# chagmgang/distributed_reinforcement_learning

Hardware: AMD Instinct MI355X
Metric: learner env-frames/sec (whole node), IMPALA deep-conv 84x84x4 (higher is better)
Workload: dtype bf16; 1 GPU; model=impala deep-conv 84x84x4 + LSTM256 V-trace, global_batch=32, seq_len=20, parallelism=dp1, num_action=18

## Files before the change

### distributed_reinforcement_learning_amd/models/blocks.py

```python

from __future__ import annotations

from typing import List, Optional, Sequence

import torch
import torch.nn as nn
import torch.nn.functional as F


class AtariConvStack(nn.Module):

    def __init__(self, in_channels: int):
        super().__init__()
        self.conv1 = nn.Conv2d(in_channels, 32, kernel_size=8, stride=4)
        self.conv2 = nn.Conv2d(32, 64, kernel_size=4, stride=2)
        self.conv3 = nn.Conv2d(64, 64, kernel_size=3, stride=1)
        self.out_features = 7 * 7 * 64
        self.conv1.to(memory_format=torch.channels_last)
        self.conv2.to(memory_format=torch.channels_last)
        self.conv3.to(memory_format=torch.channels_last)

    def forward(self, x_nhwc: torch.Tensor) -> torch.Tensor:
        if x_nhwc.is_cuda and x_nhwc.dtype == torch.uint8:
            from distributed_reinforcement_learning_amd.ops.conv_op import (
                atari_conv_stack, custom_stack_ok,
            )
            assert custom_stack_ok(self, x_nhwc), (
                "uint8 frames on GPU require the custom conv stack "
                "(bf16 weights + built extension)")
            return atari_conv_stack(self, x_nhwc)
        x = x_nhwc.to(self.conv1.weight.dtype).permute(0, 3, 1, 2)
        if x.device.type == "cuda":
            x = x.contiguous(memory_format=torch.channels_last)
        else:
            x = x.contiguous()
        x = F.relu(self.conv1(x))
        x = F.relu(self.conv2(x))
        x = F.relu(self.conv3(x))
        return x.permute(0, 2, 3, 1).flatten(1)


class ActionEmbedding(nn.Module):

    def __init__(self, num_action: int, hidden: int = 256):
        super().__init__()
        self.num_action = num_action
        self.table = nn.Parameter(torch.empty(num_action, hidden))
        self.bias1 = nn.Parameter(torch.zeros(hidden))
        nn.init.kaiming_uniform_(self.table, a=5 ** 0.5)
        self.fc2 = nn.Linear(hidden, hidden)
        self.out_features = hidden

    def forward(self, prev_action: torch.Tensor) -> torch.Tensor:
        from distributed_reinforcement_learning_amd.ops import embed_op, available
        t = self.table
        if (t.is_cuda and t.dtype == torch.bfloat16
                and t.shape[1] == 256 and self.fc2.out_features == 256
                and available()):
            return embed_op.fused_action_embed(
                prev_action.long(), t, self.bias1, self.fc2.weight,
                self.fc2.bias)
        x = F.relu(embed_op.embed_lookup(t, prev_action) + self.bias1)
        return F.relu(self.fc2(x))


class MLPHead(nn.Module):

    def __init__(self, in_features: int, hidden_list: Sequence[int],
                 out_features: int,
                 final_activation: Optional[str] = None):
        super().__init__()
        layers: List[nn.Module] = []
        prev = in_features
        for h in hidden_list:
            layers.append(nn.Linear(prev, h))
            prev = h
        self.hidden = nn.ModuleList(layers)
        self.out = nn.Linear(prev, out_features)
        self.final_activation = final_activation

    def logits(self, x: torch.Tensor) -> torch.Tensor:
        x = x.to(self.out.weight.dtype)
        for layer in self.hidden:
            x = F.relu(layer(x))
        return self.out(x)

    def forward(self, x: torch.Tensor) -> torch.Tensor:
        x = self.logits(x)
        if self.final_activation == "softmax":
            x = F.softmax(x.float(), dim=-1)
        return x


class _AugGateWeight(torch.autograd.Function):

    PAD = 8

    @staticmethod
    def forward(ctx, weight: torch.Tensor, bias: torch.Tensor):
        K, G = weight.shape
        ctx.K = K
        return weight.as_strided((K + _AugGateWeight.PAD, G), (G, 1))

    @staticmethod
    def backward(ctx, d_aug: torch.Tensor):
        return d_aug[:ctx.K], d_aug[ctx.K]


class LSTMCellTF(nn.Module):

    def __init__(self, input_size: int, hidden_size: int,
                 forget_bias: float = 1.0):
        super().__init__()
        self.input_size = input_size
        self.hidden_size = hidden_size
        self.forget_bias = forget_bias
        self.weight = nn.Parameter(
            torch.empty(input_size + hidden_size, 4 * hidden_size))
        self.bias = nn.Parameter(torch.zeros(4 * hidden_size))
        nn.init.xavier_uniform_(self.weight)

    def gates_from_xh(self, xh: torch.Tensor) -> torch.Tensor:
        if xh.is_cuda and xh.dtype == torch.bfloat16:
            return torch.addmm(self.bias, xh, self.weight)
        return torch.addmm(self.bias.to(xh.dtype), xh, self.weight)

    def _aug_weight_ok(self) -> bool:
        w, b = self.weight, self.bias
        if not (w.is_cuda and w.dtype == torch.bfloat16
                and b.dtype == w.dtype and w.numel() % 8 == 0
                and w.data_ptr() + w.numel() * w.element_size()
                == b.data_ptr()):
            return False
        need = (w.storage_offset() + w.numel()
                + _AugGateWeight.PAD * w.shape[1]) * w.element_size()
        return w.untyped_storage().nbytes() >= need

    def _ones_col(self, n: int, xh_dtype, dev) -> torch.Tensor:
        cache = getattr(self, "_ones_cache", None)
        if cache is None:
            cache = self._ones_cache = {}
        key = (n, xh_dtype, dev)
        if key not in cache:
            pad = torch.zeros(n, _AugGateWeight.PAD, dtype=xh_dtype,
                              device=dev)
            pad[:, 0] = 1
            cache[key] = pad
        return cache[key]

    def forward_cat(self, parts, c: torch.Tensor):
        dtype = parts[0].dtype
        parts = [p if p.dtype == dtype else p.to(dtype) for p in parts]
        if self._aug_weight_ok():
            n = parts[0].shape[0]
            xh = torch.cat(parts + [self._ones_col(n, dtype,
                                                   parts[0].device)], dim=1)
            g = torch.mm(xh, _AugGateWeight.apply(self.weight, self.bias))
        else:
            xh = torch.cat(parts, dim=1)
            g = self.gates_from_xh(xh)
        from distributed_reinforcement_learning_amd.ops.lstm_op import (
            lstm_fused_step,
        )
        if g.is_cuda:
            return lstm_fused_step(g, c.float(), self.forget_bias)
        return lstm_fused_step(g.float(), c.float(), self.forget_bias)

    def forward_xh(self, xh: torch.Tensor, c: torch.Tensor):
        from distributed_reinforcement_learning_amd.ops.lstm_op import (
            lstm_fused_step,
        )
        g = self.gates_from_xh(xh)
        if g.is_cuda:
            return lstm_fused_step(g, c.float(), self.forget_bias)
        return lstm_fused_step(g.float(), c.float(), self.forget_bias)

    def gates(self, x: torch.Tensor, h: torch.Tensor) -> torch.Tensor:
        xh = torch.cat([x, h.to(x.dtype)], dim=1)
        return torch.addmm(self.bias.to(xh.dtype), xh, self.weight)

    def forward(self, x: torch.Tensor, h: torch.Tensor, c: torch.Tensor):
        g = self.gates(x, h)
        from distributed_reinforcement_learning_amd.ops import lstm_fused_step
        if g.is_cuda:
            return lstm_fused_step(g, c.float(), self.forget_bias)
        return lstm_fused_step(g.float(), c.float(), self.forget_bias)
```

### distributed_reinforcement_learning_amd/models/impala_actor_critic.py

```python

from __future__ import annotations

import torch
import torch.nn as nn

from distributed_reinforcement_learning_amd.models.blocks import (
    ActionEmbedding, AtariConvStack, LSTMCellTF, MLPHead,
)


class ImpalaActorCritic(nn.Module):
    def __init__(self, input_shape, num_action: int, lstm_hidden_size: int = 256):
        super().__init__()
        h, w, c = input_shape
        assert (h, w) == (84, 84), "Atari conv stack expects 84x84 frames"
        self.num_action = num_action
        self.lstm_hidden_size = lstm_hidden_size
        self.conv = AtariConvStack(c)
        self.action_emb = ActionEmbedding(num_action)
        feat = self.conv.out_features + self.action_emb.out_features
        self.lstm = LSTMCellTF(feat, lstm_hidden_size)
        self.policy_head = MLPHead(lstm_hidden_size, [256, 256], num_action,
                                   "softmax")
        self.value_head = MLPHead(lstm_hidden_size, [256, 256], 1, None)

    def single_step(self, state: torch.Tensor, prev_action: torch.Tensor,
                    h: torch.Tensor, c: torch.Tensor):
        feat = torch.cat(
            [self.conv(state), self.action_emb(prev_action)], dim=1)
        new_h, new_c = self.lstm(feat, h, c)
        policy = self.policy_head(new_h)
        value = self.value_head(new_h).squeeze(-1)
        return policy, value, new_h, new_c

    def forward(self, state, prev_action, h, c):
        return self.single_step(state, prev_action, h, c)

    def _unroll_features(self, traj_state, traj_prev_action, traj_h, traj_c):
        B, T = traj_state.shape[:2]
        flat_state = traj_state.reshape(B * T, *traj_state.shape[2:])
        flat_pa = traj_prev_action.reshape(B * T)
        flat_h = traj_h.reshape(B * T, -1)
        flat_c = traj_c.reshape(B * T, -1)
        conv_out = self.conv(flat_state)
        emb = self.action_emb(flat_pa)
        new_h, _ = self.lstm.forward_cat([conv_out, emb, flat_h], flat_c)
        return new_h, B, T

    def unroll(self, traj_state: torch.Tensor, traj_prev_action: torch.Tensor,
               traj_h: torch.Tensor, traj_c: torch.Tensor):
        h, B, T = self._unroll_features(traj_state, traj_prev_action,
                                        traj_h, traj_c)
        policy = self.policy_head(h)
        value = self.value_head(h).squeeze(-1)
        return policy.reshape(B, T, -1), value.reshape(B, T)

    def unroll_logits(self, traj_state, traj_prev_action, traj_h, traj_c):
        h, B, T = self._unroll_features(traj_state, traj_prev_action,
                                        traj_h, traj_c)
        from distributed_reinforcement_learning_amd.ops.mlp_heads_op import (
            fused_mlp_heads, heads_fusable,
        )
        if heads_fusable(self, h):
            logits, value = fused_mlp_heads(h.float(), self.policy_head,
                                            self.value_head)
            return logits.reshape(B, T, -1), value.reshape(B, T)
        logits = self.policy_head.logits(h)
        value = self.value_head(h).squeeze(-1)
        return logits.reshape(B, T, -1), value.reshape(B, T)
```

### distributed_reinforcement_learning_amd/ops/conv_op.py

```python

from __future__ import annotations

import torch

from distributed_reinforcement_learning_amd import ops as _ops

_LAYER_CO = {0: 32, 1: 32, 2: 64, 3: 64}

_WGRAD_STREAM = None


def _side_enabled() -> bool:
    import os
    return os.environ.get("DRLA_WGRAD_SIDE") == "1"


def wgrad_stream() -> torch.cuda.Stream:
    global _WGRAD_STREAM
    if _WGRAD_STREAM is None:
        _WGRAD_STREAM = torch.cuda.Stream()
    return _WGRAD_STREAM


def join_wgrad_stream() -> None:
    if _WGRAD_STREAM is not None:
        torch.cuda.current_stream().wait_stream(_WGRAD_STREAM)


STASH_INPUTS = False


class _ConvLayer(torch.autograd.Function):
    @staticmethod
    def forward(ctx, x: torch.Tensor, w_flat: torch.Tensor,
                bias_f32: torch.Tensor, layer: int):
        ext = _ops.require_ext()
        stash = STASH_INPUTS and layer <= 1
        y, x_st = ext.conv_fwd(layer, x.contiguous(), w_flat.contiguous(),
                               bias_f32.contiguous(), stash)
        ctx.save_for_backward(x_st if stash else x, w_flat, y)
        ctx.layer = layer
        return y

    @staticmethod
    def backward(ctx, dy: torch.Tensor):
        x, w_flat, y = ctx.saved_tensors
        ext = _ops.require_ext()
        layer = ctx.layer
        co = _LAYER_CO[layer]
        if not (dy.is_contiguous() or (dy.stride(-1) == 1
                                        and dy.dim() >= 2)):
            dy = dy.contiguous()
        dy_m = ext.relu_mask_bwd(dy, y, co, layer)
        if _side_enabled():
            cur = torch.cuda.current_stream()
            side = wgrad_stream()
            side.wait_stream(cur)
            with torch.cuda.stream(side):
                dw, dbias = ext.conv_wgrad(layer, x, dy_m)
            if not torch.cuda.is_current_stream_capturing():
                cur.wait_stream(side)
                for t in (dw, dbias):
                    t.record_stream(cur)
                for t in (x, dy_m):
                    t.record_stream(side)
        else:
            dw, dbias = ext.conv_wgrad(layer, x, dy_m)
        dx = None
        if layer >= 2 and ctx.needs_input_grad[0]:
            dx = ext.conv_dgrad(layer, dy_m, w_flat)
        return dx, dw, dbias, None


def conv_layer(x: torch.Tensor, conv: torch.nn.Conv2d,
               layer: int) -> torch.Tensor:
    w = conv.weight
    co = w.shape[0]
    w_flat = w.permute(0, 2, 3, 1).reshape(co, -1)
    return _ConvLayer.apply(x, w_flat, conv.bias, layer)


def atari_conv_stack(stack, x_u8_nhwc: torch.Tensor) -> torch.Tensor:
    ci = x_u8_nhwc.shape[-1]
    l1 = 0 if ci == 4 else 1
    y = conv_layer(x_u8_nhwc, stack.conv1, l1)
    y = conv_layer(y, stack.conv2, 2)
    y = conv_layer(y, stack.conv3, 3)
    return y.reshape(y.shape[0], -1)


def custom_stack_ok(stack, x: torch.Tensor) -> bool:
    return (x.is_cuda and x.dtype == torch.uint8
            and x.shape[1] == 84 and x.shape[2] == 84
            and x.shape[3] in (1, 4)
            and stack.conv1.weight.dtype == torch.bfloat16
            and _ops.available())
```

### distributed_reinforcement_learning_amd/ops/embed_op.py

```python

from __future__ import annotations

import torch

from distributed_reinforcement_learning_amd import ops as _ops


class _EmbedLookup(torch.autograd.Function):
    @staticmethod
    def forward(ctx, table: torch.Tensor, idx: torch.Tensor):
        ctx.save_for_backward(idx)
        ctx.num_rows = table.shape[0]
        ctx.want_bf16 = table.dtype == torch.bfloat16
        return table.index_select(0, idx)

    @staticmethod
    def backward(ctx, grad_out: torch.Tensor):
        (idx,) = ctx.saved_tensors
        ext = _ops.require_ext()
        grad_table = ext.embed_bwd(idx.contiguous(),
                                   grad_out.contiguous(), ctx.num_rows,
                                   ctx.want_bf16)
        return grad_table, None


def embed_lookup(table: torch.Tensor, idx: torch.Tensor) -> torch.Tensor:
    if table.is_cuda:
        return _EmbedLookup.apply(table, idx.long())
    return torch.nn.functional.embedding(idx.long(), table)


class _FusedActionEmbed(torch.autograd.Function):

    @staticmethod
    def forward(ctx, idx, table, b1, w2, b2):
        ext = _ops.require_ext()
        out, a1 = ext.embed_mlp_fwd(idx, table, b1, w2, b2)
        ctx.save_for_backward(idx, a1, out, w2)
        ctx.A = table.shape[0]
        ctx.set_materialize_grads(False)
        return out

    @staticmethod
    def backward(ctx, dy):
        idx, a1, out, w2 = ctx.saved_tensors
        ext = _ops.require_ext()
        if dy is None:
            return (None,) * 5
        if not (dy.dim() == 2 and dy.stride(1) == 1):
            dy = dy.contiguous()
        dz2, dtable, db1, db2 = ext.embed_mlp_bwd(
            dy.to(torch.bfloat16), out, a1, w2, idx, ctx.A)
        dw2 = dz2.t().mm(a1)
        return None, dtable, db1, dw2, db2


def fused_action_embed(idx, table, b1, w2, b2):
    return _FusedActionEmbed.apply(idx, table, b1, w2, b2)
```

### distributed_reinforcement_learning_amd/ops/hip/bind.cpp

```cpp

#include <torch/extension.h>
#include <ATen/hip/HIPContext.h>
#include <hip/hip_runtime.h>

#include <algorithm>
#include <array>
#include <tuple>

#include "drla_kernels.h"

namespace {

hipStream_t cur_stream() {
  return at::hip::getCurrentHIPStream().stream();
}

void check_gpu_contig(const torch::Tensor& t, const char* name) {
  TORCH_CHECK(t.is_cuda(), name, " must be on the GPU");
  TORCH_CHECK(t.is_contiguous(), name, " must be contiguous");
}

template <typename... Ts>
void check_all_gpu_contig(const char* what, const Ts&... ts) {
  (check_gpu_contig(ts, what), ...);
// ... 27 lines not shown
torch::Tensor normalize_frames_f32(torch::Tensor frames) {
  check_gpu_contig(frames, "frames");
  TORCH_CHECK(frames.scalar_type() == torch::kUInt8, "frames must be uint8");
  auto out = torch::empty_like(frames, frames.options().dtype(torch::kFloat));
  const long long n = frames.numel();
  const long long n4 = n / 4;
  if (n4 > 0) {
    hipLaunchKernelGGL(drla_u8_normalize_f32, dim3(drla_grid(n4)),
                       dim3(DRLA_BLOCK), 0, cur_stream(),
                       reinterpret_cast<const uchar4*>(frames.data_ptr<uint8_t>()),
                       reinterpret_cast<float4*>(out.data_ptr<float>()), n4);
  }
  if (n % 4) {
    hipLaunchKernelGGL(drla_u8_normalize_f32_tail, dim3(1), dim3(DRLA_BLOCK),
                       0, cur_stream(), frames.data_ptr<uint8_t>(),
                       out.data_ptr<float>(), n4 * 4, n);
  }
  return out;
}

torch::Tensor normalize_frames_bf16(torch::Tensor frames) {
  check_gpu_contig(frames, "frames");
  TORCH_CHECK(frames.scalar_type() == torch::kUInt8, "frames must be uint8");
  auto out = torch::empty_like(frames,
                               frames.options().dtype(torch::kBFloat16));
  const long long n = frames.numel();
  const long long n4 = n / 4;
  if (n4 > 0) {
    hipLaunchKernelGGL(drla_u8_normalize_bf16, dim3(drla_grid(n4)),
                       dim3(DRLA_BLOCK), 0, cur_stream(),
                       reinterpret_cast<const uchar4*>(frames.data_ptr<uint8_t>()),
                       reinterpret_cast<ushort4v*>(out.data_ptr()), n4);
  }
  if (n % 4) {
    hipLaunchKernelGGL(drla_u8_normalize_bf16_tail, dim3(1), dim3(DRLA_BLOCK),
                       0, cur_stream(), frames.data_ptr<uint8_t>(),
                       BF16PM(out), n4 * 4, n);
  }
  return out;
}

torch::Tensor vtrace_scan(torch::Tensor deltas, torch::Tensor discounts,
                          torch::Tensor cs) {
  for (auto* t : {&deltas, &discounts, &cs}) {
    check_gpu_contig(*t, "vtrace input");
    TORCH_CHECK(t->scalar_type() == torch::kFloat, "vtrace wants float32");
  }
  const int B = deltas.size(0);
  const int T = deltas.size(1);
  auto out = torch::empty_like(deltas);
  hipLaunchKernelGGL(drla_vtrace_scan, dim3(drla_grid(B)), dim3(DRLA_BLOCK),
                     0, cur_stream(), deltas.data_ptr<float>(),
                     discounts.data_ptr<float>(), cs.data_ptr<float>(),
                     out.data_ptr<float>(), B, T);
  return out;
}

constexpr auto kConvFwdU8 = std::array{&drla_conv_fwd_l1, &drla_conv_fwd_l1_c1};
constexpr auto kConvFwdBf16 = std::array{&drla_conv_fwd_l2, &drla_conv_fwd_l3};
constexpr auto kConvWgradU8 =
    std::array{&drla_conv_wgrad_l1, &drla_conv_wgrad_l1_c1};
constexpr auto kConvWgradBf16 =
    std::array{&drla_conv_wgrad_l2, &drla_conv_wgrad_l3};

const DrlaConvLayer& conv_layer(int layer) {
  TORCH_CHECK(layer >= 0 && layer < 4, "bad layer");
  return DRLA_CONV_LAYERS[layer];
}
int conv_m_tiles(int rows) { return (rows + DRLA_CONV_BM - 1) / DRLA_CONV_BM; }

torch::Tensor mfma_probe(torch::Tensor A, torch::Tensor B) {
  check_gpu_contig(A, "A");
  check_gpu_contig(B, "B");
  auto D = torch::empty({16, 16}, A.options().dtype(torch::kFloat));
  hipLaunchKernelGGL(drla_mfma_probe, dim3(1), dim3(64), 0, cur_stream(),
                     static_cast<const bf16raw*>(A.data_ptr()),
                     static_cast<const bf16raw*>(B.data_ptr()),
                     D.data_ptr<float>());
  return D;
}

std::tuple<torch::Tensor, torch::Tensor> conv_fwd(
    int layer, torch::Tensor in, torch::Tensor w, torch::Tensor bias,
    bool stash_input) {
  check_gpu_contig(in, "in");
  check_gpu_contig(w, "w");
  check_gpu_contig(bias, "bias");
  const auto& cfg = conv_layer(layer);
  const int batch = in.size(0);
  auto out = torch::empty({batch, cfg.ho, cfg.wo, cfg.co},
                          in.options().dtype(torch::kBFloat16));
  const dim3 grid(conv_m_tiles(batch * cfg.ho * cfg.wo));
  torch::Tensor x_stash;
  unsigned char* stashp = nullptr;
  if (stash_input) {
    TORCH_CHECK(layer <= 1, "input stash is a u8-layer feature");
    TORCH_CHECK((in.numel() % 16) == 0, "stash wants 16-divisible bytes");
    x_stash = torch::empty_like(in);
    stashp = x_stash.data_ptr<uint8_t>();
  }
  if (layer <= 1) {
    hipLaunchKernelGGL(kConvFwdU8[layer], grid, dim3(DRLA_CONV_BLOCK), 0,
                       cur_stream(), in.data_ptr<uint8_t>(), BF16P(w),
                       BF16P(bias), BF16PM(out), batch, stashp);
  } else {
    hipLaunchKernelGGL(kConvFwdBf16[layer - 2], grid, dim3(DRLA_CONV_BLOCK),
                       0, cur_stream(), BF16P(in), BF16P(w), BF16P(bias),
                       BF16PM(out), batch);
  }
  return {out, x_stash};
}

static torch::Tensor& dbias_slot_buf(const torch::Tensor& like,
                                     int64_t slot_id) {
  static torch::Tensor bufs[4];
  TORCH_CHECK(slot_id >= 0 && slot_id < 4, "bad slot id");
  if (!bufs[slot_id].defined()) {
    bufs[slot_id] =
        torch::zeros({DRLA_DBIAS_SLOTS * DRLA_DBIAS_STRIDE},
                     like.options().dtype(torch::kFloat));
  }
  return bufs[slot_id];
}

torch::Tensor relu_mask_bwd(torch::Tensor dy, torch::Tensor y, int64_t CO,
                            int64_t slot_id) {
  check_gpu_contig(y, "y");
  TORCH_CHECK(dy.is_cuda(), "dy must be on GPU");
  long long n_stride, row_elems;
  if (dy.is_contiguous()) {
    n_stride = row_elems = dy.numel() / dy.size(0);
  } else {
    row_elems = 1;
    for (int d = 1; d < dy.dim(); ++d) {
      TORCH_CHECK(dy.stride(d - 1) >= dy.stride(d), "dy must be row-major");
      row_elems *= dy.size(d);
    }
    TORCH_CHECK(dy.stride(dy.dim() - 1) == 1 &&
                    dy.stride(0) >= row_elems && row_elems % 8 == 0,
                "dy view must be inner-contiguous");
    for (int d = 1; d + 1 < dy.dim(); ++d) {
      TORCH_CHECK(dy.stride(d) == dy.size(d + 1) * dy.stride(d + 1),
                  "dy inner dims must be contiguous");
    }
    n_stride = dy.stride(0);
  }
  auto out = torch::empty(dy.sizes(), dy.options());
  auto& slots = dbias_slot_buf(dy, slot_id);
  const long long n = dy.numel();
  TORCH_CHECK(n % 8 == 0, "relu_mask_bwd wants numel % 8 == 0");
  int grid = drla_grid(n / 8);
  if (grid > 640) grid = 640;
  hipLaunchKernelGGL(drla_relu_mask_bwd, dim3(grid), dim3(DRLA_BLOCK),
                     0, cur_stream(), BF16P(dy), BF16P(y), BF16PM(out),
                     slots.data_ptr<float>(), n, (int)CO, n_stride,
                     row_elems);
  return out;
}

std::tuple<torch::Tensor, torch::Tensor> conv_wgrad(int layer,
                                                    torch::Tensor in,
                                                    torch::Tensor dy) {
  check_gpu_contig(in, "in");
  check_gpu_contig(dy, "dy");
  const auto& cfg = conv_layer(layer);
  const int batch = in.size(0);
  const int K = cfg.kh * cfg.kw * cfg.ci;
  static int split_env = [] {
    const char* e = getenv("DRLA_WGRAD_SPLIT");
    return e ? atoi(e) : 0;
  }();
  const int split = split_env ? split_env : ((layer <= 1) ? 512 : 64);
  static torch::Tensor scratch_cache[4];
  if (!scratch_cache[layer].defined()) {
    scratch_cache[layer] =
        torch::zeros({K, cfg.co}, dy.options().dtype(torch::kFloat));
  }
  auto scratch = scratch_cache[layer];
  const dim3 grid((K + DRLA_CONV_WGRAD_BK - 1) / DRLA_CONV_WGRAD_BK, split);
  if (layer <= 1) {
    hipLaunchKernelGGL(kConvWgradU8[layer], grid, dim3(DRLA_CONV_BLOCK), 0,
                       cur_stream(), in.data_ptr<uint8_t>(), BF16P(dy),
                       scratch.data_ptr<float>(), batch);
  } else {
    hipLaunchKernelGGL(kConvWgradBf16[layer - 2], grid,
                       dim3(DRLA_CONV_BLOCK), 0, cur_stream(), BF16P(in),
                       BF16P(dy), scratch.data_ptr<float>(), batch);
  }
  auto dw = torch::empty({cfg.co, K}, dy.options().dtype(torch::kBFloat16));
  auto dbias = torch::empty({cfg.co}, dy.options().dtype(torch::kBFloat16));
  auto& slots = dbias_slot_buf(dy, layer);
  hipLaunchKernelGGL(drla_wgrad_finalize,
                     dim3(drla_grid((long long)K * cfg.co)),
                     dim3(DRLA_BLOCK), 0, cur_stream(),
                     scratch.data_ptr<float>(), BF16PM(dw), K, cfg.co,
                     slots.data_ptr<float>(), BF16PM(dbias));
  return {dw, dbias};
}

torch::Tensor conv_dgrad(int layer, torch::Tensor dy, torch::Tensor w) {
  check_gpu_contig(dy, "dy");
  check_gpu_contig(w, "w");
  TORCH_CHECK(layer == 2 || layer == 3, "dgrad only for l2/l3");
  const auto& cfg = conv_layer(layer);
  const int batch = dy.size(0);
  auto dx = torch::empty({batch, cfg.hi, cfg.wi, cfg.ci},
                         dy.options().dtype(torch::kBFloat16));
  if (layer == 2) {
    const int grid_c = conv_m_tiles(batch * (cfg.hi / 2) * (cfg.wi / 2));
    hipLaunchKernelGGL(drla_conv_dgrad_l2, dim3(grid_c, 4),
                       dim3(DRLA_CONV_BLOCK), 0, cur_stream(), BF16P(dy),
                       BF16P(w), BF16PM(dx), batch);
  } else {
    hipLaunchKernelGGL(drla_conv_dgrad_l3,
                       dim3(conv_m_tiles(batch * cfg.hi * cfg.wi)),
                       dim3(DRLA_CONV_BLOCK), 0, cur_stream(), BF16P(dy),
                       BF16P(w), BF16PM(dx), batch);
  }
  return dx;
}

std::tuple<torch::Tensor, torch::Tensor> dqn_loss_fwd(
    torch::Tensor main_q, torch::Tensor next_main, torch::Tensor next_tgt,
    torch::Tensor actions, torch::Tensor rewards, torch::Tensor discounts,
    torch::Tensor weights) {
  check_all_gpu_contig("dqn_loss input", main_q, next_main, next_tgt,
                       actions, rewards, discounts, weights);
  TORCH_CHECK(actions.scalar_type() == torch::kInt, "actions must be i32");
  const int B = main_q.size(0), A = main_q.size(1);
  const DualPtr mq = dual_ptr(main_q);
  auto fopt = rewards.options().dtype(torch::kFloat);
  auto loss = torch::zeros({1}, fopt);
  auto td = torch::empty({B}, fopt);
  hipLaunchKernelGGL(
      drla_dqn_loss_fwd, dim3((B + 255) / 256), dim3(256), 0, cur_stream(),
      mq.bf16, mq.f32, next_main.data_ptr<float>(), next_tgt.data_ptr<float>(),
      actions.data_ptr<int>(), rewards.data_ptr<float>(),
      discounts.data_ptr<float>(), weights.data_ptr<float>(),
      loss.data_ptr<float>(), td.data_ptr<float>(), B, A);
// ... 229 lines not shown
  check_gpu_contig(tree, "tree");
  long long hi = cap - 1;
  while (hi > 0) {
    const long long lo = hi >> 1;
    const long long count = hi - lo;
    hipLaunchKernelGGL(drla_per_rebuild_level,
                       dim3((count + 255) / 256), dim3(256), 0,
                       cur_stream(), tree.data_ptr<float>(), lo, count);
    hi = lo;
  }
}

void multi_gather(torch::Tensor rows, torch::Tensor srcs,
                  torch::Tensor dsts, torch::Tensor fbytes,
                  int64_t max_chunks) {
  check_all_gpu_contig("multi_gather table", rows, srcs, dsts, fbytes);
  TORCH_CHECK(rows.scalar_type() == torch::kLong, "rows must be i64");
  const int B = rows.numel();
  const int F = srcs.numel();
  if (B == 0 || F == 0) return;
  const long long total = (long long)B * max_chunks;
  const int gx = (int)std::min<long long>((total + 255) / 256, 4096);
  hipLaunchKernelGGL(drla_multi_gather, dim3(gx, F), dim3(256), 0,
                     cur_stream(), i64p(rows), u64p(srcs), u64p(dsts),
                     i64p(fbytes), B);
}

std::tuple<torch::Tensor, torch::Tensor> per_sample(torch::Tensor tree,
                                                    torch::Tensor s,
                                                    torch::Tensor n_entries,
                                                    int64_t cap) {
  check_gpu_contig(tree, "tree");
  check_gpu_contig(s, "s");
  check_gpu_contig(n_entries, "n_entries");
  const int n = s.numel();
  auto idx = torch::empty({n}, s.options().dtype(torch::kLong));
  auto prio = torch::empty({n}, s.options().dtype(torch::kFloat));
  if (n == 0) return {idx, prio};
  hipLaunchKernelGGL(drla_per_sample, dim3((n + 255) / 256), dim3(256), 0,
                     cur_stream(), tree.data_ptr<float>(),
                     s.data_ptr<float>(), n_entries.data_ptr<float>(),
                     i64p(idx), prio.data_ptr<float>(), n, cap);
  return {idx, prio};
}

torch::Tensor embed_bwd(torch::Tensor indices, torch::Tensor grad_out,
                        int64_t num_rows, bool want_bf16) {
  check_gpu_contig(indices, "indices");
  check_gpu_contig(grad_out, "grad_out");
  TORCH_CHECK(indices.scalar_type() == torch::kLong, "indices must be i64");
  const long long N = grad_out.size(0);
  const int H = grad_out.size(1);
  const DualPtr go = dual_ptr(grad_out);
  torch::Tensor scratch;
  if (want_bf16) {
    static torch::Tensor emb_scratch;
    if (!emb_scratch.defined() || emb_scratch.size(0) != num_rows ||
        emb_scratch.size(1) != H) {
      emb_scratch = torch::zeros({num_rows, H},
                                 grad_out.options().dtype(torch::kFloat));
    }
    scratch = emb_scratch;
  } else {
    scratch = torch::zeros({num_rows, H},
                           grad_out.options().dtype(torch::kFloat));
  }
  hipLaunchKernelGGL(
      drla_embed_bwd_scatter, dim3(drla_grid(N * H)), dim3(DRLA_BLOCK), 0,
      cur_stream(), i64p(indices), go.bf16, go.f32,
      scratch.data_ptr<float>(), N, H, (long long)num_rows);
  if (!want_bf16) return scratch;
  auto out = torch::empty({num_rows, H},
                          grad_out.options().dtype(torch::kBFloat16));
  hipLaunchKernelGGL(drla_f32_to_bf16_zero_kernel,
                     dim3(drla_grid(num_rows * H)), dim3(DRLA_BLOCK), 0,
                     cur_stream(), scratch.data_ptr<float>(), BF16PM(out),
                     (long long)(num_rows * H));
  return out;
}

std::vector<torch::Tensor> vtrace_loss_fwd(
    torch::Tensor logits, torch::Tensor value, torch::Tensor mu,
    torch::Tensor actions, torch::Tensor rewards, torch::Tensor done,
    double gamma, int64_t clip_mode, double c_bl, double c_ent) {
  check_all_gpu_contig("vtrace_loss input", logits, value, mu, actions,
                       rewards, done);
  TORCH_CHECK(actions.scalar_type() == torch::kInt, "actions must be int32");
  TORCH_CHECK(done.scalar_type() == torch::kBool, "done must be bool");
  const int B = logits.size(0), T = logits.size(1), A = logits.size(2);
  TORCH_CHECK(A <= VT_MAX_A, "num_action cap is ", VT_MAX_A);
  TORCH_CHECK(T <= VT_MAX_T, "trajectory cap is ", VT_MAX_T);
  const DualPtr lg = dual_ptr(logits);
  auto fopt = value.options().dtype(torch::kFloat);
  auto p_stash = torch::empty({B, T, A}, fopt);
  auto vs_stash = torch::empty({B, T - 2}, fopt);
  auto adv_stash = torch::empty({B, T - 2}, fopt);
  auto losses = torch::zeros({4}, fopt);
  hipLaunchKernelGGL(
      drla_vtrace_loss_fwd, dim3(B), dim3(256), 0, cur_stream(),
      lg.bf16, lg.f32, value.data_ptr<float>(), mu.data_ptr<float>(),
      actions.data_ptr<int>(), rewards.data_ptr<float>(), boolp(done),
      static_cast<float>(gamma), (int)clip_mode, static_cast<float>(c_bl),
      static_cast<float>(c_ent), p_stash.data_ptr<float>(),
      vs_stash.data_ptr<float>(), adv_stash.data_ptr<float>(),
      losses.data_ptr<float>(), B, T, A);
  return {losses, p_stash, vs_stash, adv_stash};
}

std::tuple<torch::Tensor, torch::Tensor> vtrace_loss_bwd(
    torch::Tensor p_stash, torch::Tensor vs_stash, torch::Tensor adv_stash,
    torch::Tensor value, torch::Tensor actions, torch::Tensor grad3,
    bool from_total, double c_bl, double c_ent, bool want_bf16) {
  check_all_gpu_contig("vtrace_loss bwd input", p_stash, vs_stash,
                       adv_stash, value, actions, grad3);
  const int B = p_stash.size(0), T = p_stash.size(1), A = p_stash.size(2);
  auto dlogits = torch::empty(
      {B, T, A},
      value.options().dtype(want_bf16 ? torch::kBFloat16 : torch::kFloat));
  auto dvalue = torch::empty({B, T}, value.options().dtype(torch::kFloat));
  const DualPtr out = dual_ptr(dlogits);
  hipLaunchKernelGGL(
      drla_vtrace_loss_bwd, dim3(drla_grid((long long)B * T)), dim3(256), 0,
      cur_stream(), p_stash.data_ptr<float>(), vs_stash.data_ptr<float>(),
      adv_stash.data_ptr<float>(), value.data_ptr<float>(),
      actions.data_ptr<int>(), grad3.data_ptr<float>(),
      from_total ? 1 : 0, static_cast<float>(c_bl),
      static_cast<float>(c_ent), out.bf16, out.f32, dvalue.data_ptr<float>(),
      B, T, A);
  return {dlogits, dvalue};
}

std::tuple<torch::Tensor, torch::Tensor, torch::Tensor> lstm_tail_fwd(
    torch::Tensor gates, torch::Tensor c_prev, double forget_bias) {
  check_gpu_contig(gates, "gates");
  check_gpu_contig(c_prev, "c_prev");
  const bool bf16 = gates.scalar_type() == torch::kBFloat16;
  TORCH_CHECK(bf16 || gates.scalar_type() == torch::kFloat,
              "gates must be bf16 or float32");
  TORCH_CHECK(c_prev.scalar_type() == torch::kFloat, "c_prev must be float32");
  const long long N = gates.size(0);
  const int H4 = gates.size(1);
  TORCH_CHECK(H4 % 4 == 0, "gates dim1 must be 4*H");
  const int H = H4 / 4;
  TORCH_CHECK(c_prev.size(1) == H, "c_prev width mismatch");
  auto new_h = torch::empty_like(c_prev);
  auto new_c = torch::empty_like(c_prev);
  auto stash = torch::empty({N, (long long)H4},
                            c_prev.options().dtype(torch::kFloat));
  if (bf16) {
    hipLaunchKernelGGL(drla_lstm_tail_fwd_bf16, dim3(drla_grid(N * H)),
                       dim3(DRLA_BLOCK), 0, cur_stream(), BF16P(gates),
                       c_prev.data_ptr<float>(), new_h.data_ptr<float>(),
                       new_c.data_ptr<float>(), stash.data_ptr<float>(),
                       static_cast<float>(forget_bias), N, H);
  } else {
    hipLaunchKernelGGL(drla_lstm_tail_fwd, dim3(drla_grid(N * H)),
                       dim3(DRLA_BLOCK), 0, cur_stream(),
                       gates.data_ptr<float>(), c_prev.data_ptr<float>(),
                       new_h.data_ptr<float>(), new_c.data_ptr<float>(),
                       stash.data_ptr<float>(),
                       static_cast<float>(forget_bias), N, H);
  }
  return {new_h, new_c, stash};
}

std::tuple<torch::Tensor, torch::Tensor> lstm_tail_bwd(
    torch::Tensor grad_h, c10::optional<torch::Tensor> grad_c_opt,
    torch::Tensor stash, torch::Tensor c_prev, torch::Tensor new_c,
    bool bf16_gates) {
  check_all_gpu_contig("lstm bwd input", stash, c_prev, new_c);
  const float* grad_c_ptr = nullptr;
  if (grad_c_opt.has_value()) {
    check_gpu_contig(*grad_c_opt, "grad_c");
    grad_c_ptr = grad_c_opt->data_ptr<float>();
  }
  TORCH_CHECK(grad_h.is_cuda() && grad_h.dim() == 2 &&
              grad_h.stride(1) == 1, "grad_h must be row-contiguous");
  const long long gh_stride = grad_h.stride(0);
  const long long N = stash.size(0);
  const int H = stash.size(1) / 4;
  auto grad_c_prev = torch::empty_like(c_prev);
  if (bf16_gates) {
    auto grad_gates = torch::empty(
        {N, (long long)stash.size(1)},
        stash.options().dtype(torch::kBFloat16));
    hipLaunchKernelGGL(drla_lstm_tail_bwd_bf16, dim3(drla_grid(N * H)),
                       dim3(DRLA_BLOCK), 0, cur_stream(),
                       grad_h.data_ptr<float>(), grad_c_ptr,
                       stash.data_ptr<float>(), c_prev.data_ptr<float>(),
                       new_c.data_ptr<float>(), BF16PM(grad_gates),
                       grad_c_prev.data_ptr<float>(), N, H, gh_stride);
    return {grad_gates, grad_c_prev};
  }
  auto grad_gates = torch::empty_like(stash);
  hipLaunchKernelGGL(drla_lstm_tail_bwd, dim3(drla_grid(N * H)),
                     dim3(DRLA_BLOCK), 0, cur_stream(),
                     grad_h.data_ptr<float>(), grad_c_ptr,
                     stash.data_ptr<float>(), c_prev.data_ptr<float>(),
                     new_c.data_ptr<float>(), grad_gates.data_ptr<float>(),
                     grad_c_prev.data_ptr<float>(), N, H, gh_stride);
  return {grad_gates, grad_c_prev};
}

int mh_row_tiles(int N) { return (N + MH_BM - 1) / MH_BM; }

std::vector<torch::Tensor> mlp_heads_fwd(
    torch::Tensor h, std::vector<torch::Tensor> weights,
    std::vector<torch::Tensor> biases, int64_t A) {
  check_gpu_contig(h, "h");
  TORCH_CHECK(weights.size() == 6 && biases.size() == 6);
  for (auto& t : weights) check_gpu_contig(t, "W");
  for (auto& t : biases) check_gpu_contig(t, "b");
  const int N = h.size(0);
  TORCH_CHECK(h.size(1) == MH_HID && A <= MH_MAX_A);
  auto bopt = h.options().dtype(torch::kBFloat16);
  auto logits = torch::empty({N, A}, bopt);
  auto value = torch::empty({N}, h.options().dtype(torch::kFloat));
  auto stash = torch::empty({N, 5 * 256}, bopt);
  hipLaunchKernelGGL(
      drla_mlp_heads_fwd, dim3(mh_row_tiles(N), 2), dim3(256), 0,
      cur_stream(), h.data_ptr<float>(),
      BF16P(weights[0]), BF16P(biases[0]), BF16P(weights[1]),
      BF16P(biases[1]), BF16P(weights[2]), BF16P(biases[2]),
      BF16P(weights[3]), BF16P(biases[3]), BF16P(weights[4]),
      BF16P(biases[4]), BF16P(weights[5]), BF16P(biases[5]),
      BF16PM(logits), value.data_ptr<float>(), BF16PM(stash), N, (int)A);
  return {logits, value, stash};
}

std::vector<torch::Tensor> mlp_heads_bwd(
    torch::Tensor dlogits, torch::Tensor dvalue, torch::Tensor stash,
    std::vector<torch::Tensor> weights, int64_t A) {
  check_gpu_contig(dlogits, "dlogits");
  check_gpu_contig(dvalue, "dvalue");
  check_gpu_contig(stash, "stash");
  TORCH_CHECK(weights.size() == 6);
  const int N = dvalue.numel();
  auto bopt = dlogits.options().dtype(torch::kBFloat16);
  auto fopt = dvalue.options().dtype(torch::kFloat);
  auto dz1p = torch::empty({N, 256}, bopt);
  auto dz2p = torch::empty({N, 256}, bopt);
  auto dz1v = torch::empty({N, 256}, bopt);
  auto dz2v = torch::empty({N, 256}, bopt);
  const long long ws_n = (long long)N * 256 + 4 * 256 + A + 1;
  auto ws = torch::zeros({ws_n}, fopt);
  long long off = 0;
  auto dh = ws.narrow(0, off, (long long)N * 256).view({N, 256});
  off += (long long)N * 256;
  auto db1p = ws.narrow(0, off, 256); off += 256;
  auto db2p = ws.narrow(0, off, 256); off += 256;
  auto db3p = ws.narrow(0, off, A); off += A;
  auto db1v = ws.narrow(0, off, 256); off += 256;
  auto db2v = ws.narrow(0, off, 256); off += 256;
  auto db3v = ws.narrow(0, off, 1);
  hipLaunchKernelGGL(
      drla_mlp_heads_bwd, dim3(mh_row_tiles(N), 2), dim3(256), 0,
      cur_stream(), BF16P(dlogits), dvalue.data_ptr<float>(), BF16P(stash),
      BF16P(weights[0]), BF16P(weights[1]), BF16P(weights[2]),
      BF16P(weights[3]), BF16P(weights[4]), BF16P(weights[5]), BF16PM(dz1p),
      BF16PM(dz2p), BF16PM(dz1v), BF16PM(dz2v), dh.data_ptr<float>(),
      db1p.data_ptr<float>(), db2p.data_ptr<float>(),
      db3p.data_ptr<float>(), db1v.data_ptr<float>(),
      db2v.data_ptr<float>(), db3v.data_ptr<float>(), N, (int)A);
  return {dz1p, dz2p, dz1v, dz2v, dh,   db1p, db2p, db3p, db1v, db2v,
          db3v, ws};
}

std::tuple<torch::Tensor, torch::Tensor> embed_mlp_fwd(
    torch::Tensor pa, torch::Tensor table, torch::Tensor b1,
    torch::Tensor w2, torch::Tensor b2) {
  check_all_gpu_contig("embed fwd input", pa, table, b1, w2, b2);
  TORCH_CHECK(pa.scalar_type() == torch::kLong, "pa must be int64");
  const int N = pa.numel();
  auto bopt = table.options();
  auto out = torch::empty({N, 256}, bopt);
  auto a1 = torch::empty({N, 256}, bopt);
  hipLaunchKernelGGL(drla_embed_mlp_fwd, dim3(mh_row_tiles(N)), dim3(256), 0,
                     cur_stream(), i64p(pa), BF16P(table), BF16P(b1),
                     BF16P(w2), BF16P(b2), BF16PM(out), BF16PM(a1), N,
                     (int)table.size(0));
  return {out, a1};
}

std::vector<torch::Tensor> embed_mlp_bwd(torch::Tensor dy, torch::Tensor out,
                                         torch::Tensor a1, torch::Tensor w2,
                                         torch::Tensor idx, int64_t A) {
  check_all_gpu_contig("embed bwd input", out, a1, w2);
  check_gpu_contig(idx, "idx");
  TORCH_CHECK(dy.is_cuda() && dy.dim() == 2 && dy.stride(1) == 1,
              "dy must be row-contiguous");
  const int N = out.size(0);
  const long long n_table = (long long)A * 256;
  auto bopt = out.options();
  static torch::Tensor w2t, scratch;
  if (!w2t.defined()) w2t = torch::empty({65536}, bopt);
  if (!scratch.defined() || scratch.numel() != n_table + 512) {
    scratch = torch::zeros({n_table + 512}, bopt.dtype(torch::kFloat));
  }
  hipLaunchKernelGGL(drla_embed_w2t_pack, dim3(drla_grid(65536)),
                     dim3(DRLA_BLOCK), 0, cur_stream(), BF16P(w2),
                     BF16PM(w2t));
  auto dz2 = torch::empty({N, 256}, bopt);
  auto da1 = torch::empty({N, 256}, bopt);
  float* bias_ws = scratch.data_ptr<float>() + n_table;
  hipLaunchKernelGGL(drla_embed_mlp_bwd, dim3(mh_row_tiles(N)), dim3(256), 0,
                     cur_stream(), BF16P(dy), (long long)dy.stride(0),
                     BF16P(out), BF16P(a1), BF16P(w2t), BF16PM(dz2),
                     BF16PM(da1), bias_ws, N);
  hipLaunchKernelGGL(
      drla_embed_bwd_scatter, dim3(drla_grid((long long)N * 256)),
      dim3(DRLA_BLOCK), 0, cur_stream(), i64p(idx), BF16P(da1), nullptr,
      scratch.data_ptr<float>(), N, 256, (long long)A);
  auto dtable = torch::empty({A, 256}, bopt);
  auto db1 = torch::empty({256}, bopt);
  auto db2 = torch::empty({256}, bopt);
  hipLaunchKernelGGL(drla_embed_finalize, dim3(drla_grid(n_table + 512)),
                     dim3(DRLA_BLOCK), 0, cur_stream(),
                     scratch.data_ptr<float>(), BF16PM(dtable), BF16PM(db1),
                     BF16PM(db2), n_table);
  return {dz2, dtable, db1, db2};
}

torch::Tensor mlp_heads_pack_wt(std::vector<torch::Tensor> weights,
                                int64_t A) {
  TORCH_CHECK(weights.size() == 6);
  for (auto& w : weights) check_gpu_contig(w, "pack weight");
  auto out = torch::empty({4 * 65536 + 256 * 32 + 256},
                          weights[0].options());
  hipLaunchKernelGGL(drla_heads_wt_pack, dim3(drla_grid(out.numel())),
                     dim3(DRLA_BLOCK), 0, cur_stream(), BF16P(weights[0]),
                     BF16P(weights[1]), BF16P(weights[2]), BF16P(weights[3]),
                     BF16P(weights[4]), BF16P(weights[5]), BF16PM(out),
                     (int)A);
  return out;
}

std::vector<torch::Tensor> mlp_heads_wgrad(
    torch::Tensor dz1p, torch::Tensor dz2p, torch::Tensor dz1v,
    torch::Tensor dz2v, torch::Tensor dlogits, torch::Tensor dvalue,
    torch::Tensor stash, torch::Tensor ws, int64_t A) {
  check_all_gpu_contig("wgrad input", dz1p, dz2p, dz1v, dz2v, dlogits, stash,
                       ws);
  check_gpu_contig(dvalue, "dvalue");
  const int N = dvalue.numel();
  auto bopt = dz1p.options();
  auto dw1p = torch::empty({256, 256}, bopt);
  auto dw2p = torch::empty({256, 256}, bopt);
  auto dw3p = torch::empty({A, 256}, bopt);
  auto dw1v = torch::empty({256, 256}, bopt);
  auto dw2v = torch::empty({256, 256}, bopt);
  auto dw3v = torch::empty({1, 256}, bopt);
  auto db1p = torch::empty({256}, bopt);
  auto db2p = torch::empty({256}, bopt);
  auto db3p = torch::empty({A}, bopt);
  auto db1v = torch::empty({256}, bopt);
  auto db2v = torch::empty({256}, bopt);
  auto db3v = torch::empty({1}, bopt);
  const float* ws_tail = ws.data_ptr<float>() + (long long)N * 256;
  hipLaunchKernelGGL(drla_heads_wgrad, dim3(73), dim3(256), 0, cur_stream(),
                     BF16P(dz1p), BF16P(dz2p), BF16P(dz1v), BF16P(dz2v),
                     BF16P(dlogits), dvalue.data_ptr<float>(), BF16P(stash),
                     BF16PM(dw1p), BF16PM(dw2p), BF16PM(dw3p), BF16PM(dw1v),
                     BF16PM(dw2v), BF16PM(dw3v), ws_tail, BF16PM(db1p),
                     BF16PM(db2p), BF16PM(db3p), BF16PM(db1v), BF16PM(db2v),
                     BF16PM(db3v), N, (int)A);
  return {dw1p, dw2p, dw3p, dw1v, dw2v, dw3v,
          db1p, db2p, db3p, db1v, db2v, db3v};
}

void check_lstm_seq_hidden(int H, const torch::Tensor& Wh) {
  TORCH_CHECK(H >= 1 && H <= LSTM_SEQ_MAX_HIDDEN, "lstm hidden cap is ",
              LSTM_SEQ_MAX_HIDDEN, ", got H=", H);
  TORCH_CHECK(Wh.numel() == (int64_t)drla_lstm_seq_wh_elems(H),
              "Wh must be [H, 4H] for H=", H);
}
void check_lstm_seq_wide_wh(const torch::Tensor& Wh) {
  TORCH_CHECK(reinterpret_cast<uintptr_t>(Wh.data_ptr()) % 4 == 0,
              "lstm wide kernels need a 4-byte aligned Wh");
}

std::tuple<torch::Tensor, torch::Tensor, torch::Tensor> lstm_seq_fwd(
    torch::Tensor xgates, torch::Tensor Wh, torch::Tensor h0,
    torch::Tensor c0, torch::Tensor done, double forget_bias) {
  check_all_gpu_contig("lstm_seq input", xgates, Wh, h0, c0, done);
  TORCH_CHECK(done.scalar_type() == torch::kBool, "done must be bool");
  const int B = xgates.size(0), L = xgates.size(1);
  const int H = xgates.size(2) / 4;
  check_lstm_seq_hidden(H, Wh);
  const bool wh_in_lds = drla_lstm_seq_wh_fits_lds(H);
  const DualPtr xg = dual_ptr(xgates);
  auto fopt = h0.options().dtype(torch::kFloat);
  auto h_out = torch::empty({B, L, H}, fopt);
  auto h_fin = torch::empty({B, H}, fopt);
  auto c_fin = torch::empty({B, H}, fopt);
  if (4 * H > LSTM_SEQ_MAX_GATES) {
// ... 145 lines not shown
}

void adam_step_bf16_t(torch::Tensor p, torch::Tensor g, torch::Tensor master,
                      torch::Tensor m, torch::Tensor v, double clip,
                      torch::Tensor lr_buf, double beta1, double beta2,
                      double eps) {
  check_all_gpu_contig("adam bf16 tensor", p, g, master, m, v, lr_buf);
  const long long n = p.numel();
  torch::Tensor norm_buf;
  if (clip > 0) {
    norm_buf = sq_norm_bf16(g);
  } else {
    norm_buf = torch::zeros({1}, master.options());
  }
  hipLaunchKernelGGL(drla_adam_step_bf16, dim3(drla_grid(n)),
                     dim3(DRLA_BLOCK), 0, cur_stream(), BF16PM(p), BF16P(g),
                     master.data_ptr<float>(), m.data_ptr<float>(),
                     v.data_ptr<float>(), norm_buf.data_ptr<float>(),
                     static_cast<float>(clip), lr_buf.data_ptr<float>(),
                     static_cast<float>(beta1), static_cast<float>(beta2),
                     static_cast<float>(eps), n);
}

void rmsprop_step_t(torch::Tensor p, torch::Tensor g, torch::Tensor ms,
                    double clip, torch::Tensor lr_buf, double rho,
                    double eps) {
  check_all_gpu_contig("rmsprop tensor", p, g, ms, lr_buf);
  const long long n = p.numel();
  torch::Tensor norm_buf;
  if (clip > 0) {
    norm_buf = sq_norm(g);
  } else {
    norm_buf = torch::zeros({1}, p.options());
  }
  hipLaunchKernelGGL(drla_rmsprop_step, dim3(drla_grid(n)), dim3(DRLA_BLOCK),
                     0, cur_stream(), p.data_ptr<float>(),
                     g.data_ptr<float>(), ms.data_ptr<float>(),
                     norm_buf.data_ptr<float>(), static_cast<float>(clip),
                     lr_buf.data_ptr<float>(), static_cast<float>(rho),
                     static_cast<float>(eps), n);
}

void rmsprop_step(torch::Tensor p, torch::Tensor g, torch::Tensor ms,
                  double clip, double lr, double rho, double eps) {
  auto lr_buf = torch::full({1}, lr, p.options());
  rmsprop_step_t(p, g, ms, clip, lr_buf, rho, eps);
}

void adam_step_t(torch::Tensor p, torch::Tensor g, torch::Tensor m,
                 torch::Tensor v, double clip, torch::Tensor lr_buf,
                 double beta1, double beta2, double eps) {
  check_all_gpu_contig("adam tensor", p, g, m, v, lr_buf);
  const long long n = p.numel();
  torch::Tensor norm_buf;
  if (clip > 0) {
    norm_buf = sq_norm(g);
  } else {
    norm_buf = torch::zeros({1}, p.options());
  }
  hipLaunchKernelGGL(drla_adam_step, dim3(drla_grid(n)), dim3(DRLA_BLOCK), 0,
                     cur_stream(), p.data_ptr<float>(), g.data_ptr<float>(),
                     m.data_ptr<float>(), v.data_ptr<float>(),
                     norm_buf.data_ptr<float>(), static_cast<float>(clip),
                     lr_buf.data_ptr<float>(), static_cast<float>(beta1),
                     static_cast<float>(beta2), static_cast<float>(eps), n);
}

void adam_step(torch::Tensor p, torch::Tensor g, torch::Tensor m,
               torch::Tensor v, double clip, double lr_t, double beta1,
               double beta2, double eps) {
  auto lr_buf = torch::full({1}, lr_t, p.options());
  adam_step_t(p, g, m, v, clip, lr_buf, beta1, beta2, eps);
}

}

PYBIND11_MODULE(TORCH_EXTENSION_NAME, m) {
  m.def("normalize_frames_f32", &normalize_frames_f32,
        "uint8 frames -> float32/255 (K11)");
  m.def("normalize_frames_bf16", &normalize_frames_bf16,
        "uint8 frames -> bf16/255 (K11)");
  m.def("vtrace_scan", &vtrace_scan, "fused V-trace reverse scan (K5)");
  m.def("vtrace_loss_fwd", &vtrace_loss_fwd,
        "fused IMPALA loss pipeline forward (K5+K7+K13)");
  m.def("vtrace_loss_bwd", &vtrace_loss_bwd,
        "fused IMPALA loss pipeline backward (closed form)");
  m.def("mfma_probe", &mfma_probe, "16x16x32 bf16 MFMA layout probe");
  m.def("conv_fwd", &conv_fwd,
        "MFMA implicit-GEMM conv fwd, fused normalize+bias+ReLU (K1)");
  m.def("conv_wgrad", &conv_wgrad, "MFMA conv weight gradient (K1 bwd)");
  m.def("conv_dgrad", &conv_dgrad, "MFMA conv data gradient (K1 bwd)");
  m.def("relu_mask_bwd", &relu_mask_bwd,
        "fused-ReLU backward mask + bias gradient");
  m.def("dqn_loss_fwd", &dqn_loss_fwd,
        "fused double-DQN target + IS-weighted TD loss (K8)");
  m.def("dqn_loss_bwd", &dqn_loss_bwd, "closed-form K8 backward");
  m.def("a2c_loss_fwd", &a2c_loss_fwd, "fused A2C loss fwd (K6)");
  m.def("a2c_loss_bwd", &a2c_loss_bwd, "fused A2C loss bwd (K6)");
  m.def("r2d2_loss_fwd", &r2d2_loss_fwd,
        "fused R2D2 sequence-TD tail fwd (K9; n_step > 1 or "
        "priority_eta >= 0 selects the n-step kernel)",
        py::arg("mq"), py::arg("tq"), py::arg("actions"), py::arg("rewards"),
        py::arg("done"), py::arg("weights"), py::arg("gamma"),
        py::arg("clip_mode"), py::arg("n_step") = 1,
        py::arg("priority_eta") = -1.0);
  m.def("dhead_train_fwd", &dhead_train_fwd,
        "grad-carrying dueling head fwd (R2D2 trained window)");
  m.def("dhead_train_bwd", &dhead_train_bwd,
        "grad-carrying dueling head bwd chain + weight grads");
  m.def("dueling_head_fwd", &dueling_head_fwd,
        "no-grad dueling head over the post-burn-in window");
  m.def("r2d2_loss_bwd", &r2d2_loss_bwd,
        "fused R2D2 sequence-TD tail bwd (K9)");
  m.def("per_update", &per_update, "GPU PER segment-tree batched update");
  m.def("per_sample", &per_sample, "GPU PER stratified sample descent");
  m.def("multi_gather", &multi_gather,
        "one-kernel replay batch gather (all fields)");
  m.def("per_rebuild", &per_rebuild,
        "GPU PER interior-sum rebuild (float32 drift repair)");
  m.def("embed_bwd", &embed_bwd,
        "action-embedding table gradient (K2 backward)");
  m.def("lstm_tail_fwd", &lstm_tail_fwd, "fused LSTM gate tail fwd (K3)");
  m.def("lstm_tail_bwd", &lstm_tail_bwd, "fused LSTM gate tail bwd (K3)");
  m.def("mlp_heads_fwd", &mlp_heads_fwd,
        "fused policy+value MLP heads forward (K4)");
  m.def("mlp_heads_bwd", &mlp_heads_bwd,
        "fused heads dgrad chain + ReLU masks + bias grads (K4 bwd)");
  m.def("embed_mlp_fwd", &embed_mlp_fwd,
        "fused action-embedding MLP forward (K2)");
  m.def("embed_mlp_bwd", &embed_mlp_bwd,
        "fused action-embedding MLP backward (K2 bwd)");
  m.def("mlp_heads_pack_wt", &mlp_heads_pack_wt,
        "one-kernel transposed-weight pack for the heads dgrad");
  m.def("mlp_heads_wgrad", &mlp_heads_wgrad,
        "all six head wgrads (dW = dz^T @ act) in one MFMA launch");
  m.def("lstm_seq_train_fwd", &lstm_seq_train_fwd,
        "grad-carrying whole-sequence LSTM forward (K3 seq, R2D2 train)");
  m.def("lstm_seq_train_bwd", &lstm_seq_train_bwd,
        "whole-sequence LSTM backward (one kernel over the recurrence)");
  m.def("lstm_seq_fwd", &lstm_seq_fwd,
        "whole no-grad LSTM unroll in one kernel (K3 seq / burn-in)");
  m.def("sq_norm", &sq_norm, "squared L2 norm of a flat tensor (K12)");
  m.def("grad_gather", &grad_gather,
        "one-kernel scattered-grad -> flat bucket pack (K12b)");
  m.def("rmsprop_step", &rmsprop_step,
        "fused global-norm-clip + TF-RMSProp update (K12)");
  m.def("rmsprop_step_t", &rmsprop_step_t,
        "RMSProp update with device-tensor lr (hipGraph-safe)");
  m.def("adam_step", &adam_step,
        "fused global-norm-clip + TF-Adam update (K12)");
  m.def("adam_step_t", &adam_step_t,
        "Adam update with device-tensor lr_t (hipGraph-safe)");
  m.def("sq_norm_bf16", &sq_norm_bf16, "squared L2 norm of a bf16 tensor");
  m.def("rmsprop_step_bf16_t", &rmsprop_step_bf16_t,
        "bf16-model/fp32-master RMSProp (K12, mixed precision)");
  m.def("adam_step_bf16_t", &adam_step_bf16_t,
        "bf16-model/fp32-master Adam (K12, mixed precision)");
}
```

### distributed_reinforcement_learning_amd/ops/hip/conv.hip

```cpp

#include "drla_kernels.h"

#define CONV_KERNEL \
  extern "C" __global__ __launch_bounds__(DRLA_CONV_BLOCK) void

__device__ __forceinline__ float cv_bf2f(bf16raw u) {
  unsigned int x = ((unsigned int)u) << 16;
  return __uint_as_float(x);
}

extern "C" __global__ void drla_mfma_probe(const bf16raw* __restrict__ A,
                                           const bf16raw* __restrict__ B,
                                           float* __restrict__ D) {
  const int l = threadIdx.x;
  bf16x8 a_frag, b_frag;
  for (int e = 0; e < 8; ++e) {
    a_frag[e] = (short)A[(l & 15) * 32 + ((l >> 4) * 8 + e)];
    b_frag[e] = (short)B[((l >> 4) * 8 + e) * 16 + (l & 15)];
  }
  f32x4 acc = {0.f, 0.f, 0.f, 0.f};
  acc = __builtin_amdgcn_mfma_f32_16x16x32_bf16(a_frag, b_frag, acc, 0, 0, 0);
  for (int r = 0; r < 4; ++r) {
    D[((l >> 4) * 4 + r) * 16 + (l & 15)] = acc[r];
  }
}


template <typename IN_T, int CI, int CO, int KH, int KW, int STRIDE, int HI,
          int WI, int HO, int WO>
__device__ void conv_fwd_impl(const IN_T* __restrict__ in,
                              const bf16raw* __restrict__ w,
                              const bf16raw* __restrict__ bias,
                              bf16raw* __restrict__ out,
                              int batch,
                              IN_T* __restrict__ x_stash = nullptr) {
  constexpr int K = KH * KW * CI;
  constexpr int BM = DRLA_CONV_BM;
  constexpr int BK = 32;
  constexpr int APAD = 8;
  constexpr int NFRAG = CO / 16;
  const int M = batch * HO * WO;

  __shared__ bf16raw Abuf[BM][BK + APAD];
  __shared__ bf16raw Bbuf[CO][BK + APAD];
  __shared__ float BiasBuf[CO];

  const int tid = threadIdx.x;
  const int wave = tid / 64;
  const int lane = tid % 64;
  const int row0 = blockIdx.x * BM;

  if (tid < CO) BiasBuf[tid] = cv_bf2f(bias[tid]);

  f32x4 acc[2][NFRAG];
  for (int mi = 0; mi < 2; ++mi)
    for (int ni = 0; ni < NFRAG; ++ni)
      acc[mi][ni] = {0.f, 0.f, 0.f, 0.f};

  const int a_row = tid >> 1;
  const int a_k0 = (tid & 1) * 16;
  const int gm = row0 + a_row;
  const int n_idx = gm / (HO * WO);
  const int rem = gm - n_idx * (HO * WO);
  const int ho = rem / WO;
  const int wo = rem - ho * WO;
  const long long in_base =
      ((long long)n_idx * HI + ho * STRIDE) * WI + wo * STRIDE;

  unsigned int ra4u_0, ra4u_1, ra4u_2, ra4u_3;
  unsigned int ra1u[4];
  bf16x8 rab0 = {0, 0, 0, 0, 0, 0, 0, 0}, rab1 = rab0;
  uint4 rbw4;
  uint2 rbw2;
  constexpr int THREADS_PER_CO = DRLA_CONV_BLOCK / CO;
  constexpr int KCHUNK = BK / THREADS_PER_CO;
  const int b_co = tid / THREADS_PER_CO;
  const int b_kpart = (tid % THREADS_PER_CO) * KCHUNK;

  auto load_chunk = [&](int k0) {
    if (gm < M) {
      if constexpr (CI == 4) {
        const int kk = k0 + a_k0;
        const int kh = kk / (KW * CI);
        const int kw = (kk - kh * KW * CI) / CI;
        const uint4 packed = *reinterpret_cast<const uint4*>(
            in + (in_base + (long long)kh * WI + kw) * CI);
        ra4u_0 = packed.x; ra4u_1 = packed.y;
        ra4u_2 = packed.z; ra4u_3 = packed.w;
      } else if constexpr (CI == 1) {
        const int kh0 = (k0 + a_k0) / KW;
#pragma unroll
        for (int rrow = 0; rrow < 2; ++rrow) {
          const unsigned char* src =
              in + in_base + (long long)(kh0 + rrow) * WI;
          ra1u[rrow * 2 + 0] = *reinterpret_cast<const unsigned int*>(src);
          ra1u[rrow * 2 + 1] =
              *reinterpret_cast<const unsigned int*>(src + 4);
        }
      } else {
        const int kk = k0 + a_k0;
        const int kh = kk / (KW * CI);
        const int kwci = kk - kh * KW * CI;
        const int kw = kwci / CI;
        const int ci = kwci - kw * CI;
        const bf16raw* src = reinterpret_cast<const bf16raw*>(in) +
                             (in_base + (long long)kh * WI + kw) * CI + ci;
        rab0 = *reinterpret_cast<const bf16x8*>(src);
        rab1 = *reinterpret_cast<const bf16x8*>(src + 8);
      }
    }
    const bf16raw* src = w + (long long)b_co * K + k0 + b_kpart;
    if constexpr (KCHUNK == 8) {
      rbw4 = *reinterpret_cast<const uint4*>(src);
    } else {
      rbw2 = *reinterpret_cast<const uint2*>(src);
    }
  };

  auto store_chunk = [&]() {
    if (gm < M) {
      if constexpr (CI == 4) {
        const float sc = 1.0f / 255.0f;
#define DRLA_CF_PUT(t, u)                                               \
        {                                                               \
          const int o = a_k0 + (t) * 4;                                 \
          Abuf[a_row][o + 0] = drla_f32_to_bf16((float)((u) & 0xFF) * sc); \
          Abuf[a_row][o + 1] =                                          \
              drla_f32_to_bf16((float)(((u) >> 8) & 0xFF) * sc);        \
          Abuf[a_row][o + 2] =                                          \
              drla_f32_to_bf16((float)(((u) >> 16) & 0xFF) * sc);       \
          Abuf[a_row][o + 3] = drla_f32_to_bf16((float)((u) >> 24) * sc); \
        }
        DRLA_CF_PUT(0, ra4u_0); DRLA_CF_PUT(1, ra4u_1);
        DRLA_CF_PUT(2, ra4u_2); DRLA_CF_PUT(3, ra4u_3);
#undef DRLA_CF_PUT
      } else if constexpr (CI == 1) {
        const float sc = 1.0f / 255.0f;
#pragma unroll
        for (int q = 0; q < 4; ++q) {
          const unsigned int u = ra1u[q];
          Abuf[a_row][a_k0 + q * 4 + 0] =
              drla_f32_to_bf16((float)(u & 0xFF) * sc);
          Abuf[a_row][a_k0 + q * 4 + 1] =
              drla_f32_to_bf16((float)((u >> 8) & 0xFF) * sc);
          Abuf[a_row][a_k0 + q * 4 + 2] =
              drla_f32_to_bf16((float)((u >> 16) & 0xFF) * sc);
          Abuf[a_row][a_k0 + q * 4 + 3] =
              drla_f32_to_bf16((float)(u >> 24) * sc);
        }
      } else {
        *reinterpret_cast<bf16x8*>(&Abuf[a_row][a_k0]) = rab0;
        *reinterpret_cast<bf16x8*>(&Abuf[a_row][a_k0 + 8]) = rab1;
      }
    } else {
      for (int t = 0; t < 16; t += 8) {
        *reinterpret_cast<uint4*>(&Abuf[a_row][a_k0 + t]) = uint4{0, 0, 0, 0};
      }
    }
    if constexpr (KCHUNK == 8) {
      *reinterpret_cast<uint4*>(&Bbuf[b_co][b_kpart]) = rbw4;
    } else {
      *reinterpret_cast<uint2*>(&Bbuf[b_co][b_kpart]) = rbw2;
    }
  };

  load_chunk(0);
  for (int k0 = 0; k0 < K; k0 += BK) {
    store_chunk();
    __syncthreads();
    if (k0 + BK < K) load_chunk(k0 + BK);
    for (int mi = 0; mi < 2; ++mi) {
      const int arow = wave * 32 + mi * 16 + (lane & 15);
      const bf16x8 a_frag =
          *reinterpret_cast<const bf16x8*>(&Abuf[arow][(lane >> 4) * 8]);
      for (int ni = 0; ni < NFRAG; ++ni) {
        const bf16x8 b_frag = *reinterpret_cast<const bf16x8*>(
            &Bbuf[ni * 16 + (lane & 15)][(lane >> 4) * 8]);
        acc[mi][ni] = __builtin_amdgcn_mfma_f32_16x16x32_bf16(
            a_frag, b_frag, acc[mi][ni], 0, 0, 0);
      }
    }
    __syncthreads();
  }

  for (int mi = 0; mi < 2; ++mi) {
    for (int ni = 0; ni < NFRAG; ++ni) {
      const int col = ni * 16 + (lane & 15);
      const float b = BiasBuf[col];
      for (int r = 0; r < 4; ++r) {
        const int grow = row0 + wave * 32 + mi * 16 + (lane >> 4) * 4 + r;
        if (grow < M) {
          const float v = fmaxf(acc[mi][ni][r] + b, 0.0f);
          out[(long long)grow * CO + col] = drla_f32_to_bf16(v);
        }
      }
    }
  }

  if (x_stash) {
    const long long n16 =
        (long long)batch * HI * WI * CI * (long long)sizeof(IN_T) / 16;
    const uint4* src = reinterpret_cast<const uint4*>(in);
    uint4* dst = reinterpret_cast<uint4*>(x_stash);
    const long long nthreads = gridDim.x * (long long)blockDim.x;
    for (long long i = blockIdx.x * (long long)blockDim.x + threadIdx.x;
         i < n16; i += nthreads) {
      dst[i] = src[i];
    }
  }
}


CONV_KERNEL drla_conv_fwd_l1(
    const unsigned char* in, const bf16raw* w, const bf16raw* bias,
    bf16raw* out, int batch, unsigned char* x_stash) {
  conv_fwd_impl<unsigned char, DRLA_CONV_GEOM(0)>(in, w, bias, out, batch,
                                                  x_stash);
}

CONV_KERNEL drla_conv_fwd_l1_c1(
    const unsigned char* in, const bf16raw* w, const bf16raw* bias,
    bf16raw* out, int batch, unsigned char* x_stash) {
  conv_fwd_impl<unsigned char, DRLA_CONV_GEOM(1)>(in, w, bias, out, batch,
                                                  x_stash);
}

CONV_KERNEL drla_conv_fwd_l2(
    const bf16raw* in, const bf16raw* w, const bf16raw* bias, bf16raw* out,
    int batch) {
  conv_fwd_impl<bf16raw, DRLA_CONV_GEOM(2)>(in, w, bias, out, batch);
}

CONV_KERNEL drla_conv_fwd_l3(
    const bf16raw* in, const bf16raw* w, const bf16raw* bias, bf16raw* out,
    int batch) {
  conv_fwd_impl<bf16raw, DRLA_CONV_GEOM(3)>(in, w, bias, out, batch);
}


extern "C" __global__ void drla_relu_mask_bwd(
    const bf16raw* __restrict__ dy, const bf16raw* __restrict__ y,
    bf16raw* __restrict__ out, float* __restrict__ dbias_slots,
    long long n, int CO, long long n_stride, long long row_elems) {
  const long long n8 = n / 8;
  const long long stride = gridDim.x * (long long)blockDim.x;
  long long i = blockIdx.x * (long long)blockDim.x + threadIdx.x;
  const int tid = threadIdx.x;
  float acc[8] = {0, 0, 0, 0, 0, 0, 0, 0};
  const uint4* dy4 = reinterpret_cast<const uint4*>(dy);
  const uint4* y4 = reinterpret_cast<const uint4*>(y);
  uint4* out4 = reinterpret_cast<uint4*>(out);
#define DRLA_RM_LANE(dw, yw, ow, a0, a1)                              \
  {                                                                   \
    const bf16raw d0 = (bf16raw)((dw) & 0xFFFF);                      \
    const bf16raw d1 = (bf16raw)((dw) >> 16);                         \
    const bf16raw m0 =                                                \
        (cv_bf2f((bf16raw)((yw) & 0xFFFF)) > 0.0f) ? d0 : (bf16raw)0; \
    const bf16raw m1 =                                                \
        (cv_bf2f((bf16raw)((yw) >> 16)) > 0.0f) ? d1 : (bf16raw)0;    \
    (ow) = ((unsigned int)m1 << 16) | m0;                             \
    (a0) += cv_bf2f(m0);                                              \
    (a1) += cv_bf2f(m1);                                              \
  }
  const long long row8 = row_elems / 8;
  const bool strided = (n_stride != row_elems);
  for (; i < n8; i += stride) {
    long long si = i;
    if (strided) {
      const long long r = i / row8;
      si = (r * n_stride + (i - r * row8) * 8) / 8;
    }
    const uint4 dv = dy4[si];
    const uint4 yv = y4[i];
    uint4 ov;
    DRLA_RM_LANE(dv.x, yv.x, ov.x, acc[0], acc[1]);
    DRLA_RM_LANE(dv.y, yv.y, ov.y, acc[2], acc[3]);
    DRLA_RM_LANE(dv.z, yv.z, ov.z, acc[4], acc[5]);
    DRLA_RM_LANE(dv.w, yv.w, ov.w, acc[6], acc[7]);
    out4[i] = ov;
  }
#undef DRLA_RM_LANE
  __shared__ float red[DRLA_BLOCK * 8];
  for (int e = 0; e < 8; ++e) red[tid * 8 + e] = acc[e];
  __syncthreads();
  if (tid < CO) {
    const int g = tid / 8;
    const int e = tid % 8;
    float s = 0.0f;
    for (int t = g; t < DRLA_BLOCK; t += CO / 8) s += red[t * 8 + e];
    atomicAdd(&dbias_slots[(blockIdx.x & (DRLA_DBIAS_SLOTS - 1)) *
                               DRLA_DBIAS_STRIDE +
                           tid], s);
  }
}

extern "C" __global__ void drla_wgrad_finalize(
    float* __restrict__ scratch, bf16raw* __restrict__ dw, int K,
    int CO, float* __restrict__ dbias_slots,
    bf16raw* __restrict__ dbias) {
  if (dbias_slots && blockIdx.x == 0 && (int)threadIdx.x < CO) {
    float s = 0.0f;
    for (int t = 0; t < DRLA_DBIAS_SLOTS; ++t) {
      s += dbias_slots[t * DRLA_DBIAS_STRIDE + threadIdx.x];
      dbias_slots[t * DRLA_DBIAS_STRIDE + threadIdx.x] = 0.0f;
    }
    dbias[threadIdx.x] = drla_f32_to_bf16(s);
  }
  long long i = blockIdx.x * (long long)blockDim.x + threadIdx.x;
  const long long total = (long long)K * CO;
  const long long stride = gridDim.x * (long long)blockDim.x;
  for (; i < total; i += stride) {
    const int co = i / K;
    const int k = i - (long long)co * K;
    const long long si = (long long)k * CO + co;
    dw[i] = drla_f32_to_bf16(scratch[si]);
    scratch[si] = 0.0f;
  }
}


template <typename IN_T, int CI, int CO, int KH, int KW, int STRIDE, int HI,
          int WI, int HO, int WO>
__device__ void conv_wgrad_impl(const IN_T* __restrict__ in,
                                const bf16raw* __restrict__ dy,
                                float* __restrict__ scratch,
                                int batch) {
  constexpr int K = KH * KW * CI;
  constexpr int BKM = 64;
  constexpr int BKK = DRLA_CONV_WGRAD_BK;
  constexpr int PAD = 8;
  constexpr int NFRAG = CO / 16;
  constexpr int CO_PER_T = (CO * 32) / DRLA_CONV_BLOCK;
  const int M = batch * HO * WO;

  __shared__ bf16raw Am[2][BKK][BKM + PAD];
  __shared__ bf16raw BmT[2][CO][BKM + PAD];

  const int tid = threadIdx.x;
  const int wave = tid / 64;
  const int lane = tid % 64;
  const int k_row0 = blockIdx.x * BKK;

  f32x4 acc[NFRAG];
  for (int ni = 0; ni < NFRAG; ++ni) acc[ni] = {0.f, 0.f, 0.f, 0.f};

  const int m_per_split = (M + gridDim.y - 1) / gridDim.y;
  const int m_begin = blockIdx.y * m_per_split;
  const int m_end = min(M, m_begin + m_per_split);

  const int a_m = tid >> 2;
  const int a_k = (tid & 3) * 16;
  long long a_off0 = 0, a_off1 = 0;
  long long a_offc[16];
  if constexpr (CI == 4) {
    const int kb = k_row0 + a_k;
    const int kh = kb / (KW * CI);
// ... 452 lines not shown
```

### distributed_reinforcement_learning_amd/ops/hip/drla_kernels.h

```cpp
#pragma once

#include <hip/hip_runtime.h>

#include "drla_common.h"

#define DRLA_KERNEL extern "C" __global__ void

DRLA_KERNEL drla_u8_normalize_f32(const uchar4*, float4*, long long);
DRLA_KERNEL drla_u8_normalize_bf16(const uchar4*, ushort4v*, long long);
DRLA_KERNEL drla_u8_normalize_f32_tail(const unsigned char*, float*,
                                       long long, long long);
DRLA_KERNEL drla_u8_normalize_bf16_tail(const unsigned char*, bf16raw*,
                                        long long, long long);
DRLA_KERNEL drla_embed_bwd_scatter(const long long*, const bf16raw*,
                                   const float*, float*, long long, int,
                                   long long);
DRLA_KERNEL drla_f32_to_bf16_zero_kernel(float*, bf16raw*, long long);

DRLA_KERNEL drla_vtrace_scan(const float*, const float*, const float*,
                             float*, int, int);

DRLA_KERNEL drla_vtrace_loss_fwd(
    const bf16raw*, const float*, const float*, const float*, const int*,
    const float*, const unsigned char*, float, int, float, float, float*,
    float*, float*, float*, int, int, int);
DRLA_KERNEL drla_vtrace_loss_bwd(
    const float*, const float*, const float*, const float*, const int*,
    const float*, int, float, float, bf16raw*, float*, float*, int, int,
    int);

DRLA_KERNEL drla_lstm_tail_fwd(const float*, const float*, float*, float*,
                               float*, float, long long, int);
DRLA_KERNEL drla_lstm_tail_bwd(const float*, const float*, const float*,
                               const float*, const float*, float*, float*,
                               long long, int, long long);
DRLA_KERNEL drla_lstm_tail_fwd_bf16(const bf16raw*, const float*, float*,
                                    float*, float*, float, long long, int);
DRLA_KERNEL drla_lstm_tail_bwd_bf16(const float*, const float*, const float*,
                                    const float*, const float*, bf16raw*,
                                    float*, long long, int, long long);
DRLA_KERNEL drla_lstm_seq_fwd(
    const bf16raw*, const float*, const bf16raw*, const float*, const float*,
    const unsigned char*, float*, float*, float*, float, int, int, int);
DRLA_KERNEL drla_lstm_seq_fwd_gmem(
    const bf16raw*, const float*, const bf16raw*, const float*, const float*,
    const unsigned char*, float*, float*, float*, float, int, int, int);
DRLA_KERNEL drla_lstm_seq_train_fwd(
    const bf16raw*, const bf16raw*, const float*, const float*,
    const unsigned char*, float*, float*, float*, float*, float*, bf16raw*,
    float, int, int, int);
DRLA_KERNEL drla_lstm_seq_train_bwd(
    const float*, const float*, const float*, const float*, const float*,
    const bf16raw*, const unsigned char*, bf16raw*, float*, float*, int, int,
    int);
DRLA_KERNEL drla_lstm_seq_wide_fwd(
    const bf16raw*, const float*, const bf16raw*, const float*, const float*,
    const unsigned char*, float*, float*, float*, float, int, int, int);
DRLA_KERNEL drla_lstm_seq_wide_train_fwd(
    const bf16raw*, const bf16raw*, const float*, const float*,
    const unsigned char*, float*, float*, float*, float*, float*, bf16raw*,
    float, int, int, int);
DRLA_KERNEL drla_lstm_seq_wide_train_bwd(
    const float*, const float*, const float*, const float*, const float*,
    const bf16raw*, const unsigned char*, bf16raw*, float*, float*, int, int,
    int);

DRLA_KERNEL drla_sq_norm(const float*, float*, long long);
DRLA_KERNEL drla_sq_norm_bf16(const bf16raw*, float*, long long);
DRLA_KERNEL drla_rmsprop_step(float*, const float*, float*, const float*,
                              float, const float*, float, float, long long);
DRLA_KERNEL drla_rmsprop_step_bf16(bf16raw*, const bf16raw*, float*, float*,
                                   const float*, float, const float*, float,
                                   float, long long);
DRLA_KERNEL drla_adam_step(float*, const float*, float*, float*,
                           const float*, float, const float*, float, float,
                           float, long long);
DRLA_KERNEL drla_adam_step_bf16(bf16raw*, const bf16raw*, float*, float*,
                                float*, const float*, float, const float*,
                                float, float, float, long long);
DRLA_KERNEL drla_grad_gather(const unsigned long long*, const long long*,
                             const long long*, bf16raw*, int, long long,
                             float*, int);

DRLA_KERNEL drla_mfma_probe(const bf16raw*, const bf16raw*, float*);
DRLA_KERNEL drla_conv_fwd_l1(const unsigned char*, const bf16raw*,
                             const bf16raw*, bf16raw*, int, unsigned char*);
DRLA_KERNEL drla_conv_fwd_l1_c1(const unsigned char*, const bf16raw*,
                                const bf16raw*, bf16raw*, int,
                                unsigned char*);
DRLA_KERNEL drla_conv_fwd_l2(const bf16raw*, const bf16raw*, const bf16raw*,
                             bf16raw*, int);
DRLA_KERNEL drla_conv_fwd_l3(const bf16raw*, const bf16raw*, const bf16raw*,
                             bf16raw*, int);
DRLA_KERNEL drla_relu_mask_bwd(const bf16raw*, const bf16raw*, bf16raw*,
                               float*, long long, int, long long, long long);
DRLA_KERNEL drla_wgrad_finalize(float*, bf16raw*, int, int, float*,
                                bf16raw*);
DRLA_KERNEL drla_conv_wgrad_l1(const unsigned char*, const bf16raw*, float*,
                               int);
DRLA_KERNEL drla_conv_wgrad_l1_c1(const unsigned char*, const bf16raw*,
                                  float*, int);
DRLA_KERNEL drla_conv_wgrad_l2(const bf16raw*, const bf16raw*, float*, int);
DRLA_KERNEL drla_conv_wgrad_l3(const bf16raw*, const bf16raw*, float*, int);
DRLA_KERNEL drla_conv_dgrad_l2(const bf16raw*, const bf16raw*, bf16raw*,
                               int);
DRLA_KERNEL drla_conv_dgrad_l3(const bf16raw*, const bf16raw*, bf16raw*,
                               int);

DRLA_KERNEL drla_per_update(float*, const long long*, const float*, int,
                            long long);
DRLA_KERNEL drla_per_rebuild_level(float*, long long, long long);
DRLA_KERNEL drla_multi_gather(const long long*, const unsigned long long*,
                              const unsigned long long*, const long long*,
                              int);
DRLA_KERNEL drla_per_sample(const float*, const float*, const float*,
                            long long*, float*, int, long long);

DRLA_KERNEL drla_dqn_loss_fwd(
    const bf16raw*, const float*, const float*, const float*, const int*,
    const float*, const float*, const float*, float*, float*, int, int);
DRLA_KERNEL drla_dqn_loss_bwd(const float*, const int*, const float*,
                              const float*, bf16raw*, float*, int, int);

DRLA_KERNEL drla_a2c_loss_fwd(
    const bf16raw*, const float*, const float*, const float*, const int*,
    const float*, const unsigned char*, float, int, float, float, float*,
    float*, float*, int, int);
DRLA_KERNEL drla_a2c_loss_bwd(const float*, const float*, const int*,
                              const float*, int, float, float, bf16raw*,
                              float*, float*, int, int);

DRLA_KERNEL drla_r2d2_loss_fwd(
    const bf16raw*, const float*, const bf16raw*, const float*, const int*,
    const float*, const unsigned char*, const float*, float, int, float*,
    float*, float*, int, int, int);
DRLA_KERNEL drla_r2d2_nstep_loss_fwd(
    const bf16raw*, const float*, const bf16raw*, const float*, const int*,
    const float*, const unsigned char*, const float*, float, int, int, float,
    float*, float*, float*, int, int, int);
DRLA_KERNEL drla_r2d2_loss_bwd(const float*, const int*, const float*,
                               const float*, bf16raw*, float*, int, int,
                               int);
DRLA_KERNEL drla_dueling_head_fwd(
    const float*, const bf16raw*, const bf16raw*, const bf16raw*,
    const bf16raw*, bf16raw*, int, int, int, int, int, int);
DRLA_KERNEL drla_dhead_train_fwd(
    const float*, const bf16raw*, const bf16raw*, const bf16raw*,
    const bf16raw*, bf16raw*, bf16raw*, int, int, int, int);
DRLA_KERNEL drla_dhead_train_bwd(
    const bf16raw*, const bf16raw*, const float*, const bf16raw*,
    const bf16raw*, float*, float*, int, int, int, int);
DRLA_KERNEL drla_dhead_train_fin(const float*, bf16raw*, bf16raw*, bf16raw*,
                                 bf16raw*, int, int, int);

DRLA_KERNEL drla_mlp_heads_fwd(
    const float*, const bf16raw*, const bf16raw*, const bf16raw*,
    const bf16raw*, const bf16raw*, const bf16raw*, const bf16raw*,
    const bf16raw*, const bf16raw*, const bf16raw*, const bf16raw*,
    const bf16raw*, bf16raw*, float*, bf16raw*, int, int);
DRLA_KERNEL drla_mlp_heads_bwd(
    const bf16raw*, const float*, const bf16raw*, const bf16raw*,
    const bf16raw*, const bf16raw*, const bf16raw*, const bf16raw*,
    const bf16raw*, bf16raw*, bf16raw*, bf16raw*, bf16raw*, float*, float*,
    float*, float*, float*, float*, float*, int, int);
DRLA_KERNEL drla_heads_wt_pack(const bf16raw*, const bf16raw*,
                               const bf16raw*, const bf16raw*,
                               const bf16raw*, const bf16raw*, bf16raw*,
                               int);
DRLA_KERNEL drla_heads_wgrad(
    const bf16raw*, const bf16raw*, const bf16raw*, const bf16raw*,
    const bf16raw*, const float*, const bf16raw*, bf16raw*, bf16raw*,
    bf16raw*, bf16raw*, bf16raw*, bf16raw*, const float*, bf16raw*,
    bf16raw*, bf16raw*, bf16raw*, bf16raw*, bf16raw*, int, int);
DRLA_KERNEL drla_embed_mlp_fwd(const long long*, const bf16raw*,
                               const bf16raw*, const bf16raw*,
                               const bf16raw*, bf16raw*, bf16raw*, int, int);
DRLA_KERNEL drla_embed_w2t_pack(const bf16raw*, bf16raw*);
DRLA_KERNEL drla_embed_mlp_bwd(const bf16raw*, long long, const bf16raw*,
                               const bf16raw*, const bf16raw*, bf16raw*,
                               bf16raw*, float*, int);
DRLA_KERNEL drla_embed_finalize(float*, bf16raw*, bf16raw*, bf16raw*,
                                long long);

#undef DRLA_KERNEL
```

### distributed_reinforcement_learning_amd/ops/hip/lstm_gates.hip

```cpp

#include "drla_kernels.h"

__device__ __forceinline__ float lstm_b2f(bf16raw u) {
  unsigned int x = ((unsigned int)u) << 16;
  return __uint_as_float(x);
}

extern "C" __global__ void drla_lstm_tail_fwd(
    const float* __restrict__ gates, const float* __restrict__ c_prev,
    float* __restrict__ new_h, float* __restrict__ new_c,
    float* __restrict__ stash,
    float forget_bias, long long N, int H) {
  long long idx = blockIdx.x * (long long)blockDim.x + threadIdx.x;
  const long long total = N * H;
  const long long stride = gridDim.x * (long long)blockDim.x;
  for (; idx < total; idx += stride) {
    const long long n = idx / H;
    const int h = idx - n * H;
    const long long g0 = n * 4LL * H + h;
    const float i_s = drla_sigmoid(gates[g0]);
    const float g_t = tanhf(gates[g0 + H]);
    const float f_s = drla_sigmoid(gates[g0 + 2 * H] + forget_bias);
    const float o_s = drla_sigmoid(gates[g0 + 3 * H]);
    const float c_new = f_s * c_prev[idx] + i_s * g_t;
    new_c[idx] = c_new;
    new_h[idx] = o_s * tanhf(c_new);
    stash[g0] = i_s;
    stash[g0 + H] = g_t;
    stash[g0 + 2 * H] = f_s;
    stash[g0 + 3 * H] = o_s;
  }
}

extern "C" __global__ void drla_lstm_tail_bwd(
    const float* __restrict__ grad_h, const float* __restrict__ grad_c,
    const float* __restrict__ stash, const float* __restrict__ c_prev,
    const float* __restrict__ new_c, float* __restrict__ grad_gates,
    float* __restrict__ grad_c_prev, long long N, int H,
    long long gh_stride) {
  long long idx = blockIdx.x * (long long)blockDim.x + threadIdx.x;
  const long long total = N * H;
  const long long stride = gridDim.x * (long long)blockDim.x;
  for (; idx < total; idx += stride) {
    const long long n = idx / H;
    const int h = idx - n * H;
    const long long g0 = n * 4LL * H + h;
    const float i_s = stash[g0];
    const float g_t = stash[g0 + H];
    const float f_s = stash[g0 + 2 * H];
    const float o_s = stash[g0 + 3 * H];
    const float tc = tanhf(new_c[idx]);
    const float dh = grad_h[n * gh_stride + h];
    const float gc = grad_c ? grad_c[idx] : 0.0f;
    const float d_tc = dh * o_s * (1.0f - tc * tc) + gc;
    grad_c_prev[idx] = d_tc * f_s;
    const float di = d_tc * g_t;
    const float dg = d_tc * i_s;
    const float df = d_tc * c_prev[idx];
    const float do_ = dh * tc;
    grad_gates[g0] = di * i_s * (1.0f - i_s);
    grad_gates[g0 + H] = dg * (1.0f - g_t * g_t);
    grad_gates[g0 + 2 * H] = df * f_s * (1.0f - f_s);
    grad_gates[g0 + 3 * H] = do_ * o_s * (1.0f - o_s);
  }
}

extern "C" __global__ void drla_lstm_tail_fwd_bf16(
    const unsigned short* __restrict__ gates,
    const float* __restrict__ c_prev, float* __restrict__ new_h,
    float* __restrict__ new_c, float* __restrict__ stash, float forget_bias,
    long long N, int H) {
  long long idx = blockIdx.x * (long long)blockDim.x + threadIdx.x;
  const long long total = N * H;
  const long long stride = gridDim.x * (long long)blockDim.x;
  for (; idx < total; idx += stride) {
    const long long n = idx / H;
    const int h = idx - n * H;
    const long long g0 = n * 4LL * H + h;
    const float i_s = drla_sigmoid(lstm_b2f(gates[g0]));
    const float g_t = tanhf(lstm_b2f(gates[g0 + H]));
    const float f_s = drla_sigmoid(lstm_b2f(gates[g0 + 2 * H])
                                   + forget_bias);
    const float o_s = drla_sigmoid(lstm_b2f(gates[g0 + 3 * H]));
    const float c_new = f_s * c_prev[idx] + i_s * g_t;
    new_c[idx] = c_new;
    new_h[idx] = o_s * tanhf(c_new);
    stash[g0] = i_s;
    stash[g0 + H] = g_t;
    stash[g0 + 2 * H] = f_s;
    stash[g0 + 3 * H] = o_s;
  }
}

extern "C" __global__ void drla_lstm_tail_bwd_bf16(
    const float* __restrict__ grad_h, const float* __restrict__ grad_c,
    const float* __restrict__ stash, const float* __restrict__ c_prev,
    const float* __restrict__ new_c, unsigned short* __restrict__ grad_gates,
    float* __restrict__ grad_c_prev, long long N, int H,
    long long gh_stride) {
  long long idx = blockIdx.x * (long long)blockDim.x + threadIdx.x;
  const long long total = N * H;
  const long long stride = gridDim.x * (long long)blockDim.x;
  for (; idx < total; idx += stride) {
    const long long n = idx / H;
    const int h = idx - n * H;
    const long long g0 = n * 4LL * H + h;
    const float i_s = stash[g0];
    const float g_t = stash[g0 + H];
    const float f_s = stash[g0 + 2 * H];
    const float o_s = stash[g0 + 3 * H];
    const float tc = tanhf(new_c[idx]);
    const float dh = grad_h[n * gh_stride + h];
    const float gc = grad_c ? grad_c[idx] : 0.0f;
    const float d_tc = dh * o_s * (1.0f - tc * tc) + gc;
    grad_c_prev[idx] = d_tc * f_s;
    const float di = d_tc * g_t;
    const float dg = d_tc * i_s;
    const float df = d_tc * c_prev[idx];
    const float do_ = dh * tc;
    grad_gates[g0] = drla_f32_to_bf16(di * i_s * (1.0f - i_s));
    grad_gates[g0 + H] = drla_f32_to_bf16(dg * (1.0f - g_t * g_t));
    grad_gates[g0 + 2 * H] = drla_f32_to_bf16(df * f_s * (1.0f - f_s));
    grad_gates[g0 + 3 * H] = drla_f32_to_bf16(do_ * o_s * (1.0f - o_s));
  }
}


template <bool WH_IN_LDS>
__device__ __forceinline__ void lstm_seq_fwd_impl(
    const bf16raw* __restrict__ xg16,
    const float* __restrict__ xg32,
    const bf16raw* __restrict__ Wh,
    const float* __restrict__ h0,
    const float* __restrict__ c0,
    const unsigned char* __restrict__ done,
    float* __restrict__ h_out,
    float* __restrict__ h_fin,
    float* __restrict__ c_fin,
    float forget_bias, int B, int L, int H) {
  extern __shared__ __attribute__((aligned(16))) char smem[];
  bf16raw* wh_lds = reinterpret_cast<bf16raw*>(smem);
  float* hbuf = reinterpret_cast<float*>(
      wh_lds + (WH_IN_LDS ? drla_lstm_seq_wh_elems(H) : 0));
  float* cbuf = hbuf + H;

  const int b = blockIdx.x;
  const int j = threadIdx.x;
  const int G = 4 * H;

  if (WH_IN_LDS) {
    for (int i = j; i < H * G; i += blockDim.x) wh_lds[i] = Wh[i];
  }
  const bf16raw* wh = WH_IN_LDS ? wh_lds : Wh;
  if (j < H) {
    hbuf[j] = h0[(long long)b * H + j];
    cbuf[j] = c0[(long long)b * H + j];
  }
  __syncthreads();

  for (int t = 0; t < L; ++t) {
    float g = 0.0f;
    for (int k = 0; k < H; ++k) {
      g = fmaf(hbuf[k], lstm_b2f(wh[k * G + j]), g);
    }
    const long long xbase = ((long long)b * L + t) * G + j;
    g += xg16 ? lstm_b2f(xg16[xbase]) : xg32[xbase];
    __shared__ float gates[LSTM_SEQ_MAX_GATES];
// ... 364 lines not shown
```

### distributed_reinforcement_learning_amd/ops/hip/mlp_heads.hip

```cpp

#include "drla_kernels.h"

#define MH_PAD 8
#define MH_LD (MH_HID + MH_PAD)

__device__ __forceinline__ float mh_b2f(bf16raw u) {
  unsigned int x = ((unsigned int)u) << 16;
  return __uint_as_float(x);
}

template <bool RELU, bool ACCUM>
__device__ void mh_pass(const bf16raw (*act_in)[MH_LD],
                        bf16raw (*act_out)[MH_LD],
                        const bf16raw* __restrict__ M,
                        const bf16raw* __restrict__ bias,
                        const bf16raw* __restrict__ mask_stash,
                        bf16raw* __restrict__ dz_global,
                        float* __restrict__ colsum,
                        bf16raw* __restrict__ stash,
                        float* __restrict__ dh_global,
                        int row0, int N, int nout, int kdim) {
  const int tid = threadIdx.x;
  const int wave = tid / 64;
  const int lane = tid % 64;
  const int out0 = wave * 64;
  const bool live = out0 < nout;

  f32x4 acc[4];
  for (int ni = 0; ni < 4; ++ni) acc[ni] = {0.f, 0.f, 0.f, 0.f};

  const bf16x8 zero8 = {0, 0, 0, 0, 0, 0, 0, 0};
  if (live) {
    bf16x8 a_cur0, a_cur1, a_cur2, a_cur3;
    const int kf = (lane >> 4) * 8;
#define DRLA_MH_LOAD(ni, dst, k0)                                       \
    {                                                                   \
      const int orow = out0 + (ni) * 16 + (lane & 15);                  \
      dst = (orow < nout)                                               \
          ? *reinterpret_cast<const bf16x8*>(                           \
                M + (long long)orow * kdim + (k0) + kf)                 \
          : zero8;                                                      \
    }
    DRLA_MH_LOAD(0, a_cur0, 0); DRLA_MH_LOAD(1, a_cur1, 0);
    DRLA_MH_LOAD(2, a_cur2, 0); DRLA_MH_LOAD(3, a_cur3, 0);
    for (int k0 = 0; k0 < kdim; k0 += 32) {
      bf16x8 a_nxt0, a_nxt1, a_nxt2, a_nxt3;
      if (k0 + 32 < kdim) {
        DRLA_MH_LOAD(0, a_nxt0, k0 + 32); DRLA_MH_LOAD(1, a_nxt1, k0 + 32);
        DRLA_MH_LOAD(2, a_nxt2, k0 + 32); DRLA_MH_LOAD(3, a_nxt3, k0 + 32);
      }
      const bf16x8 b_frag =
          *reinterpret_cast<const bf16x8*>(&act_in[lane & 15][k0 + kf]);
      acc[0] = __builtin_amdgcn_mfma_f32_16x16x32_bf16(a_cur0, b_frag,
                                                       acc[0], 0, 0, 0);
      acc[1] = __builtin_amdgcn_mfma_f32_16x16x32_bf16(a_cur1, b_frag,
                                                       acc[1], 0, 0, 0);
      acc[2] = __builtin_amdgcn_mfma_f32_16x16x32_bf16(a_cur2, b_frag,
                                                       acc[2], 0, 0, 0);
      acc[3] = __builtin_amdgcn_mfma_f32_16x16x32_bf16(a_cur3, b_frag,
                                                       acc[3], 0, 0, 0);
      a_cur0 = a_nxt0; a_cur1 = a_nxt1; a_cur2 = a_nxt2; a_cur3 = a_nxt3;
    }
#undef DRLA_MH_LOAD
  }
  __syncthreads();
  if (live) {
    for (int ni = 0; ni < 4; ++ni) {
      for (int r = 0; r < 4; ++r) {
        const int oc = out0 + ni * 16 + (lane >> 4) * 4 + r;
        const int lrow = lane & 15;
        const int grow = row0 + lrow;
        float v = acc[ni][r];
        if (bias) v += (oc < nout) ? mh_b2f(bias[oc]) : 0.0f;
        if (RELU) v = fmaxf(v, 0.0f);
        if (mask_stash) {
          const float a = (grow < N)
              ? mh_b2f(mask_stash[(long long)grow * MH_HID + oc]) : 0.0f;
          v = (a > 0.0f) ? v : 0.0f;
        }
        if (dh_global) {
          if (grow < N && oc < nout) {
            atomicAdd(&dh_global[(long long)grow * MH_HID + oc], v);
          }
        } else {
          const bf16raw bv = drla_f32_to_bf16(v);
          act_out[lrow][oc] = bv;
          if (stash && grow < N && oc < nout) {
            stash[(long long)grow * nout + oc] = bv;
          }
          if (dz_global && grow < N && oc < nout) {
            dz_global[(long long)grow * MH_HID + oc] = bv;
          }
          if (colsum && oc < nout && grow < N) {
            atomicAdd(&colsum[oc], v);
          }
        }
      }
    }
  }
  __syncthreads();
}

extern "C" __global__ __launch_bounds__(256) void drla_mlp_heads_fwd(
    const float* __restrict__ h,
    const bf16raw* __restrict__ W1p, const bf16raw* __restrict__ b1p,
    const bf16raw* __restrict__ W2p, const bf16raw* __restrict__ b2p,
    const bf16raw* __restrict__ W3p, const bf16raw* __restrict__ b3p,
    const bf16raw* __restrict__ W1v, const bf16raw* __restrict__ b1v,
    const bf16raw* __restrict__ W2v, const bf16raw* __restrict__ b2v,
    const bf16raw* __restrict__ W3v, const bf16raw* __restrict__ b3v,
    bf16raw* __restrict__ logits,
    float* __restrict__ value,
    bf16raw* __restrict__ stash,
    int N, int A) {
  __shared__ bf16raw hb[MH_BM][MH_LD];
  __shared__ bf16raw acta[MH_BM][MH_LD];
  __shared__ bf16raw actb[MH_BM][MH_LD];

  const int tid = threadIdx.x;
  const int row0 = blockIdx.x * MH_BM;
  const bool policy = blockIdx.y == 0;
  const long long soff = (long long)N * MH_HID;

  {
    const int r = tid >> 4;
    const int c0 = (tid & 15) * 16;
    const int grow = row0 + r;
    for (int c = 0; c < 16; ++c) {
      const float v = (grow < N) ? h[(long long)grow * MH_HID + c0 + c]
                                 : 0.0f;
      const bf16raw bv = drla_f32_to_bf16(v);
      hb[r][c0 + c] = bv;
      if (policy && grow < N) {
        stash[4 * soff + (long long)grow * MH_HID + c0 + c] = bv;
      }
    }
  }
  __syncthreads();

  if (policy) {
    mh_pass<true, false>(hb, acta, W1p, b1p, nullptr, nullptr, nullptr,
                         stash, nullptr, row0, N, MH_HID, MH_HID);
    mh_pass<true, false>(acta, actb, W2p, b2p, nullptr, nullptr, nullptr,
                         stash + soff, nullptr, row0, N, MH_HID, MH_HID);
    mh_pass<false, false>(actb, acta, W3p, b3p, nullptr, nullptr, nullptr,
                          nullptr, nullptr, row0, N, A, MH_HID);
    const int r = tid >> 3;
    const int c = tid & 7;
    if (r < MH_BM) {
      for (int cc = c; cc < A; cc += 8) {
        if (row0 + r < N) {
          logits[(long long)(row0 + r) * A + cc] = acta[r][cc];
        }
      }
    }
  } else {
    mh_pass<true, false>(hb, acta, W1v, b1v, nullptr, nullptr, nullptr,
                         stash + 2 * soff, nullptr, row0, N, MH_HID,
                         MH_HID);
    mh_pass<true, false>(acta, actb, W2v, b2v, nullptr, nullptr, nullptr,
                         stash + 3 * soff, nullptr, row0, N, MH_HID,
                         MH_HID);
    mh_pass<false, false>(actb, acta, W3v, b3v, nullptr, nullptr, nullptr,
                          nullptr, nullptr, row0, N, 1, MH_HID);
    if (tid < MH_BM && row0 + tid < N) {
      value[row0 + tid] = mh_b2f(acta[tid][0]);
    }
  }
}

extern "C" __global__ __launch_bounds__(256) void drla_mlp_heads_bwd(
    const bf16raw* __restrict__ dlogits,
    const float* __restrict__ dvalue,
    const bf16raw* __restrict__ stash,
    const bf16raw* __restrict__ wT1p, const bf16raw* __restrict__ wT2p,
    const bf16raw* __restrict__ wT3p,
    const bf16raw* __restrict__ wT1v, const bf16raw* __restrict__ wT2v,
    const bf16raw* __restrict__ W3v,
    bf16raw* __restrict__ dz1p, bf16raw* __restrict__ dz2p,
    bf16raw* __restrict__ dz1v, bf16raw* __restrict__ dz2v,
    float* __restrict__ dh,
    float* __restrict__ db1p, float* __restrict__ db2p,
    float* __restrict__ db3p,
    float* __restrict__ db1v, float* __restrict__ db2v,
    float* __restrict__ db3v,
    int N, int A) {
  __shared__ bf16raw dza[MH_BM][MH_LD];
  __shared__ bf16raw dzb[MH_BM][MH_LD];
  __shared__ float colsum[MH_HID];

  const int tid = threadIdx.x;
  const int row0 = blockIdx.x * MH_BM;
  const long long soff = (long long)N * MH_HID;
  const bf16raw* a1p = stash;
  const bf16raw* a2p = stash + soff;
  const bf16raw* a1v = stash + 2 * soff;
  const bf16raw* a2v = stash + 3 * soff;

  if (tid < MH_HID) colsum[tid] = 0.0f;

  if (blockIdx.y == 0) {
    {
      const int r = tid >> 4;
      const int c = tid & 15;
      for (int cc = c; cc < 32; cc += 16) {
// ... 164 lines not shown

  f32x4 acc[4];
  for (int ni = 0; ni < 4; ++ni) acc[ni] = {0.f, 0.f, 0.f, 0.f};

  const int st_kk = tid >> 3;
  const int st_c0 = (tid & 7) * 8;
  const bf16x8 z8 = {0, 0, 0, 0, 0, 0, 0, 0};
  bf16x8 r_act = z8, r_dz = z8;

  auto load_chunk = [&](int k0) {
    const int k = k0 + st_kk;
    r_act = z8;
    if (k < N) {
      r_act = *reinterpret_cast<const bf16x8*>(
          act + (long long)k * MH_HID + n0 + st_c0);
    }
    if (job < 4) {
      r_dz = z8;
      if (k < N) {
        r_dz = *reinterpret_cast<const bf16x8*>(
            dz + (long long)k * MH_HID + m0 + st_c0);
      }
    } else if (job == 4) {
#pragma unroll
      for (int e = 0; e < 8; ++e) {
        const int m = st_c0 + e;
        r_dz[e] = (k < N && m < A)
            ? (short)dlogits[(long long)k * A + m] : (short)0;
      }
    } else {
#pragma unroll
      for (int e = 0; e < 8; ++e) {
        const int m = st_c0 + e;
        r_dz[e] = (k < N && m == 0)
            ? (short)drla_f32_to_bf16(dvalue[k]) : (short)0;
      }
    }
  };

  auto store_chunk = [&]() {
    actT[st_c0 + 0][st_kk] = r_act[0]; actT[st_c0 + 1][st_kk] = r_act[1];
    actT[st_c0 + 2][st_kk] = r_act[2]; actT[st_c0 + 3][st_kk] = r_act[3];
    actT[st_c0 + 4][st_kk] = r_act[4]; actT[st_c0 + 5][st_kk] = r_act[5];
    actT[st_c0 + 6][st_kk] = r_act[6]; actT[st_c0 + 7][st_kk] = r_act[7];
    dzT[st_c0 + 0][st_kk] = r_dz[0]; dzT[st_c0 + 1][st_kk] = r_dz[1];
    dzT[st_c0 + 2][st_kk] = r_dz[2]; dzT[st_c0 + 3][st_kk] = r_dz[3];
    dzT[st_c0 + 4][st_kk] = r_dz[4]; dzT[st_c0 + 5][st_kk] = r_dz[5];
    dzT[st_c0 + 6][st_kk] = r_dz[6]; dzT[st_c0 + 7][st_kk] = r_dz[7];
  };

  load_chunk(0);
  for (int k0 = 0; k0 < N; k0 += 32) {
    store_chunk();
    __syncthreads();
    if (k0 + 32 < N) load_chunk(k0 + 32);
    const bf16x8 a_frag = *reinterpret_cast<const bf16x8*>(
        &dzT[wave * 16 + (lane & 15)][(lane >> 4) * 8]);
    for (int ni = 0; ni < 4; ++ni) {
      const bf16x8 b_frag = *reinterpret_cast<const bf16x8*>(
          &actT[ni * 16 + (lane & 15)][(lane >> 4) * 8]);
      acc[ni] = __builtin_amdgcn_mfma_f32_16x16x32_bf16(
          a_frag, b_frag, acc[ni], 0, 0, 0);
    }
    __syncthreads();
  }
  for (int ni = 0; ni < 4; ++ni) {
    for (int r = 0; r < 4; ++r) {
      const int m = m0 + wave * 16 + (lane >> 4) * 4 + r;
      const int n = n0 + ni * 16 + (lane & 15);
      if (m < M) out[(long long)m * MH_HID + n] = drla_f32_to_bf16(acc[ni][r]);
    }
  }
}


extern "C" __global__ __launch_bounds__(256) void drla_embed_mlp_fwd(
    const long long* __restrict__ pa,
    const bf16raw* __restrict__ table,
    const bf16raw* __restrict__ b1,
    const bf16raw* __restrict__ W2,
    const bf16raw* __restrict__ b2,
    bf16raw* __restrict__ out,
    bf16raw* __restrict__ a1stash,
    int N, int A) {
  __shared__ bf16raw a1img[MH_BM][MH_LD];
  __shared__ bf16raw outimg[MH_BM][MH_LD];
  const int tid = threadIdx.x;
  const int row0 = blockIdx.x * MH_BM;
  {
    const int r = tid >> 4;
    const int c0 = (tid & 15) * 16;
    const int grow = row0 + r;
    const long long idx =
        (grow < N) ? drla_clamp_idx((int)pa[grow], A) : 0;
    const bf16raw* trow = table + idx * MH_HID + c0;
    for (int c = 0; c < 16; ++c) {
      const float v =
          fmaxf(mh_b2f(trow[c]) + mh_b2f(b1[c0 + c]), 0.0f);
      const bf16raw bv = drla_f32_to_bf16(v);
      a1img[r][c0 + c] = bv;
      if (grow < N) a1stash[(long long)grow * MH_HID + c0 + c] = bv;
    }
  }
  __syncthreads();
  mh_pass<true, false>(a1img, outimg, W2, b2, nullptr, nullptr, nullptr,
                       out, nullptr, row0, N, MH_HID, MH_HID);
}

extern "C" __global__ void drla_embed_w2t_pack(
    const bf16raw* __restrict__ w2, bf16raw* __restrict__ out) {
  for (int i = blockIdx.x * blockDim.x + threadIdx.x; i < 65536;
       i += gridDim.x * blockDim.x) {
    out[i] = w2[(i & 255) * 256 + (i >> 8)];
  }
}

extern "C" __global__ __launch_bounds__(256) void drla_embed_mlp_bwd(
    const bf16raw* __restrict__ dy, long long dy_stride,
    const bf16raw* __restrict__ out, const bf16raw* __restrict__ a1stash,
    const bf16raw* __restrict__ W2T,
    bf16raw* __restrict__ dz2,
    bf16raw* __restrict__ da1,
    float* __restrict__ bias_ws, int N) {
  __shared__ bf16raw dz2img[MH_BM][MH_LD];
  __shared__ bf16raw da1img[MH_BM][MH_LD];
  __shared__ float colsum[MH_HID];
  const int tid = threadIdx.x;
  const int row0 = blockIdx.x * MH_BM;
  if (tid < MH_HID) colsum[tid] = 0.0f;
  __syncthreads();
  {
    const int r = tid >> 4;
    const int c0 = (tid & 15) * 16;
    const int grow = row0 + r;
    float part[16];
    for (int c = 0; c < 16; ++c) {
      float v = 0.0f;
      if (grow < N) {
        const float o =
            mh_b2f(out[(long long)grow * MH_HID + c0 + c]);
        if (o > 0.0f) {
          v = mh_b2f(dy[(long long)grow * dy_stride + c0 + c]);
        }
      }
      const bf16raw bv = drla_f32_to_bf16(v);
      dz2img[r][c0 + c] = bv;
      if (grow < N) dz2[(long long)grow * MH_HID + c0 + c] = bv;
      part[c] = v;
    }
    for (int c = 0; c < 16; ++c) atomicAdd(&colsum[c0 + c], part[c]);
  }
  __syncthreads();
  if (tid < MH_HID) {
    atomicAdd(&bias_ws[MH_HID + tid], colsum[tid]);
    colsum[tid] = 0.0f;
  }
  __syncthreads();
  mh_pass<false, false>(dz2img, da1img, W2T, nullptr, a1stash, da1,
                        colsum, nullptr, nullptr, row0, N, MH_HID, MH_HID);
  if (tid < MH_HID) atomicAdd(&bias_ws[tid], colsum[tid]);
}

extern "C" __global__ void drla_embed_finalize(
    float* __restrict__ src, bf16raw* __restrict__ dtable,
    bf16raw* __restrict__ db1, bf16raw* __restrict__ db2,
    long long n_table) {
  const long long total = n_table + 512;
  for (long long i = blockIdx.x * (long long)blockDim.x + threadIdx.x;
       i < total; i += gridDim.x * (long long)blockDim.x) {
    const bf16raw v = drla_f32_to_bf16(src[i]);
    src[i] = 0.0f;
    if (i < n_table) dtable[i] = v;
    else if (i < n_table + 256) db1[i - n_table] = v;
    else db2[i - n_table - 256] = v;
  }
}
```

### distributed_reinforcement_learning_amd/ops/hip/vtrace_loss.hip

```cpp

#include "drla_kernels.h"

__device__ __forceinline__ float vt_ld(const bf16raw* p, long long i) {
  unsigned int x = ((unsigned int)p[i]) << 16;
  return __uint_as_float(x);
}

extern "C" __global__ __launch_bounds__(256)
void drla_vtrace_loss_fwd(
    const bf16raw* __restrict__ logits_bf16,
    const float* __restrict__ logits_f32,
    const float* __restrict__ value,
    const float* __restrict__ mu,
    const int* __restrict__ actions,
    const float* __restrict__ rewards,
    const unsigned char* __restrict__ done,
    float gamma, int clip_mode, float c_bl, float c_ent,
    float* __restrict__ p_stash,
    float* __restrict__ vs_stash,
    float* __restrict__ adv_stash,
    float* __restrict__ losses,
    int B, int T, int A) {
  __shared__ float rho[VT_MAX_T];
  __shared__ float vsm[VT_MAX_T];
  __shared__ float rc[VT_MAX_T];
  __shared__ float gc[VT_MAX_T];
  __shared__ float red[3 * 4];

  const int b = blockIdx.x;
  const int tid = threadIdx.x;
  const int Tp = T - 2;
  const long long row = (long long)b * T;

  for (int t = tid; t < T; t += blockDim.x) {
    {
      const float rr = rewards[row + t];
      float rcl;
      if (clip_mode == 0) {
        rcl = fminf(1.0f, fmaxf(-1.0f, rr));
      } else if (clip_mode == 1) {
        const float sq = tanhf(rr * 0.2f);
        rcl = ((rr < 0.0f) ? 0.3f * sq : sq) * 5.0f;
      } else {
        rcl = rr;
      }
      rc[t] = rcl;
      gc[t] = done[row + t] ? 0.0f : gamma;
    }
    const long long base = (row + t) * (long long)A;
    float mx = -1e30f;
    for (int k = 0; k < A; ++k) {
      const float x = logits_bf16 ? vt_ld(logits_bf16, base + k)
                                  : logits_f32[base + k];
      mx = fmaxf(mx, x);
    }
    float denom = 0.0f;
    for (int k = 0; k < A; ++k) {
      const float x = logits_bf16 ? vt_ld(logits_bf16, base + k)
                                  : logits_f32[base + k];
      denom += __expf(x - mx);
    }
    const float inv = 1.0f / denom;
    for (int k = 0; k < A; ++k) {
      const float x = logits_bf16 ? vt_ld(logits_bf16, base + k)
                                  : logits_f32[base + k];
      p_stash[base + k] = __expf(x - mx) * inv;
    }
    const int a = drla_clamp_idx(actions[row + t], A);
    rho[t] = p_stash[base + a] / mu[base + a];
  }
  __syncthreads();

  if (tid == 0) {
    const float* v = value + row;
    const float* r = rc;
    const float* g = gc;
    float acc = 0.0f;
    for (int t = Tp - 1; t >= 0; --t) {
      const float c = fminf(1.0f, rho[t + 1]);
      const float delta = c * (r[t + 1] + g[t + 1] * v[t + 2] - v[t + 1]);
      acc = delta + g[t + 1] * c * acc;
      vsm[t] = acc + v[t + 1];
    }
    acc = 0.0f;
    for (int t = Tp - 1; t >= 0; --t) {
      const float c = fminf(1.0f, rho[t]);
      const float delta = c * (r[t] + g[t] * v[t + 1] - v[t]);
      acc = delta + g[t] * c * acc;
      const float vs = acc + v[t];
      vs_stash[b * Tp + t] = vs;
      adv_stash[b * Tp + t] = c * (r[t] + g[t] * vsm[t] - v[t]);
    }
  }
  __syncthreads();

  float pi_l = 0.0f, base_l = 0.0f, ent_l = 0.0f;
  for (int i = tid; i < Tp * A; i += blockDim.x) {
    const int t = i / A;
    const int k = i - t * A;
    const long long pbase = (row + t) * (long long)A;
    const float p = p_stash[pbase + k];
    ent_l += p * __logf(fmaxf(p, 1e-30f));
    if (k == 0) {
      const float adv = adv_stash[b * Tp + t];
      pi_l -= __logf(p_stash[pbase + drla_clamp_idx(
                  actions[row + t], A)] + 1e-8f) * adv;
      const float diff = vs_stash[b * Tp + t] - value[row + t];
      base_l += 0.5f * diff * diff;
    }
  }
  for (int off = DRLA_WAVE / 2; off > 0; off >>= 1) {
    pi_l += __shfl_down(pi_l, off, DRLA_WAVE);
    base_l += __shfl_down(base_l, off, DRLA_WAVE);
    ent_l += __shfl_down(ent_l, off, DRLA_WAVE);
  }
  const int wave = tid / DRLA_WAVE;
  const int lane = tid % DRLA_WAVE;
  if (lane == 0) {
    red[wave] = pi_l;
    red[4 + wave] = base_l;
    red[8 + wave] = ent_l;
  }
  __syncthreads();
  if (tid == 0) {
    float s0 = 0, s1 = 0, s2 = 0;
    for (int w = 0; w < (int)(blockDim.x / DRLA_WAVE); ++w) {
      s0 += red[w];
      s1 += red[4 + w];
      s2 += red[8 + w];
    }
    atomicAdd(&losses[0], s0);
    atomicAdd(&losses[1], s1);
    atomicAdd(&losses[2], s2);
    atomicAdd(&losses[3], s0 + c_bl * s1 + c_ent * s2);
  }
}

extern "C" __global__ void drla_vtrace_loss_bwd(
    const float* __restrict__ p_stash, const float* __restrict__ vs_stash,
    const float* __restrict__ adv_stash, const float* __restrict__ value,
    const int* __restrict__ actions, const float* __restrict__ grad3,
    int from_total, float c_bl, float c_ent,
    bf16raw* __restrict__ dlogits_bf16, float* __restrict__ dlogits_f32,
    float* __restrict__ dvalue, int B, int T, int A) {
  const float gpi = grad3[0];
  const float gb = from_total ? gpi * c_bl : grad3[1];
  const float ge = from_total ? gpi * c_ent : grad3[2];
  const int Tp = T - 2;
  long long i = blockIdx.x * (long long)blockDim.x + threadIdx.x;
  const long long total = (long long)B * T;
  const long long stride = gridDim.x * (long long)blockDim.x;
  for (; i < total; i += stride) {
    const int b = i / T;
    const int t = i - (long long)b * T;
    const long long pbase = i * A;
    if (t >= Tp) {
      for (int k = 0; k < A; ++k) {
        if (dlogits_bf16) dlogits_bf16[pbase + k] = 0;
        else dlogits_f32[pbase + k] = 0.0f;
      }
      dvalue[i] = 0.0f;
      continue;
    }
    const int wi = b * Tp + t;
    const int a = drla_clamp_idx(actions[i], A);
    const float adv = adv_stash[wi];
    const float sa = p_stash[pbase + a];
    const float w = sa / (sa + 1e-8f);
    float E = 0.0f;
    for (int k = 0; k < A; ++k) {
      const float s = p_stash[pbase + k];
      E += s * __logf(fmaxf(s, 1e-30f));
    }
    for (int k = 0; k < A; ++k) {
      const float s = p_stash[pbase + k];
      const float onehot = (k == a) ? 1.0f : 0.0f;
      const float d_pi = -adv * w * (onehot - s);
      const float d_ent = s * (__logf(fmaxf(s, 1e-30f)) - E);
      const float d = gpi * d_pi + ge * d_ent;
      if (dlogits_bf16) dlogits_bf16[pbase + k] = drla_f32_to_bf16(d);
      else dlogits_f32[pbase + k] = d;
    }
    dvalue[i] = gb * (value[i] - vs_stash[wi]);
  }
}
```

### distributed_reinforcement_learning_amd/ops/lstm_op.py

```python

from __future__ import annotations

from typing import Tuple

import torch

from distributed_reinforcement_learning_amd import ops as _ops

LSTM_SEQ_MAX_HIDDEN = 512


class _FusedLstmTail(torch.autograd.Function):
    @staticmethod
    def forward(ctx, gates: torch.Tensor, c_prev: torch.Tensor,
                forget_bias: float):
        ext = _ops.require_ext()
        new_h, new_c, stash = ext.lstm_tail_fwd(gates.contiguous(),
                                                c_prev.contiguous(),
                                                forget_bias)
        ctx.save_for_backward(stash, c_prev, new_c)
        ctx.bf16_gates = gates.dtype == torch.bfloat16
        ctx.set_materialize_grads(False)
        return new_h, new_c

    @staticmethod
    def backward(ctx, grad_h: torch.Tensor, grad_c: torch.Tensor):
        stash, c_prev, new_c = ctx.saved_tensors
        ext = _ops.require_ext()
        if grad_h is None:
            grad_h = torch.zeros(c_prev.shape, dtype=torch.float32,
                                 device=c_prev.device)
        if not (grad_h.dim() == 2 and grad_h.stride(1) == 1):
            grad_h = grad_h.contiguous()
        grad_gates, grad_c_prev = ext.lstm_tail_bwd(
            grad_h, None if grad_c is None else grad_c.contiguous(),
            stash, c_prev.contiguous(), new_c, ctx.bf16_gates)
        return grad_gates, grad_c_prev, None


def lstm_fused_step(gates: torch.Tensor, c_prev: torch.Tensor,
                    forget_bias: float = 1.0
                    ) -> Tuple[torch.Tensor, torch.Tensor]:
    if gates.is_cuda:
        return _FusedLstmTail.apply(gates, c_prev, forget_bias)
    gates = gates.float()
    i, g, f, o = gates.chunk(4, dim=1)
    new_c = torch.sigmoid(f + forget_bias) * c_prev \
        + torch.sigmoid(i) * torch.tanh(g)
    new_h = torch.sigmoid(o) * torch.tanh(new_c)
    return new_h, new_c


class _LstmSeqTrain(torch.autograd.Function):

    @staticmethod
    def forward(ctx, xg, wh, h0, c0, done, forget_bias):
        ext = _ops.require_ext()
        wh = wh.contiguous()
        done = done.contiguous()
        h_out, h_fin, c_fin, acts, c_prev, h_prev = ext.lstm_seq_train_fwd(
            xg.contiguous(), wh, h0.contiguous(),
            c0.contiguous(), done, forget_bias)
        ctx.save_for_backward(acts, c_prev, h_prev, wh, done)
        ctx.set_materialize_grads(False)
        return h_out, h_fin, c_fin

    @staticmethod
    def backward(ctx, dh_out, dh_fin, dc_fin):
        acts, c_prev, h_prev, wh, done = ctx.saved_tensors
        ext = _ops.require_ext()
        B, L, H = c_prev.shape
        if dh_out is None:
            dh_out = torch.zeros(B, L, H, dtype=torch.float32,
                                 device=c_prev.device)
        dxg, dh0, dc0 = ext.lstm_seq_train_bwd(
            dh_out.float().contiguous(),
            None if dh_fin is None else dh_fin.float().contiguous(),
            None if dc_fin is None else dc_fin.float().contiguous(),
            acts, c_prev, wh, done)
        dwh = h_prev.reshape(B * L, H).t().mm(dxg.reshape(B * L, 4 * H))
        return dxg, dwh, dh0, dc0, None, None


def lstm_seq_train(xg, wh, h0, c0, done, forget_bias: float = 1.0):
    return _LstmSeqTrain.apply(xg, wh, h0, c0, done, float(forget_bias))
```

### distributed_reinforcement_learning_amd/ops/mlp_heads_op.py

```python

from __future__ import annotations

from typing import Tuple

import torch

from distributed_reinforcement_learning_amd import ops as _ops


class _FusedMlpHeads(torch.autograd.Function):
    @staticmethod
    def forward(ctx, h: torch.Tensor,
                w1p, b1p, w2p, b2p, w3p, b3p,
                w1v, b1v, w2v, b2v, w3v, b3v):
        ext = _ops.require_ext()
        A = w3p.shape[0]
        weights = [w1p, w2p, w3p, w1v, w2v, w3v]
        biases = [b.contiguous() for b in (b1p, b2p, b3p, b1v, b2v, b3v)]
        logits, value, stash = ext.mlp_heads_fwd(
            h.contiguous(), [w.contiguous() for w in weights], biases, A)
        ctx.save_for_backward(stash, *weights)
        ctx.A = A
        ctx.N = h.shape[0]
        return logits, value

    @staticmethod
    def backward(ctx, dlogits: torch.Tensor, dvalue: torch.Tensor):
        stash, w1p, w2p, w3p, w1v, w2v, w3v = ctx.saved_tensors
        ext = _ops.require_ext()
        N, A = ctx.N, ctx.A
        dev = stash.device
        if dlogits is None:
            dlogits = torch.zeros(N, A, dtype=torch.bfloat16, device=dev)
        if dvalue is None:
            dvalue = torch.zeros(N, dtype=torch.float32, device=dev)
        dlogits = dlogits.to(torch.bfloat16).contiguous()
        dvalue = dvalue.float().contiguous()
        packed = ext.mlp_heads_pack_wt(
            [w1p, w2p, w3p, w1v, w2v, w3v], A)
        wT = [packed.narrow(0, 0, 65536).view(256, 256),
              packed.narrow(0, 65536, 65536).view(256, 256),
              packed.narrow(0, 131072, 8192).view(256, 32),
              packed.narrow(0, 139264, 65536).view(256, 256),
              packed.narrow(0, 204800, 65536).view(256, 256),
              packed.narrow(0, 270336, 256).view(1, 256)]
        (dz1p, dz2p, dz1v, dz2v, dh, _db1p, _db2p, _db3p, _db1v, _db2v,
         _db3v, ws) = ext.mlp_heads_bwd(dlogits, dvalue, stash, wT, A)
        (dw1p, dw2p, dw3p, dw1v, dw2v, dw3v, db1p, db2p, db3p, db1v,
         db2v, db3v) = ext.mlp_heads_wgrad(
            dz1p, dz2p, dz1v, dz2v, dlogits, dvalue, stash, ws, A)
        return (dh, dw1p, db1p, dw2p, db2p, dw3p, db3p,
                dw1v, db1v, dw2v, db2v, dw3v, db3v)


def fused_mlp_heads(h: torch.Tensor, policy_head, value_head
                    ) -> Tuple[torch.Tensor, torch.Tensor]:
    return _FusedMlpHeads.apply(
        h,
        policy_head.hidden[0].weight, policy_head.hidden[0].bias,
        policy_head.hidden[1].weight, policy_head.hidden[1].bias,
        policy_head.out.weight, policy_head.out.bias,
        value_head.hidden[0].weight, value_head.hidden[0].bias,
        value_head.hidden[1].weight, value_head.hidden[1].bias,
        value_head.out.weight, value_head.out.bias)


def heads_fusable(model, h: torch.Tensor) -> bool:
    ph, vh = model.policy_head, model.value_head
    return (h.is_cuda and h.shape[-1] == 256
            and ph.out.weight.dtype == torch.bfloat16
            and len(ph.hidden) == 2
            and all(l.out_features == 256 for l in ph.hidden)
            and all(l.out_features == 256 for l in vh.hidden)
            and ph.out.out_features <= 32 and vh.out.out_features == 1
            and _ops.available())
```

### distributed_reinforcement_learning_amd/ops/vtrace_loss_op.py

```python

from __future__ import annotations

from typing import Tuple

import torch

from distributed_reinforcement_learning_amd import ops as _ops

_CLIP_MODE = {"abs_one": 0, "soft_asymmetric": 1, "none": 2}


class _FusedVtraceLoss(torch.autograd.Function):
    @staticmethod
    def forward(ctx, logits: torch.Tensor, value: torch.Tensor,
                mu: torch.Tensor, actions: torch.Tensor,
                rewards: torch.Tensor, done: torch.Tensor, gamma: float,
                clip_mode: int, c_bl: float, c_ent: float):
        ext = _ops.require_ext()
        losses, p_stash, vs_stash, adv_stash = ext.vtrace_loss_fwd(
            logits.contiguous(), value.contiguous(), mu.contiguous(),
            actions.contiguous(), rewards.contiguous(), done.contiguous(),
            gamma, clip_mode, c_bl, c_ent)
        ctx.save_for_backward(p_stash, vs_stash, adv_stash,
                              value.contiguous(), actions.contiguous())
        ctx.want_bf16 = logits.dtype == torch.bfloat16
        ctx.coefs = (c_bl, c_ent)
        ctx.set_materialize_grads(False)
        return losses[0], losses[1], losses[2], losses[3]

    @staticmethod
    def backward(ctx, g_pi, g_base, g_ent, g_total):
        p_stash, vs_stash, adv_stash, value, actions = ctx.saved_tensors
        ext = _ops.require_ext()
        c_bl, c_ent = ctx.coefs
        none3 = g_pi is None and g_base is None and g_ent is None
        if g_total is not None and none3:
            grad3 = g_total.reshape(1)
            from_total = True
        else:
            dev = p_stash.device
            z = torch.zeros((), dtype=torch.float32, device=dev)
            grad3 = torch.stack([
                g_pi if g_pi is not None else z,
                g_base if g_base is not None else z,
                g_ent if g_ent is not None else z,
            ]).float().contiguous()
            if g_total is not None:
                grad3 = grad3 + g_total.float() * torch.tensor(
                    [1.0, c_bl, c_ent], device=dev)
            from_total = False
        dlogits, dvalue = ext.vtrace_loss_bwd(
            p_stash, vs_stash, adv_stash, value, actions,
            grad3.float().contiguous(), from_total, c_bl, c_ent,
            ctx.want_bf16)
        return (dlogits, dvalue) + (None,) * 8


def fused_vtrace_loss(logits: torch.Tensor, value: torch.Tensor,
                      mu: torch.Tensor, actions: torch.Tensor,
                      rewards: torch.Tensor, done: torch.Tensor,
                      gamma: float, reward_clipping: str, c_bl: float,
                      c_ent: float
                      ) -> Tuple[torch.Tensor, torch.Tensor, torch.Tensor,
                                 torch.Tensor]:
    return _FusedVtraceLoss.apply(logits, value, mu,
                                  actions.to(torch.int32), rewards, done,
                                  float(gamma), _CLIP_MODE[reward_clipping],
                                  float(c_bl), float(c_ent))
```

### distributed_reinforcement_learning_amd/runtime/graphed.py

```python

from __future__ import annotations

import os
from typing import Dict, Optional, Tuple

import numpy as np
import torch

from distributed_reinforcement_learning_amd.ops import conv_op
from distributed_reinforcement_learning_amd.runtime._capture import (
    CapturedStep, OptimizerGraph, warmup_preserving_state,
)


class GraphedImpalaStep(CapturedStep):
    def __init__(self, agent, batch_size: int, warmup_iters: int = 3):
        assert agent.device.type == "cuda", "graphed step needs a GPU"
        conv_op.STASH_INPUTS = True
        self.agent = agent
        B, T = batch_size, agent.trajectory
        A, H = agent.num_action, agent.lstm_hidden_size
        HH, WW, C = agent.input_shape
        dev = agent.device

        def z(shape, dtype):
            return torch.zeros(shape, dtype=dtype, device=dev)

        self.inputs: Dict[str, torch.Tensor] = {
            "state": z((B, T, HH, WW, C), torch.uint8),
            "reward": z((B, T), torch.float32),
            "action": z((B, T), torch.int32),
            "done": z((B, T), torch.bool),
            "behavior_policy": z((B, T, A), torch.float32),
            "previous_action": z((B, T), torch.int64),
            "initial_h": z((B, T, H), torch.float32),
            "initial_c": z((B, T, H), torch.float32),
        }
        self.pinned: Dict[str, torch.Tensor] = {
            k: torch.empty_like(v, device="cpu").pin_memory()
            for k, v in self.inputs.items()
        }
        self.lr_buf = torch.zeros(1, dtype=torch.float32, device=dev)
        self._consumed = torch.cuda.Event()
        self._consumed.record()
        self._uploaded = torch.cuda.Event()
        self._uploaded.record()
        self._fwd_done = torch.cuda.Event()
        self._copy_stream = torch.cuda.Stream()
        self._primed = False
        self._last_lr = 0.0

        opt = agent.optimizer
        warmup_preserving_state(opt, self._fwd_bwd, warmup_iters, self.lr_buf)

        self.g_fwd = torch.cuda.CUDAGraph()
        with torch.cuda.graph(self.g_fwd):
            self._total, self.losses = self._fwd()
        self._bwd_seed = torch.ones((), device=dev)
        self.g_bwd = torch.cuda.CUDAGraph()
        with torch.cuda.graph(self.g_bwd, pool=self.g_fwd.pool()):
            self._total.backward(gradient=self._bwd_seed,
                                 retain_graph=True)
            conv_op.join_wgrad_stream()
        opt.build_gather_table()
        self._opt = OptimizerGraph(agent, self.lr_buf, self.g_fwd.pool())

    def _fwd(self):
        agent = self.agent
        i = dict(self.inputs)
        if os.environ.get("DRLA_NO_INPUT_CLONE") != "1":
            for k in ("previous_action", "action", "initial_c"):
                i[k] = i[k].clone()
        s = agent.prepare_frames(i["state"])
        pi_loss, baseline_loss, entropy, total = agent.compute_losses(
            s, i["reward"], i["action"], i["done"], i["behavior_policy"],
            i["previous_action"], i["initial_h"], i["initial_c"])
        return total, (pi_loss.detach(), baseline_loss.detach(),
                       entropy.detach())

    def _fwd_bwd(self) -> Tuple[torch.Tensor, ...]:
        agent = self.agent
        if not agent.optimizer.scatter:
            agent.optimizer.flat_grads.zero_()
        total, losses = self._fwd()
        total.backward()
        return losses


    def stage_to_pinned(self, batch: Dict[str, np.ndarray]) -> None:
        for k, pin in self.pinned.items():
            pin.copy_(torch.as_tensor(np.asarray(batch[k])))

    def upload_inputs(self, src: Optional[Dict[str, torch.Tensor]] = None
                      ) -> None:
        self._consumed.synchronize()
        src = src or self.pinned
        for k, dst in self.inputs.items():
            dst.copy_(src[k], non_blocking=True)
        self._uploaded.record()
        self._primed = True

    def _upload_overlapped(self, src: Dict[str, torch.Tensor]) -> None:
        with torch.cuda.stream(self._copy_stream):
            self._copy_stream.wait_event(self._fwd_done)
            for k, dst in self.inputs.items():
                dst.copy_(src[k], non_blocking=True)
            self._uploaded.record(self._copy_stream)

    def wait_pinned_free(self) -> None:
        self._uploaded.synchronize()


    def step(self, batch: Optional[Dict[str, np.ndarray]] = None,
             pinned_src: Optional[Dict[str, torch.Tensor]] = None
             ) -> Tuple[torch.Tensor, ...]:
        agent = self.agent
        main = torch.cuda.current_stream()
        if batch is not None:
            self.stage_to_pinned(batch)
            self.upload_inputs()
            src = None
        else:
            src = pinned_src if pinned_src is not None else self.pinned
            if not self._primed:
                self.upload_inputs(src)
                src = None
        main.wait_event(self._uploaded)
        self._last_lr = self._opt.begin_step()
        self.g_fwd.replay()
        self._fwd_done.record(main)
        if src is not None:
            self._upload_overlapped(src)
        self.g_bwd.replay()
        self._opt.replay()
        self._consumed.record()
        agent.global_step += 1
        agent.num_env_frames += int(np.prod(self.inputs["reward"].shape))
        return self.losses

    def last_losses(self) -> Tuple[float, float, float, float]:
        pi, bl, ent = (float(x) for x in self.losses)
        return pi, bl, ent, self._last_lr
```

Before: 1.014 million frames/s.

## Write conv, embedding and h directly into a shared LSTM input slab

The conv3 output, the fused action embedding and the hidden state are now written straight into one preallocated bf16 xh slab with a ones-pad column, so the torch.cat before the gate GEMM goes away. Inside the graph, the per-step input clones are replaced by kernels that stash the small tensors they need for backward (idx, c, actions). Other parts of the diff: the V-trace loss drops its zero-fill in favour of a last-block partials reduction, and the transposed weights for the MLP heads and embedding are precomputed during forward. The cost is added complexity from strided outputs, alignment checks and static scratch buffers.

```diff
diff --git a/distributed_reinforcement_learning_amd/models/blocks.py b/distributed_reinforcement_learning_amd/models/blocks.py
--- a/distributed_reinforcement_learning_amd/models/blocks.py
+++ b/distributed_reinforcement_learning_amd/models/blocks.py
@@ -51,12 +51,25 @@
         self.fc2 = nn.Linear(hidden, hidden)
         self.out_features = hidden
 
+    def fused_ok(self) -> bool:
+        from distributed_reinforcement_learning_amd.ops import available
+        t = self.table
+        return (t.is_cuda and t.dtype == torch.bfloat16
+                and t.shape[1] == 256 and self.fc2.out_features == 256
+                and available())
+
+    def forward_into(self, prev_action: torch.Tensor, xh_slab: torch.Tensor,
+                     emb_col: int, h: torch.Tensor) -> torch.Tensor:
+        from distributed_reinforcement_learning_amd.ops import embed_op
+        assert self.fused_ok()
+        return embed_op.fused_action_embed(
+            prev_action.long(), self.table, self.bias1, self.fc2.weight,
+            self.fc2.bias, xh_slab, emb_col, h)
+
     def forward(self, prev_action: torch.Tensor) -> torch.Tensor:
-        from distributed_reinforcement_learning_amd.ops import embed_op, available
+        from distributed_reinforcement_learning_amd.ops import embed_op
         t = self.table
-        if (t.is_cuda and t.dtype == torch.bfloat16
-                and t.shape[1] == 256 and self.fc2.out_features == 256
-                and available()):
+        if self.fused_ok():
             return embed_op.fused_action_embed(
                 prev_action.long(), t, self.bias1, self.fc2.weight,
                 self.fc2.bias)
@@ -166,6 +179,13 @@
             return lstm_fused_step(g, c.float(), self.forget_bias)
         return lstm_fused_step(g.float(), c.float(), self.forget_bias)
 
+    def forward_slab(self, xh: torch.Tensor, c: torch.Tensor):
+        from distributed_reinforcement_learning_amd.ops.lstm_op import (
+            lstm_fused_step,
+        )
+        g = torch.mm(xh, _AugGateWeight.apply(self.weight, self.bias))
+        return lstm_fused_step(g, c.float(), self.forget_bias)
+
     def forward_xh(self, xh: torch.Tensor, c: torch.Tensor):
         from distributed_reinforcement_learning_amd.ops.lstm_op import (
             lstm_fused_step,
diff --git a/distributed_reinforcement_learning_amd/models/impala_actor_critic.py b/distributed_reinforcement_learning_amd/models/impala_actor_critic.py
--- a/distributed_reinforcement_learning_amd/models/impala_actor_critic.py
+++ b/distributed_reinforcement_learning_amd/models/impala_actor_critic.py
@@ -36,12 +36,44 @@
     def forward(self, state, prev_action, h, c):
         return self.single_step(state, prev_action, h, c)
 
+    USE_XH_SLAB = True
+
+    def _xh_slab_ok(self, flat_state, flat_h) -> bool:
+        if not (self.USE_XH_SLAB and flat_state.is_cuda
+                and flat_state.dtype == torch.uint8):
+            return False
+        from distributed_reinforcement_learning_amd.ops.conv_op import (
+            custom_stack_ok,
+        )
+        return (custom_stack_ok(self.conv, flat_state)
+                and self.action_emb.fused_ok()
+                and self.lstm._aug_weight_ok()
+                and flat_h.dtype == torch.float32
+                and flat_h.shape[1] % 8 == 0)
+
     def _unroll_features(self, traj_state, traj_prev_action, traj_h, traj_c):
         B, T = traj_state.shape[:2]
         flat_state = traj_state.reshape(B * T, *traj_state.shape[2:])
         flat_pa = traj_prev_action.reshape(B * T)
         flat_h = traj_h.reshape(B * T, -1)
         flat_c = traj_c.reshape(B * T, -1)
+        if self._xh_slab_ok(flat_state, flat_h):
+            from distributed_reinforcement_learning_amd.ops import xh_op
+            from distributed_reinforcement_learning_amd.ops.conv_op import (
+                atari_conv_stack,
+            )
+            n_conv = self.conv.out_features
+            H = flat_h.shape[1]
+            slab = torch.empty(
+                B * T, xh_op.slab_width(n_conv, self.action_emb.out_features,
+                                        H),
+                dtype=torch.bfloat16, device=flat_state.device)
+            conv_y = atari_conv_stack(self.conv, flat_state, out_slab=slab)
+            emb = self.action_emb.forward_into(flat_pa, slab, n_conv,
+                                               flat_h.contiguous())
+            xh = xh_op.assemble_xh(conv_y, emb, slab)
+            new_h, _ = self.lstm.forward_slab(xh, flat_c)
+            return new_h, B, T
         conv_out = self.conv(flat_state)
         emb = self.action_emb(flat_pa)
         new_h, _ = self.lstm.forward_cat([conv_out, emb, flat_h], flat_c)
diff --git a/distributed_reinforcement_learning_amd/ops/conv_op.py b/distributed_reinforcement_learning_amd/ops/conv_op.py
--- a/distributed_reinforcement_learning_amd/ops/conv_op.py
+++ b/distributed_reinforcement_learning_amd/ops/conv_op.py
@@ -33,11 +33,11 @@
 class _ConvLayer(torch.autograd.Function):
     @staticmethod
     def forward(ctx, x: torch.Tensor, w_flat: torch.Tensor,
-                bias_f32: torch.Tensor, layer: int):
+                bias_f32: torch.Tensor, layer: int, out_slab=None):
         ext = _ops.require_ext()
         stash = STASH_INPUTS and layer <= 1
         y, x_st = ext.conv_fwd(layer, x.contiguous(), w_flat.contiguous(),
-                               bias_f32.contiguous(), stash)
+                               bias_f32.contiguous(), stash, out_slab)
         ctx.save_for_backward(x_st if stash else x, w_flat, y)
         ctx.layer = layer
         return y
@@ -49,7 +49,9 @@
         layer = ctx.layer
         co = _LAYER_CO[layer]
         if not (dy.is_contiguous() or (dy.stride(-1) == 1
-                                        and dy.dim() >= 2)):
+                                        and dy.dim() >= 2
+                                        and dy.stride(0) % 8 == 0
+                                        and dy.storage_offset() % 8 == 0)):
             dy = dy.contiguous()
         dy_m = ext.relu_mask_bwd(dy, y, co, layer)
         if _side_enabled():
@@ -69,23 +71,26 @@
         dx = None
         if layer >= 2 and ctx.needs_input_grad[0]:
             dx = ext.conv_dgrad(layer, dy_m, w_flat)
-        return dx, dw, dbias, None
+        return dx, dw, dbias, None, None
 
 
 def conv_layer(x: torch.Tensor, conv: torch.nn.Conv2d,
-               layer: int) -> torch.Tensor:
+               layer: int, out_slab=None) -> torch.Tensor:
     w = conv.weight
     co = w.shape[0]
     w_flat = w.permute(0, 2, 3, 1).reshape(co, -1)
-    return _ConvLayer.apply(x, w_flat, conv.bias, layer)
+    return _ConvLayer.apply(x, w_flat, conv.bias, layer, out_slab)
 
 
-def atari_conv_stack(stack, x_u8_nhwc: torch.Tensor) -> torch.Tensor:
+def atari_conv_stack(stack, x_u8_nhwc: torch.Tensor,
+                     out_slab=None) -> torch.Tensor:
     ci = x_u8_nhwc.shape[-1]
     l1 = 0 if ci == 4 else 1
     y = conv_layer(x_u8_nhwc, stack.conv1, l1)
     y = conv_layer(y, stack.conv2, 2)
-    y = conv_layer(y, stack.conv3, 3)
+    y = conv_layer(y, stack.conv3, 3, out_slab)
+    if out_slab is not None:
+        return y
     return y.reshape(y.shape[0], -1)
 
 
diff --git a/distributed_reinforcement_learning_amd/ops/embed_op.py b/distributed_reinforcement_learning_amd/ops/embed_op.py
--- a/distributed_reinforcement_learning_amd/ops/embed_op.py
+++ b/distributed_reinforcement_learning_amd/ops/embed_op.py
@@ -4,12 +4,13 @@
 import torch
 
 from distributed_reinforcement_learning_amd import ops as _ops
+from distributed_reinforcement_learning_amd.ops import conv_op
 
 
 class _EmbedLookup(torch.autograd.Function):
     @staticmethod
     def forward(ctx, table: torch.Tensor, idx: torch.Tensor):
-        ctx.save_for_backward(idx)
+        ctx.save_for_backward(idx.clone() if conv_op.STASH_INPUTS else idx)
         ctx.num_rows = table.shape[0]
         ctx.want_bf16 = table.dtype == torch.bfloat16
         return table.index_select(0, idx)
@@ -33,10 +34,17 @@
 class _FusedActionEmbed(torch.autograd.Function):
 
     @staticmethod
-    def forward(ctx, idx, table, b1, w2, b2):
+    def forward(ctx, idx, table, b1, w2, b2, xh_slab=None, emb_col=0,
+                h=None, grad_on=False):
         ext = _ops.require_ext()
-        out, a1 = ext.embed_mlp_fwd(idx, table, b1, w2, b2)
-        ctx.save_for_backward(idx, a1, out, w2)
+        stash = conv_op.STASH_INPUTS
+        want_w2t = grad_on and any(ctx.needs_input_grad)
+        res = ext.embed_mlp_fwd(idx, table, b1, w2, b2, stash_idx=stash,
+                                want_w2t=want_w2t, xh_slab=xh_slab,
+                                emb_col=emb_col, h=h)
+        out, a1 = res[0], res[1]
+        ctx.save_for_backward(res[2] if stash else idx, a1, out, w2)
+        ctx.w2t = res[-1] if want_w2t else None
         ctx.A = table.shape[0]
         ctx.set_materialize_grads(False)
         return out
@@ -46,14 +54,17 @@
         idx, a1, out, w2 = ctx.saved_tensors
         ext = _ops.require_ext()
         if dy is None:
-            return (None,) * 5
+            return (None,) * 9
         if not (dy.dim() == 2 and dy.stride(1) == 1):
             dy = dy.contiguous()
         dz2, dtable, db1, db2 = ext.embed_mlp_bwd(
-            dy.to(torch.bfloat16), out, a1, w2, idx, ctx.A)
+            dy.to(torch.bfloat16), out, a1, w2, idx, ctx.A, w2t=ctx.w2t,
+            fuse_scatter=True)
         dw2 = dz2.t().mm(a1)
-        return None, dtable, db1, dw2, db2
+        return None, dtable, db1, dw2, db2, None, None, None, None
 
 
-def fused_action_embed(idx, table, b1, w2, b2):
-    return _FusedActionEmbed.apply(idx, table, b1, w2, b2)
+def fused_action_embed(idx, table, b1, w2, b2, xh_slab=None, emb_col=0,
+                       h=None):
+    return _FusedActionEmbed.apply(idx, table, b1, w2, b2, xh_slab, emb_col,
+                                   h, torch.is_grad_enabled())
diff --git a/distributed_reinforcement_learning_amd/ops/hip/bind.cpp b/distributed_reinforcement_learning_amd/ops/hip/bind.cpp
--- a/distributed_reinforcement_learning_amd/ops/hip/bind.cpp
+++ b/distributed_reinforcement_learning_amd/ops/hip/bind.cpp
@@ -133,14 +133,32 @@
 
 std::tuple<torch::Tensor, torch::Tensor> conv_fwd(
     int layer, torch::Tensor in, torch::Tensor w, torch::Tensor bias,
-    bool stash_input) {
+    bool stash_input, c10::optional<torch::Tensor> out_slab) {
   check_gpu_contig(in, "in");
   check_gpu_contig(w, "w");
   check_gpu_contig(bias, "bias");
   const auto& cfg = conv_layer(layer);
   const int batch = in.size(0);
-  auto out = torch::empty({batch, cfg.ho, cfg.wo, cfg.co},
-                          in.options().dtype(torch::kBFloat16));
+  torch::Tensor out;
+  long long out_n_stride = 0;
+  if (out_slab.has_value()) {
+    const auto& slab = *out_slab;
+    const long long row = (long long)cfg.ho * cfg.wo * cfg.co;
+    TORCH_CHECK(layer >= 2, "out_slab is a bf16-layer feature");
+    TORCH_CHECK(slab.is_cuda() && slab.dim() == 2 &&
+                    slab.scalar_type() == torch::kBFloat16 &&
+                    slab.size(0) == batch && slab.size(1) >= row &&
+                    slab.stride(1) == 1 && slab.stride(0) >= slab.size(1),
+                "out_slab must be a row-major [batch, >= ho*wo*co] bf16 "
+                "buffer");
+    out_n_stride = slab.stride(0);
+    out = slab.as_strided(
+        {batch, cfg.ho, cfg.wo, cfg.co},
+        {out_n_stride, (long long)cfg.wo * cfg.co, cfg.co, 1});
+  } else {
+    out = torch::empty({batch, cfg.ho, cfg.wo, cfg.co},
+                       in.options().dtype(torch::kBFloat16));
+  }
   const dim3 grid(conv_m_tiles(batch * cfg.ho * cfg.wo));
   torch::Tensor x_stash;
   unsigned char* stashp = nullptr;
@@ -157,7 +175,7 @@
   } else {
     hipLaunchKernelGGL(kConvFwdBf16[layer - 2], grid, dim3(DRLA_CONV_BLOCK),
                        0, cur_stream(), BF16P(in), BF16P(w), BF16P(bias),
-                       BF16PM(out), batch);
+                       BF16PM(out), batch, out_n_stride);
   }
   return {out, x_stash};
 }
@@ -176,26 +194,27 @@
 
 torch::Tensor relu_mask_bwd(torch::Tensor dy, torch::Tensor y, int64_t CO,
                             int64_t slot_id) {
-  check_gpu_contig(y, "y");
-  TORCH_CHECK(dy.is_cuda(), "dy must be on GPU");
-  long long n_stride, row_elems;
-  if (dy.is_contiguous()) {
-    n_stride = row_elems = dy.numel() / dy.size(0);
-  } else {
-    row_elems = 1;
-    for (int d = 1; d < dy.dim(); ++d) {
-      TORCH_CHECK(dy.stride(d - 1) >= dy.stride(d), "dy must be row-major");
-      row_elems *= dy.size(d);
+  TORCH_CHECK(dy.is_cuda() && y.is_cuda(), "dy and y must be on GPU");
+  TORCH_CHECK(dy.numel() == y.numel() && dy.size(0) == y.size(0),
+              "dy and y must hold the same rows");
+  long long row_elems = dy.numel() / std::max<int64_t>(dy.size(0), 1);
+  auto n_stride_of = [row_elems](const torch::Tensor& t, const char* name) {
+    if (t.is_contiguous()) return row_elems;
+    for (int d = 1; d < t.dim(); ++d) {
+      TORCH_CHECK(t.stride(d - 1) >= t.stride(d), name, " must be row-major");
     }
-    TORCH_CHECK(dy.stride(dy.dim() - 1) == 1 &&
-                    dy.stride(0) >= row_elems && row_elems % 8 == 0,
-                "dy view must be inner-contiguous");
-    for (int d = 1; d + 1 < dy.dim(); ++d) {
-      TORCH_CHECK(dy.stride(d) == dy.size(d + 1) * dy.stride(d + 1),
-                  "dy inner dims must be contiguous");
+    TORCH_CHECK(t.stride(t.dim() - 1) == 1 && t.stride(0) >= row_elems &&
+                    row_elems % 8 == 0 && t.stride(0) % 8 == 0 &&
+                    t.storage_offset() % 8 == 0,
+                name, " view must be inner-contiguous and 16 B aligned");
+    for (int d = 1; d + 1 < t.dim(); ++d) {
+      TORCH_CHECK(t.stride(d) == t.size(d + 1) * t.stride(d + 1), name,
+                  " inner dims must be contiguous");
     }
-    n_stride = dy.stride(0);
-  }
+    return (long long)t.stride(0);
+  };
+  const long long n_stride = n_stride_of(dy, "dy");
+  const long long y_n_stride = n_stride_of(y, "y");
   auto out = torch::empty(dy.sizes(), dy.options());
   auto& slots = dbias_slot_buf(dy, slot_id);
   const long long n = dy.numel();
@@ -205,7 +224,7 @@
   hipLaunchKernelGGL(drla_relu_mask_bwd, dim3(grid), dim3(DRLA_BLOCK),
                      0, cur_stream(), BF16P(dy), BF16P(y), BF16PM(out),
                      slots.data_ptr<float>(), n, (int)CO, n_stride,
-                     row_elems);
+                     row_elems, y_n_stride);
   return out;
 }
 
@@ -601,7 +620,8 @@
 std::vector<torch::Tensor> vtrace_loss_fwd(
     torch::Tensor logits, torch::Tensor value, torch::Tensor mu,
     torch::Tensor actions, torch::Tensor rewards, torch::Tensor done,
-    double gamma, int64_t clip_mode, double c_bl, double c_ent) {
+    double gamma, int64_t clip_mode, double c_bl, double c_ent,
+    bool nofill, bool stash_actions) {
   check_all_gpu_contig("vtrace_loss input", logits, value, mu, actions,
                        rewards, done);
   TORCH_CHECK(actions.scalar_type() == torch::kInt, "actions must be int32");
@@ -614,7 +634,32 @@
   auto p_stash = torch::empty({B, T, A}, fopt);
   auto vs_stash = torch::empty({B, T - 2}, fopt);
   auto adv_stash = torch::empty({B, T - 2}, fopt);
-  auto losses = torch::zeros({4}, fopt);
+  torch::Tensor losses, act_stash;
+  float* partials_ptr = nullptr;
+  unsigned int* counter_ptr = nullptr;
+  if (nofill) {
+    static torch::Tensor partials, counter;
+    static std::vector<torch::Tensor> retired;
+    if (!partials.defined() || partials.size(0) < B ||
+        partials.device() != value.device()) {
+      if (partials.defined()) {
+        retired.push_back(partials);
+        retired.push_back(counter);
+      }
+      partials = torch::zeros({std::max<int64_t>(B, 4096), 4}, fopt);
+      counter = torch::zeros({1}, fopt.dtype(torch::kInt));
+    }
+    partials_ptr = partials.data_ptr<float>();
+    counter_ptr = reinterpret_cast<unsigned int*>(counter.data_ptr<int>());
+    losses = torch::empty({4}, fopt);
+  } else {
+    losses = torch::zeros({4}, fopt);
+  }
+  int* act_stash_ptr = nullptr;
+  if (stash_actions) {
+    act_stash = torch::empty_like(actions);
+    act_stash_ptr = act_stash.data_ptr<int>();
+  }
   hipLaunchKernelGGL(
       drla_vtrace_loss_fwd, dim3(B), dim3(256), 0, cur_stream(),
       lg.bf16, lg.f32, value.data_ptr<float>(), mu.data_ptr<float>(),
@@ -622,7 +667,9 @@
       static_cast<float>(gamma), (int)clip_mode, static_cast<float>(c_bl),
       static_cast<float>(c_ent), p_stash.data_ptr<float>(),
       vs_stash.data_ptr<float>(), adv_stash.data_ptr<float>(),
-      losses.data_ptr<float>(), B, T, A);
+      losses.data_ptr<float>(), B, T, A, partials_ptr, counter_ptr,
+      act_stash_ptr);
+  if (stash_actions) return {losses, p_stash, vs_stash, adv_stash, act_stash};
   return {losses, p_stash, vs_stash, adv_stash};
 }
 
@@ -649,8 +696,9 @@
   return {dlogits, dvalue};
 }
 
-std::tuple<torch::Tensor, torch::Tensor, torch::Tensor> lstm_tail_fwd(
-    torch::Tensor gates, torch::Tensor c_prev, double forget_bias) {
+std::vector<torch::Tensor> lstm_tail_fwd(
+    torch::Tensor gates, torch::Tensor c_prev, double forget_bias,
+    bool stash_c) {
   check_gpu_contig(gates, "gates");
   check_gpu_contig(c_prev, "c_prev");
   const bool bf16 = gates.scalar_type() == torch::kBFloat16;
@@ -666,20 +714,27 @@
   auto new_c = torch::empty_like(c_prev);
   auto stash = torch::empty({N, (long long)H4},
                             c_prev.options().dtype(torch::kFloat));
+  torch::Tensor c_stash;
+  float* c_stash_ptr = nullptr;
+  if (stash_c) {
+    c_stash = torch::empty_like(c_prev);
+    c_stash_ptr = c_stash.data_ptr<float>();
+  }
   if (bf16) {
     hipLaunchKernelGGL(drla_lstm_tail_fwd_bf16, dim3(drla_grid(N * H)),
                        dim3(DRLA_BLOCK), 0, cur_stream(), BF16P(gates),
                        c_prev.data_ptr<float>(), new_h.data_ptr<float>(),
                        new_c.data_ptr<float>(), stash.data_ptr<float>(),
-                       static_cast<float>(forget_bias), N, H);
+                       static_cast<float>(forget_bias), N, H, c_stash_ptr);
   } else {
     hipLaunchKernelGGL(drla_lstm_tail_fwd, dim3(drla_grid(N * H)),
                        dim3(DRLA_BLOCK), 0, cur_stream(),
                        gates.data_ptr<float>(), c_prev.data_ptr<float>(),
                        new_h.data_ptr<float>(), new_c.data_ptr<float>(),
                        stash.data_ptr<float>(),
-                       static_cast<float>(forget_bias), N, H);
-  }
+                       static_cast<float>(forget_bias), N, H, c_stash_ptr);
+  }
+  if (stash_c) return {new_h, new_c, stash, c_stash};
   return {new_h, new_c, stash};
 }
 
@@ -725,7 +780,7 @@
 
 std::vector<torch::Tensor> mlp_heads_fwd(
     torch::Tensor h, std::vector<torch::Tensor> weights,
-    std::vector<torch::Tensor> biases, int64_t A) {
+    std::vector<torch::Tensor> biases, int64_t A, bool want_bwd_bufs) {
   check_gpu_contig(h, "h");
   TORCH_CHECK(weights.size() == 6 && biases.size() == 6);
   for (auto& t : weights) check_gpu_contig(t, "W");
@@ -736,6 +791,16 @@
   auto logits = torch::empty({N, A}, bopt);
   auto value = torch::empty({N}, h.options().dtype(torch::kFloat));
   auto stash = torch::empty({N, 5 * 256}, bopt);
+  torch::Tensor ws, wt;
+  float* ws_ptr = nullptr;
+  bf16raw* wt_ptr = nullptr;
+  if (want_bwd_bufs) {
+    ws = torch::empty({(long long)N * 256 + 4 * 256 + A + 1},
+                      h.options().dtype(torch::kFloat));
+    wt = torch::empty({4 * 65536 + 256 * 32 + 256}, bopt);
+    ws_ptr = ws.data_ptr<float>();
+    wt_ptr = BF16PM(wt);
+  }
   hipLaunchKernelGGL(
       drla_mlp_heads_fwd, dim3(mh_row_tiles(N), 2), dim3(256), 0,
       cur_stream(), h.data_ptr<float>(),
@@ -743,13 +808,16 @@
       BF16P(biases[1]), BF16P(weights[2]), BF16P(biases[2]),
       BF16P(weights[3]), BF16P(biases[3]), BF16P(weights[4]),
       BF16P(biases[4]), BF16P(weights[5]), BF16P(biases[5]),
-      BF16PM(logits), value.data_ptr<float>(), BF16PM(stash), N, (int)A);
+      BF16PM(logits), value.data_ptr<float>(), BF16PM(stash), N, (int)A,
+      wt_ptr, ws_ptr);
+  if (want_bwd_bufs) return {logits, value, stash, ws, wt};
   return {logits, value, stash};
 }
 
 std::vector<torch::Tensor> mlp_heads_bwd(
     torch::Tensor dlogits, torch::Tensor dvalue, torch::Tensor stash,
-    std::vector<torch::Tensor> weights, int64_t A) {
+    std::vector<torch::Tensor> weights, int64_t A,
+    c10::optional<torch::Tensor> ws_opt) {
   check_gpu_contig(dlogits, "dlogits");
   check_gpu_contig(dvalue, "dvalue");
   check_gpu_contig(stash, "stash");
@@ -762,7 +830,15 @@
   auto dz1v = torch::empty({N, 256}, bopt);
   auto dz2v = torch::empty({N, 256}, bopt);
   const long long ws_n = (long long)N * 256 + 4 * 256 + A + 1;
-  auto ws = torch::zeros({ws_n}, fopt);
+  torch::Tensor ws;
+  if (ws_opt.has_value()) {
+    ws = *ws_opt;
+    check_gpu_contig(ws, "ws");
+    TORCH_CHECK(ws.scalar_type() == torch::kFloat && ws.numel() == ws_n,
+                "ws must be f32 [N*256 + 4*256 + A + 1]");
+  } else {
+    ws = torch::zeros({ws_n}, fopt);
+  }
   long long off = 0;
   auto dh = ws.narrow(0, off, (long long)N * 256).view({N, 256});
   off += (long long)N * 256;
@@ -785,51 +861,115 @@
           db3v, ws};
 }
 
-std::tuple<torch::Tensor, torch::Tensor> embed_mlp_fwd(
+std::vector<torch::Tensor> embed_mlp_fwd(
     torch::Tensor pa, torch::Tensor table, torch::Tensor b1,
-    torch::Tensor w2, torch::Tensor b2) {
+    torch::Tensor w2, torch::Tensor b2, bool stash_idx, bool want_w2t,
+    c10::optional<torch::Tensor> xh_slab, int64_t emb_col,
+    c10::optional<torch::Tensor> h_opt) {
   check_all_gpu_contig("embed fwd input", pa, table, b1, w2, b2);
   TORCH_CHECK(pa.scalar_type() == torch::kLong, "pa must be int64");
   const int N = pa.numel();
   auto bopt = table.options();
-  auto out = torch::empty({N, 256}, bopt);
+  torch::Tensor out;
+  long long slab_stride = 0;
+  const float* h_ptr = nullptr;
+  int H = 0;
+  if (xh_slab.has_value()) {
+    const auto& slab = *xh_slab;
+    TORCH_CHECK(h_opt.has_value(), "xh_slab needs h");
+    const auto& h = *h_opt;
+    check_gpu_contig(h, "h");
+    check_gpu_contig(slab, "xh_slab");
+    TORCH_CHECK(h.scalar_type() == torch::kFloat && h.dim() == 2 &&
+                    h.size(0) == N && h.size(1) % 8 == 0,
+                "h must be f32 [N, H], H % 8 == 0");
+    H = h.size(1);
+    TORCH_CHECK(slab.dim() == 2 && slab.scalar_type() == torch::kBFloat16 &&
+                    slab.size(0) == N && emb_col >= 0 && emb_col % 8 == 0 &&
+                    slab.size(1) == emb_col + 256 + H + 8 &&
+                    slab.storage_offset() % 8 == 0,
+                "xh_slab must be bf16 [N, emb_col + 256 + H + 8]");
+    slab_stride = slab.stride(0);
+    h_ptr = h.data_ptr<float>();
+    out = slab.narrow(1, emb_col, 256);
+  } else {
+    out = torch::empty({N, 256}, bopt);
+  }
   auto a1 = torch::empty({N, 256}, bopt);
+  std::vector<torch::Tensor> res = {out, a1};
+  long long* idx_ptr = nullptr;
+  bf16raw* w2t_ptr = nullptr;
+  if (stash_idx) {
+    res.push_back(torch::empty({N}, pa.options()));
+    idx_ptr = reinterpret_cast<long long*>(res.back().data_ptr<int64_t>());
+  }
+  if (want_w2t) {
+    res.push_back(torch::empty({256, 256}, bopt));
+    w2t_ptr = BF16PM(res.back());
+  }
   hipLaunchKernelGGL(drla_embed_mlp_fwd, dim3(mh_row_tiles(N)), dim3(256), 0,
                      cur_stream(), i64p(pa), BF16P(table), BF16P(b1),
                      BF16P(w2), BF16P(b2), BF16PM(out), BF16PM(a1), N,
-                     (int)table.size(0));
-  return {out, a1};
+                     (int)table.size(0), idx_ptr, w2t_ptr, slab_stride, h_ptr,
+                     H);
+  return res;
 }
 
 std::vector<torch::Tensor> embed_mlp_bwd(torch::Tensor dy, torch::Tensor out,
                                          torch::Tensor a1, torch::Tensor w2,
-                                         torch::Tensor idx, int64_t A) {
-  check_all_gpu_contig("embed bwd input", out, a1, w2);
+                                         torch::Tensor idx, int64_t A,
+                                         c10::optional<torch::Tensor> w2t_opt,
+                                         bool fuse_scatter) {
+  check_all_gpu_contig("embed bwd input", a1, w2);
   check_gpu_contig(idx, "idx");
+  TORCH_CHECK(out.is_cuda() && out.dim() == 2 && out.size(1) == 256 &&
+                  out.stride(1) == 1 && out.stride(0) >= 256,
+              "out must be row-contiguous [N,256]");
+  const long long out_stride = out.stride(0);
+  TORCH_CHECK(idx.scalar_type() == torch::kLong && idx.numel() == out.size(0),
+              "idx must be int64 [N]");
   TORCH_CHECK(dy.is_cuda() && dy.dim() == 2 && dy.stride(1) == 1,
               "dy must be row-contiguous");
   const int N = out.size(0);
   const long long n_table = (long long)A * 256;
-  auto bopt = out.options();
-  static torch::Tensor w2t, scratch;
-  if (!w2t.defined()) w2t = torch::empty({65536}, bopt);
+  auto bopt = a1.options();
+  static torch::Tensor w2t_own, scratch;
   if (!scratch.defined() || scratch.numel() != n_table + 512) {
     scratch = torch::zeros({n_table + 512}, bopt.dtype(torch::kFloat));
   }
-  hipLaunchKernelGGL(drla_embed_w2t_pack, dim3(drla_grid(65536)),
-                     dim3(DRLA_BLOCK), 0, cur_stream(), BF16P(w2),
-                     BF16PM(w2t));
+  torch::Tensor w2t;
+  if (w2t_opt.has_value()) {
+    w2t = *w2t_opt;
+    check_gpu_contig(w2t, "w2t");
+    TORCH_CHECK(w2t.numel() == 65536 && w2t.scalar_type() == w2.scalar_type(),
+                "w2t must be bf16 [256,256]");
+  } else {
+    if (!w2t_own.defined()) w2t_own = torch::empty({65536}, bopt);
+    w2t = w2t_own;
+    hipLaunchKernelGGL(drla_embed_w2t_pack, dim3(drla_grid(65536)),
+                       dim3(DRLA_BLOCK), 0, cur_stream(), BF16P(w2),
+                       BF16PM(w2t));
+  }
   auto dz2 = torch::empty({N, 256}, bopt);
-  auto da1 = torch::empty({N, 256}, bopt);
   float* bias_ws = scratch.data_ptr<float>() + n_table;
-  hipLaunchKernelGGL(drla_embed_mlp_bwd, dim3(mh_row_tiles(N)), dim3(256), 0,
-                     cur_stream(), BF16P(dy), (long long)dy.stride(0),
-                     BF16P(out), BF16P(a1), BF16P(w2t), BF16PM(dz2),
-                     BF16PM(da1), bias_ws, N);
-  hipLaunchKernelGGL(
-      drla_embed_bwd_scatter, dim3(drla_grid((long long)N * 256)),
-      dim3(DRLA_BLOCK), 0, cur_stream(), i64p(idx), BF16P(da1), nullptr,
-      scratch.data_ptr<float>(), N, 256, (long long)A);
+  if (fuse_scatter) {
+    hipLaunchKernelGGL(drla_embed_mlp_bwd, dim3(mh_row_tiles(N)), dim3(256),
+                       0, cur_stream(), BF16P(dy), (long long)dy.stride(0),
+                       BF16P(out), BF16P(a1), BF16P(w2t), BF16PM(dz2),
+                       (bf16raw*)nullptr, bias_ws, N, i64p(idx),
+                       scratch.data_ptr<float>(), (int)A, out_stride);
+  } else {
+    auto da1 = torch::empty({N, 256}, bopt);
+    hipLaunchKernelGGL(drla_embed_mlp_bwd, dim3(mh_row_tiles(N)), dim3(256),
+                       0, cur_stream(), BF16P(dy), (long long)dy.stride(0),
+                       BF16P(out), BF16P(a1), BF16P(w2t), BF16PM(dz2),
+                       BF16PM(da1), bias_ws, N, (const long long*)nullptr,
+                       (float*)nullptr, (int)A, out_stride);
+    hipLaunchKernelGGL(
+        drla_embed_bwd_scatter, dim3(drla_grid((long long)N * 256)),
+        dim3(DRLA_BLOCK), 0, cur_stream(), i64p(idx), BF16P(da1), nullptr,
+        scratch.data_ptr<float>(), N, 256, (long long)A);
+  }
   auto dtable = torch::empty({A, 256}, bopt);
   auto db1 = torch::empty({256}, bopt);
   auto db2 = torch::empty({256}, bopt);
@@ -1141,12 +1281,21 @@
         "uint8 frames -> bf16/255 (K11)");
   m.def("vtrace_scan", &vtrace_scan, "fused V-trace reverse scan (K5)");
   m.def("vtrace_loss_fwd", &vtrace_loss_fwd,
-        "fused IMPALA loss pipeline forward (K5+K7+K13)");
+        "fused IMPALA loss pipeline forward (K5+K7+K13); nofill: ticketed "
+        "fixed-order loss sums, no zero-fill; stash_actions: also returns "
+        "a copy of actions made in-kernel",
+        py::arg("logits"), py::arg("value"), py::arg("mu"),
+        py::arg("actions"), py::arg("rewards"), py::arg("done"),
+        py::arg("gamma"), py::arg("clip_mode"), py::arg("c_bl"),
+        py::arg("c_ent"), py::arg("nofill") = false,
+        py::arg("stash_actions") = false);
   m.def("vtrace_loss_bwd", &vtrace_loss_bwd,
         "fused IMPALA loss pipeline backward (closed form)");
   m.def("mfma_probe", &mfma_probe, "16x16x32 bf16 MFMA layout probe");
   m.def("conv_fwd", &conv_fwd,
-        "MFMA implicit-GEMM conv fwd, fused normalize+bias+ReLU (K1)");
+        "MFMA implicit-GEMM conv fwd, fused normalize+bias+ReLU (K1)",
+        py::arg("layer"), py::arg("x"), py::arg("w"), py::arg("bias"),
+        py::arg("stash_input"), py::arg("out_slab") = py::none());
   m.def("conv_wgrad", &conv_wgrad, "MFMA conv weight gradient (K1 bwd)");
   m.def("conv_dgrad", &conv_dgrad, "MFMA conv data gradient (K1 bwd)");
   m.def("relu_mask_bwd", &relu_mask_bwd,
@@ -1179,16 +1328,29 @@
         "GPU PER interior-sum rebuild (float32 drift repair)");
   m.def("embed_bwd", &embed_bwd,
         "action-embedding table gradient (K2 backward)");
-  m.def("lstm_tail_fwd", &lstm_tail_fwd, "fused LSTM gate tail fwd (K3)");
+  m.def("lstm_tail_fwd", &lstm_tail_fwd, "fused LSTM gate tail fwd (K3)",
+        py::arg("gates"), py::arg("c_prev"), py::arg("forget_bias"),
+        py::arg("stash_c") = false);
   m.def("lstm_tail_bwd", &lstm_tail_bwd, "fused LSTM gate tail bwd (K3)");
   m.def("mlp_heads_fwd", &mlp_heads_fwd,
-        "fused policy+value MLP heads forward (K4)");
+        "fused policy+value MLP heads forward (K4)",
+        py::arg("h"), py::arg("weights"), py::arg("biases"), py::arg("A"),
+        py::arg("want_bwd_bufs") = false);
   m.def("mlp_heads_bwd", &mlp_heads_bwd,
-        "fused heads dgrad chain + ReLU masks + bias grads (K4 bwd)");
+        "fused heads dgrad chain + ReLU masks + bias grads (K4 bwd)",
+        py::arg("dlogits"), py::arg("dvalue"), py::arg("stash"),
+        py::arg("weights"), py::arg("A"), py::arg("ws") = py::none());
   m.def("embed_mlp_fwd", &embed_mlp_fwd,
-        "fused action-embedding MLP forward (K2)");
+        "fused action-embedding MLP forward (K2)",
+        py::arg("pa"), py::arg("table"), py::arg("b1"), py::arg("w2"),
+        py::arg("b2"), py::arg("stash_idx") = false,
+        py::arg("want_w2t") = false, py::arg("xh_slab") = py::none(),
+        py::arg("emb_col") = 0, py::arg("h") = py::none());
   m.def("embed_mlp_bwd", &embed_mlp_bwd,
-        "fused action-embedding MLP backward (K2 bwd)");
+        "fused action-embedding MLP backward (K2 bwd)",
+        py::arg("dy"), py::arg("out"), py::arg("a1"), py::arg("w2"),
+        py::arg("idx"), py::arg("A"), py::arg("w2t") = py::none(),
+        py::arg("fuse_scatter") = false);
   m.def("mlp_heads_pack_wt", &mlp_heads_pack_wt,
         "one-kernel transposed-weight pack for the heads dgrad");
   m.def("mlp_heads_wgrad", &mlp_heads_wgrad,
diff --git a/distributed_reinforcement_learning_amd/ops/hip/conv.hip b/distributed_reinforcement_learning_amd/ops/hip/conv.hip
--- a/distributed_reinforcement_learning_amd/ops/hip/conv.hip
+++ b/distributed_reinforcement_learning_amd/ops/hip/conv.hip
@@ -33,7 +33,8 @@
                               const bf16raw* __restrict__ bias,
                               bf16raw* __restrict__ out,
                               int batch,
-                              IN_T* __restrict__ x_stash = nullptr) {
+                              IN_T* __restrict__ x_stash = nullptr,
+                              long long out_n_stride = 0) {
   constexpr int K = KH * KW * CI;
   constexpr int BM = DRLA_CONV_BM;
   constexpr int BK = 32;
@@ -183,15 +184,18 @@
     __syncthreads();
   }
 
+  if (out_n_stride == 0) out_n_stride = (long long)HO * WO * CO;
   for (int mi = 0; mi < 2; ++mi) {
-    for (int ni = 0; ni < NFRAG; ++ni) {
-      const int col = ni * 16 + (lane & 15);
-      const float b = BiasBuf[col];
-      for (int r = 0; r < 4; ++r) {
-        const int grow = row0 + wave * 32 + mi * 16 + (lane >> 4) * 4 + r;
-        if (grow < M) {
-          const float v = fmaxf(acc[mi][ni][r] + b, 0.0f);
-          out[(long long)grow * CO + col] = drla_f32_to_bf16(v);
+    for (int r = 0; r < 4; ++r) {
+      const int grow = row0 + wave * 32 + mi * 16 + (lane >> 4) * 4 + r;
+      if (grow < M) {
+        const int n = grow / (HO * WO);
+        bf16raw* orow = out + (long long)n * out_n_stride +
+                        (grow - n * (HO * WO)) * CO + (lane & 15);
+        for (int ni = 0; ni < NFRAG; ++ni) {
+          const float v =
+              fmaxf(acc[mi][ni][r] + BiasBuf[ni * 16 + (lane & 15)], 0.0f);
+          orow[ni * 16] = drla_f32_to_bf16(v);
         }
       }
     }
@@ -227,21 +231,24 @@
 
 CONV_KERNEL drla_conv_fwd_l2(
     const bf16raw* in, const bf16raw* w, const bf16raw* bias, bf16raw* out,
-    int batch) {
-  conv_fwd_impl<bf16raw, DRLA_CONV_GEOM(2)>(in, w, bias, out, batch);
+    int batch, long long out_n_stride) {
+  conv_fwd_impl<bf16raw, DRLA_CONV_GEOM(2)>(in, w, bias, out, batch, nullptr,
+                                            out_n_stride);
 }
 
 CONV_KERNEL drla_conv_fwd_l3(
     const bf16raw* in, const bf16raw* w, const bf16raw* bias, bf16raw* out,
-    int batch) {
-  conv_fwd_impl<bf16raw, DRLA_CONV_GEOM(3)>(in, w, bias, out, batch);
+    int batch, long long out_n_stride) {
+  conv_fwd_impl<bf16raw, DRLA_CONV_GEOM(3)>(in, w, bias, out, batch, nullptr,
+                                            out_n_stride);
 }
 
 
 extern "C" __global__ void drla_relu_mask_bwd(
     const bf16raw* __restrict__ dy, const bf16raw* __restrict__ y,
     bf16raw* __restrict__ out, float* __restrict__ dbias_slots,
-    long long n, int CO, long long n_stride, long long row_elems) {
+    long long n, int CO, long long n_stride, long long row_elems,
+    long long y_n_stride) {
   const long long n8 = n / 8;
   const long long stride = gridDim.x * (long long)blockDim.x;
   long long i = blockIdx.x * (long long)blockDim.x + threadIdx.x;
@@ -264,14 +271,17 @@
   }
   const long long row8 = row_elems / 8;
   const bool strided = (n_stride != row_elems);
+  const bool y_strided = (y_n_stride != row_elems);
   for (; i < n8; i += stride) {
-    long long si = i;
-    if (strided) {
+    long long si = i, yi = i;
+    if (strided || y_strided) {
       const long long r = i / row8;
-      si = (r * n_stride + (i - r * row8) * 8) / 8;
+      const long long c8 = i - r * row8;
+      if (strided) si = (r * n_stride) / 8 + c8;
+      if (y_strided) yi = (r * y_n_stride) / 8 + c8;
     }
     const uint4 dv = dy4[si];
-    const uint4 yv = y4[i];
+    const uint4 yv = y4[yi];
     uint4 ov;
     DRLA_RM_LANE(dv.x, yv.x, ov.x, acc[0], acc[1]);
     DRLA_RM_LANE(dv.y, yv.y, ov.y, acc[2], acc[3]);
diff --git a/distributed_reinforcement_learning_amd/ops/hip/drla_kernels.h b/distributed_reinforcement_learning_amd/ops/hip/drla_kernels.h
--- a/distributed_reinforcement_learning_amd/ops/hip/drla_kernels.h
+++ b/distributed_reinforcement_learning_amd/ops/hip/drla_kernels.h
@@ -23,19 +23,20 @@
 DRLA_KERNEL drla_vtrace_loss_fwd(
     const bf16raw*, const float*, const float*, const float*, const int*,
     const float*, const unsigned char*, float, int, float, float, float*,
-    float*, float*, float*, int, int, int);
+    float*, float*, float*, int, int, int, float*, unsigned int*, int*);
 DRLA_KERNEL drla_vtrace_loss_bwd(
     const float*, const float*, const float*, const float*, const int*,
     const float*, int, float, float, bf16raw*, float*, float*, int, int,
     int);
 
 DRLA_KERNEL drla_lstm_tail_fwd(const float*, const float*, float*, float*,
-                               float*, float, long long, int);
+                               float*, float, long long, int, float*);
 DRLA_KERNEL drla_lstm_tail_bwd(const float*, const float*, const float*,
                                const float*, const float*, float*, float*,
                                long long, int, long long);
 DRLA_KERNEL drla_lstm_tail_fwd_bf16(const bf16raw*, const float*, float*,
-                                    float*, float*, float, long long, int);
+                                    float*, float*, float, long long, int,
+                                    float*);
 DRLA_KERNEL drla_lstm_tail_bwd_bf16(const float*, const float*, const float*,
                                     const float*, const float*, bf16raw*,
                                     float*, long long, int, long long);
@@ -89,11 +90,12 @@
                                 const bf16raw*, bf16raw*, int,
                                 unsigned char*);
 DRLA_KERNEL drla_conv_fwd_l2(const bf16raw*, const bf16raw*, const bf16raw*,
-                             bf16raw*, int);
+                             bf16raw*, int, long long);
 DRLA_KERNEL drla_conv_fwd_l3(const bf16raw*, const bf16raw*, const bf16raw*,
-                             bf16raw*, int);
+                             bf16raw*, int, long long);
 DRLA_KERNEL drla_relu_mask_bwd(const bf16raw*, const bf16raw*, bf16raw*,
-                               float*, long long, int, long long, long long);
+                               float*, long long, int, long long, long long,
+                               long long);
 DRLA_KERNEL drla_wgrad_finalize(float*, bf16raw*, int, int, float*,
                                 bf16raw*);
 DRLA_KERNEL drla_conv_wgrad_l1(const unsigned char*, const bf16raw*, float*,
@@ -157,7 +159,7 @@
     const float*, const bf16raw*, const bf16raw*, const bf16raw*,
     const bf16raw*, const bf16raw*, const bf16raw*, const bf16raw*,
     const bf16raw*, const bf16raw*, const bf16raw*, const bf16raw*,
-    const bf16raw*, bf16raw*, float*, bf16raw*, int, int);
+    const bf16raw*, bf16raw*, float*, bf16raw*, int, int, bf16raw*, float*);
 DRLA_KERNEL drla_mlp_heads_bwd(
     const bf16raw*, const float*, const bf16raw*, const bf16raw*,
     const bf16raw*, const bf16raw*, const bf16raw*, const bf16raw*,
@@ -174,11 +176,14 @@
     bf16raw*, bf16raw*, bf16raw*, bf16raw*, bf16raw*, int, int);
 DRLA_KERNEL drla_embed_mlp_fwd(const long long*, const bf16raw*,
                                const bf16raw*, const bf16raw*,
-                               const bf16raw*, bf16raw*, bf16raw*, int, int);
+                               const bf16raw*, bf16raw*, bf16raw*, int, int,
+                               long long*, bf16raw*, long long, const float*,
+                               int);
 DRLA_KERNEL drla_embed_w2t_pack(const bf16raw*, bf16raw*);
 DRLA_KERNEL drla_embed_mlp_bwd(const bf16raw*, long long, const bf16raw*,
                                const bf16raw*, const bf16raw*, bf16raw*,
-                               bf16raw*, float*, int);
+                               bf16raw*, float*, int, const long long*,
+                               float*, int, long long);
 DRLA_KERNEL drla_embed_finalize(float*, bf16raw*, bf16raw*, bf16raw*,
                                 long long);
 
diff --git a/distributed_reinforcement_learning_amd/ops/hip/lstm_gates.hip b/distributed_reinforcement_learning_amd/ops/hip/lstm_gates.hip
--- a/distributed_reinforcement_learning_amd/ops/hip/lstm_gates.hip
+++ b/distributed_reinforcement_learning_amd/ops/hip/lstm_gates.hip
@@ -10,7 +10,8 @@
     const float* __restrict__ gates, const float* __restrict__ c_prev,
     float* __restrict__ new_h, float* __restrict__ new_c,
     float* __restrict__ stash,
-    float forget_bias, long long N, int H) {
+    float forget_bias, long long N, int H,
+    float* __restrict__ c_stash) {
   long long idx = blockIdx.x * (long long)blockDim.x + threadIdx.x;
   const long long total = N * H;
   const long long stride = gridDim.x * (long long)blockDim.x;
@@ -22,7 +23,9 @@
     const float g_t = tanhf(gates[g0 + H]);
     const float f_s = drla_sigmoid(gates[g0 + 2 * H] + forget_bias);
     const float o_s = drla_sigmoid(gates[g0 + 3 * H]);
-    const float c_new = f_s * c_prev[idx] + i_s * g_t;
+    const float c_in = c_prev[idx];
+    if (c_stash) c_stash[idx] = c_in;
+    const float c_new = f_s * c_in + i_s * g_t;
     new_c[idx] = c_new;
     new_h[idx] = o_s * tanhf(c_new);
     stash[g0] = i_s;
@@ -69,7 +72,8 @@
     const unsigned short* __restrict__ gates,
     const float* __restrict__ c_prev, float* __restrict__ new_h,
     float* __restrict__ new_c, float* __restrict__ stash, float forget_bias,
-    long long N, int H) {
+    long long N, int H,
+    float* __restrict__ c_stash) {
   long long idx = blockIdx.x * (long long)blockDim.x + threadIdx.x;
   const long long total = N * H;
   const long long stride = gridDim.x * (long long)blockDim.x;
@@ -82,7 +86,9 @@
     const float f_s = drla_sigmoid(lstm_b2f(gates[g0 + 2 * H])
                                    + forget_bias);
     const float o_s = drla_sigmoid(lstm_b2f(gates[g0 + 3 * H]));
-    const float c_new = f_s * c_prev[idx] + i_s * g_t;
+    const float c_in = c_prev[idx];
+    if (c_stash) c_stash[idx] = c_in;
+    const float c_new = f_s * c_in + i_s * g_t;
     new_c[idx] = c_new;
     new_h[idx] = o_s * tanhf(c_new);
     stash[g0] = i_s;
diff --git a/distributed_reinforcement_learning_amd/ops/hip/mlp_heads.hip b/distributed_reinforcement_learning_amd/ops/hip/mlp_heads.hip
--- a/distributed_reinforcement_learning_amd/ops/hip/mlp_heads.hip
+++ b/distributed_reinforcement_learning_amd/ops/hip/mlp_heads.hip
@@ -101,6 +101,16 @@
   __syncthreads();
 }
 
+__device__ __forceinline__ void mh_wt_unit(const bf16raw* __restrict__ w,
+                                           bf16raw* __restrict__ out,
+                                           int u) {
+  const int r = u & 255;
+  const int k0 = (u >> 8) * 8;
+  const bf16x8 v = *reinterpret_cast<const bf16x8*>(w + r * 256 + k0);
+#pragma unroll
+  for (int j = 0; j < 8; ++j) out[(k0 + j) * 256 + r] = (bf16raw)v[j];
+}
+
 extern "C" __global__ __launch_bounds__(256) void drla_mlp_heads_fwd(
     const float* __restrict__ h,
     const bf16raw* __restrict__ W1p, const bf16raw* __restrict__ b1p,
@@ -112,7 +122,9 @@
     bf16raw* __restrict__ logits,
     float* __restrict__ value,
     bf16raw* __restrict__ stash,
-    int N, int A) {
+    int N, int A,
+    bf16raw* __restrict__ wt_pack,
+    float* __restrict__ ws) {
   __shared__ bf16raw hb[MH_BM][MH_LD];
   __shared__ bf16raw acta[MH_BM][MH_LD];
   __shared__ bf16raw actb[MH_BM][MH_LD];
@@ -121,6 +133,43 @@
   const int row0 = blockIdx.x * MH_BM;
   const bool policy = blockIdx.y == 0;
   const long long soff = (long long)N * MH_HID;
+
+  if (wt_pack) {
+    const int gt = (blockIdx.y * gridDim.x + blockIdx.x) * 256 + tid;
+    const int nt = gridDim.x * gridDim.y * 256;
+    for (int u = gt; u < 4 * 8192; u += nt) {
+      const int m = u >> 13;
+      const bf16raw* w = (m == 0) ? W1p : (m == 1) ? W2p
+                       : (m == 2) ? W1v : W2v;
+      const int off = (m == 0) ? 0 : (m == 1) ? 65536
+                    : (m == 2) ? 139264 : 204800;
+      mh_wt_unit(w, wt_pack + off, u & 8191);
+    }
+    for (int e = gt; e < 8192 + 256; e += nt) {
+      if (e < 8192) {
+        const int c = e & 31;
+        wt_pack[131072 + e] =
+            (c < A) ? W3p[c * 256 + (e >> 5)] : (bf16raw)0;
+      } else {
+        wt_pack[270336 + (e - 8192)] = W3v[e - 8192];
+      }
+    }
+  }
+  if (ws && policy) {
+    const int r = tid >> 4;
+    const int c0 = (tid & 15) * 16;
+    const int grow = row0 + r;
+    if (grow < N) {
+      float4* p = reinterpret_cast<float4*>(
+          ws + (long long)grow * MH_HID + c0);
+      const float4 z4 = {0.f, 0.f, 0.f, 0.f};
+      p[0] = z4; p[1] = z4; p[2] = z4; p[3] = z4;
+    }
+    if (blockIdx.x == 0) {
+      const int tail = 4 * MH_HID + A + 1;
+      for (int i = tid; i < tail; i += 256) ws[soff + i] = 0.0f;
+    }
+  }
 
   {
     const int r = tid >> 4;
@@ -451,7 +500,12 @@
     const bf16raw* __restrict__ b2,
     bf16raw* __restrict__ out,
     bf16raw* __restrict__ a1stash,
-    int N, int A) {
+    int N, int A,
+    long long* __restrict__ idx_stash,
+    bf16raw* __restrict__ w2t,
+    long long slab_stride,
+    const float* __restrict__ h_src,
+    int H) {
   __shared__ bf16raw a1img[MH_BM][MH_LD];
   __shared__ bf16raw outimg[MH_BM][MH_LD];
   const int tid = threadIdx.x;
@@ -462,6 +516,7 @@
     const int grow = row0 + r;
     const long long idx =
         (grow < N) ? drla_clamp_idx((int)pa[grow], A) : 0;
+    if (idx_stash && grow < N && (tid & 15) == 0) idx_stash[grow] = idx;
     const bf16raw* trow = table + idx * MH_HID + c0;
     for (int c = 0; c < 16; ++c) {
       const float v =
@@ -473,7 +528,42 @@
   }
   __syncthreads();
   mh_pass<true, false>(a1img, outimg, W2, b2, nullptr, nullptr, nullptr,
-                       out, nullptr, row0, N, MH_HID, MH_HID);
+                       slab_stride ? nullptr : out, nullptr, row0, N, MH_HID,
+                       MH_HID);
+  if (slab_stride != 0) {
+    const int r = tid >> 4;
+    const int c0 = (tid & 15) * 16;
+    const int grow = row0 + r;
+    if (grow < N) {
+      bf16raw* orow = out + (long long)grow * slab_stride;
+      *reinterpret_cast<uint4*>(orow + c0) =
+          *reinterpret_cast<const uint4*>(&outimg[r][c0]);
+      *reinterpret_cast<uint4*>(orow + c0 + 8) =
+          *reinterpret_cast<const uint4*>(&outimg[r][c0 + 8]);
+      bf16raw* hrow = orow + MH_HID;
+#pragma unroll 1
+      for (int c = (tid & 15) * 8; c < H; c += 128) {
+        const float4 v0 = *reinterpret_cast<const float4*>(
+            h_src + (long long)grow * H + c);
+        const float4 v1 = *reinterpret_cast<const float4*>(
+            h_src + (long long)grow * H + c + 4);
+        uint4 p;
+        p.x = drla_f32x2_to_bf16x2(v0.x, v0.y);
+        p.y = drla_f32x2_to_bf16x2(v0.z, v0.w);
+        p.z = drla_f32x2_to_bf16x2(v1.x, v1.y);
+        p.w = drla_f32x2_to_bf16x2(v1.z, v1.w);
+        *reinterpret_cast<uint4*>(hrow + c) = p;
+      }
+      if ((tid & 15) == 0) {
+        *reinterpret_cast<uint4*>(hrow + H) = uint4{0x3F80u, 0u, 0u, 0u};
+      }
+    }
+  }
+  if (w2t) {
+    for (int u = blockIdx.x * 256 + tid; u < 8192; u += gridDim.x * 256) {
+      mh_wt_unit(W2, w2t, u);
+    }
+  }
 }
 
 extern "C" __global__ void drla_embed_w2t_pack(
@@ -490,12 +580,21 @@
     const bf16raw* __restrict__ W2T,
     bf16raw* __restrict__ dz2,
     bf16raw* __restrict__ da1,
-    float* __restrict__ bias_ws, int N) {
+    float* __restrict__ bias_ws, int N,
+    const long long* __restrict__ scat_idx,
+    float* __restrict__ scat,
+    int A,
+    long long out_stride) {
   __shared__ bf16raw dz2img[MH_BM][MH_LD];
   __shared__ bf16raw da1img[MH_BM][MH_LD];
   __shared__ float colsum[MH_HID];
+  __shared__ int srow[MH_BM];
   const int tid = threadIdx.x;
   const int row0 = blockIdx.x * MH_BM;
+  if (scat_idx && tid < MH_BM) {
+    srow[tid] = (row0 + tid < N)
+        ? drla_clamp_idx((int)scat_idx[row0 + tid], A) : -1;
+  }
   if (tid < MH_HID) colsum[tid] = 0.0f;
   __syncthreads();
   {
@@ -507,7 +606,7 @@
       float v = 0.0f;
       if (grow < N) {
         const float o =
-            mh_b2f(out[(long long)grow * MH_HID + c0 + c]);
+            mh_b2f(out[(long long)grow * out_stride + c0 + c]);
         if (o > 0.0f) {
           v = mh_b2f(dy[(long long)grow * dy_stride + c0 + c]);
         }
@@ -528,6 +627,23 @@
   mh_pass<false, false>(dz2img, da1img, W2T, nullptr, a1stash, da1,
                         colsum, nullptr, nullptr, row0, N, MH_HID, MH_HID);
   if (tid < MH_HID) atomicAdd(&bias_ws[tid], colsum[tid]);
+  if (scat_idx) {
+    const int oc = tid;
+    float acc = 0.0f;
+    int cur = -1;
+#pragma unroll 1
+    for (int r = 0; r < MH_BM; ++r) {
+      const int row = srow[r];
+      if (row < 0) break;
+      if (row != cur) {
+        if (cur >= 0) atomicAdd(&scat[(long long)cur * MH_HID + oc], acc);
+        acc = 0.0f;
+        cur = row;
+      }
+      acc += mh_b2f(da1img[r][oc]);
+    }
+    if (cur >= 0) atomicAdd(&scat[(long long)cur * MH_HID + oc], acc);
+  }
 }
 
 extern "C" __global__ void drla_embed_finalize(
diff --git a/distributed_reinforcement_learning_amd/ops/hip/vtrace_loss.hip b/distributed_reinforcement_learning_amd/ops/hip/vtrace_loss.hip
--- a/distributed_reinforcement_learning_amd/ops/hip/vtrace_loss.hip
+++ b/distributed_reinforcement_learning_amd/ops/hip/vtrace_loss.hip
@@ -20,12 +20,17 @@
     float* __restrict__ vs_stash,
     float* __restrict__ adv_stash,
     float* __restrict__ losses,
-    int B, int T, int A) {
+    int B, int T, int A,
+    float* __restrict__ partials,
+    unsigned int* __restrict__ counter,
+    int* __restrict__ act_stash) {
   __shared__ float rho[VT_MAX_T];
   __shared__ float vsm[VT_MAX_T];
   __shared__ float rc[VT_MAX_T];
   __shared__ float gc[VT_MAX_T];
   __shared__ float red[3 * 4];
+  __shared__ int is_last;
+  __shared__ float stage[256];
 
   const int b = blockIdx.x;
   const int tid = threadIdx.x;
@@ -66,7 +71,9 @@
                                   : logits_f32[base + k];
       p_stash[base + k] = __expf(x - mx) * inv;
     }
-    const int a = drla_clamp_idx(actions[row + t], A);
+    const int a_raw = actions[row + t];
+    if (act_stash) act_stash[row + t] = a_raw;
+    const int a = drla_clamp_idx(a_raw, A);
     rho[t] = p_stash[base + a] / mu[base + a];
   }
   __syncthreads();
@@ -129,11 +136,41 @@
       s1 += red[4 + w];
       s2 += red[8 + w];
     }
-    atomicAdd(&losses[0], s0);
-    atomicAdd(&losses[1], s1);
-    atomicAdd(&losses[2], s2);
-    atomicAdd(&losses[3], s0 + c_bl * s1 + c_ent * s2);
-  }
+    if (!partials) {
+      atomicAdd(&losses[0], s0);
+      atomicAdd(&losses[1], s1);
+      atomicAdd(&losses[2], s2);
+      atomicAdd(&losses[3], s0 + c_bl * s1 + c_ent * s2);
+    } else {
+      partials[b * 4 + 0] = s0;
+      partials[b * 4 + 1] = s1;
+      partials[b * 4 + 2] = s2;
+      partials[b * 4 + 3] = s0 + c_bl * s1 + c_ent * s2;
+      __threadfence();
+      const unsigned int ticket = atomicAdd(counter, 1u);
+      is_last = (ticket == (unsigned int)(B - 1));
+    }
+  }
+  if (!partials) return;
+  __syncthreads();
+  if (!is_last) return;
+  __threadfence();
+  float s = 0.0f;
+  for (int base = 0; base < B * 4; base += 256) {
+    const int i = base + tid;
+    stage[tid] = (i < B * 4)
+        ? __hip_atomic_load(&partials[i], __ATOMIC_RELAXED,
+                            __HIP_MEMORY_SCOPE_AGENT)
+        : 0.0f;
+    __syncthreads();
+    if (tid < 4) {
+      const int nb = min(64, B - base / 4);
+      for (int j = 0; j < nb; ++j) s += stage[j * 4 + tid];
+    }
+    __syncthreads();
+  }
+  if (tid < 4) losses[tid] = s;
+  if (tid == 0) *counter = 0u;
 }
 
 extern "C" __global__ void drla_vtrace_loss_bwd(
diff --git a/distributed_reinforcement_learning_amd/ops/lstm_op.py b/distributed_reinforcement_learning_amd/ops/lstm_op.py
--- a/distributed_reinforcement_learning_amd/ops/lstm_op.py
+++ b/distributed_reinforcement_learning_amd/ops/lstm_op.py
@@ -6,6 +6,7 @@
 import torch
 
 from distributed_reinforcement_learning_amd import ops as _ops
+from distributed_reinforcement_learning_amd.ops import conv_op
 
 LSTM_SEQ_MAX_HIDDEN = 512
 
@@ -15,10 +16,11 @@
     def forward(ctx, gates: torch.Tensor, c_prev: torch.Tensor,
                 forget_bias: float):
         ext = _ops.require_ext()
-        new_h, new_c, stash = ext.lstm_tail_fwd(gates.contiguous(),
-                                                c_prev.contiguous(),
-                                                forget_bias)
-        ctx.save_for_backward(stash, c_prev, new_c)
+        stash_c = conv_op.STASH_INPUTS
+        res = ext.lstm_tail_fwd(gates.contiguous(), c_prev.contiguous(),
+                                forget_bias, stash_c=stash_c)
+        new_h, new_c, stash = res[:3]
+        ctx.save_for_backward(stash, res[3] if stash_c else c_prev, new_c)
         ctx.bf16_gates = gates.dtype == torch.bfloat16
         ctx.set_materialize_grads(False)
         return new_h, new_c
diff --git a/distributed_reinforcement_learning_amd/ops/mlp_heads_op.py b/distributed_reinforcement_learning_amd/ops/mlp_heads_op.py
--- a/distributed_reinforcement_learning_amd/ops/mlp_heads_op.py
+++ b/distributed_reinforcement_learning_amd/ops/mlp_heads_op.py
@@ -12,13 +12,18 @@
     @staticmethod
     def forward(ctx, h: torch.Tensor,
                 w1p, b1p, w2p, b2p, w3p, b3p,
-                w1v, b1v, w2v, b2v, w3v, b3v):
+                w1v, b1v, w2v, b2v, w3v, b3v, grad_on=False):
         ext = _ops.require_ext()
         A = w3p.shape[0]
         weights = [w1p, w2p, w3p, w1v, w2v, w3v]
         biases = [b.contiguous() for b in (b1p, b2p, b3p, b1v, b2v, b3v)]
-        logits, value, stash = ext.mlp_heads_fwd(
-            h.contiguous(), [w.contiguous() for w in weights], biases, A)
+        want = grad_on and any(ctx.needs_input_grad)
+        res = ext.mlp_heads_fwd(
+            h.contiguous(), [w.contiguous() for w in weights], biases, A,
+            want_bwd_bufs=want)
+        logits, value, stash = res[:3]
+        ctx.ws, ctx.wt = (res[3], res[4]) if want else (None, None)
+        ctx.ws_used = not want
         ctx.save_for_backward(stash, *weights)
         ctx.A = A
         ctx.N = h.shape[0]
@@ -36,8 +41,12 @@
             dvalue = torch.zeros(N, dtype=torch.float32, device=dev)
         dlogits = dlogits.to(torch.bfloat16).contiguous()
         dvalue = dvalue.float().contiguous()
-        packed = ext.mlp_heads_pack_wt(
-            [w1p, w2p, w3p, w1v, w2v, w3v], A)
+        packed = ctx.wt
+        if packed is None:
+            packed = ext.mlp_heads_pack_wt(
+                [w1p, w2p, w3p, w1v, w2v, w3v], A)
+        ws = None if ctx.ws_used else ctx.ws
+        ctx.ws_used = True
         wT = [packed.narrow(0, 0, 65536).view(256, 256),
               packed.narrow(0, 65536, 65536).view(256, 256),
               packed.narrow(0, 131072, 8192).view(256, 32),
@@ -45,12 +54,13 @@
               packed.narrow(0, 204800, 65536).view(256, 256),
               packed.narrow(0, 270336, 256).view(1, 256)]
         (dz1p, dz2p, dz1v, dz2v, dh, _db1p, _db2p, _db3p, _db1v, _db2v,
-         _db3v, ws) = ext.mlp_heads_bwd(dlogits, dvalue, stash, wT, A)
+         _db3v, ws) = ext.mlp_heads_bwd(dlogits, dvalue, stash, wT, A,
+                                        ws=ws)
         (dw1p, dw2p, dw3p, dw1v, dw2v, dw3v, db1p, db2p, db3p, db1v,
          db2v, db3v) = ext.mlp_heads_wgrad(
             dz1p, dz2p, dz1v, dz2v, dlogits, dvalue, stash, ws, A)
         return (dh, dw1p, db1p, dw2p, db2p, dw3p, db3p,
-                dw1v, db1v, dw2v, db2v, dw3v, db3v)
+                dw1v, db1v, dw2v, db2v, dw3v, db3v, None)
 
 
 def fused_mlp_heads(h: torch.Tensor, policy_head, value_head
@@ -62,7 +72,8 @@
         policy_head.out.weight, policy_head.out.bias,
         value_head.hidden[0].weight, value_head.hidden[0].bias,
         value_head.hidden[1].weight, value_head.hidden[1].bias,
-        value_head.out.weight, value_head.out.bias)
+        value_head.out.weight, value_head.out.bias,
+        torch.is_grad_enabled())
 
 
 def heads_fusable(model, h: torch.Tensor) -> bool:
diff --git a/distributed_reinforcement_learning_amd/ops/vtrace_loss_op.py b/distributed_reinforcement_learning_amd/ops/vtrace_loss_op.py
--- a/distributed_reinforcement_learning_amd/ops/vtrace_loss_op.py
+++ b/distributed_reinforcement_learning_amd/ops/vtrace_loss_op.py
@@ -6,6 +6,7 @@
 import torch
 
 from distributed_reinforcement_learning_amd import ops as _ops
+from distributed_reinforcement_learning_amd.ops import conv_op
 
 _CLIP_MODE = {"abs_one": 0, "soft_asymmetric": 1, "none": 2}
 
@@ -17,12 +18,17 @@
                 rewards: torch.Tensor, done: torch.Tensor, gamma: float,
                 clip_mode: int, c_bl: float, c_ent: float):
         ext = _ops.require_ext()
-        losses, p_stash, vs_stash, adv_stash = ext.vtrace_loss_fwd(
+        stash = conv_op.STASH_INPUTS
+        actions = actions.contiguous()
+        res = ext.vtrace_loss_fwd(
             logits.contiguous(), value.contiguous(), mu.contiguous(),
-            actions.contiguous(), rewards.contiguous(), done.contiguous(),
-            gamma, clip_mode, c_bl, c_ent)
+            actions, rewards.contiguous(), done.contiguous(),
+            gamma, clip_mode, c_bl, c_ent, nofill=True,
+            stash_actions=stash)
+        losses, p_stash, vs_stash, adv_stash = res[:4]
         ctx.save_for_backward(p_stash, vs_stash, adv_stash,
-                              value.contiguous(), actions.contiguous())
+                              value.contiguous(),
+                              res[4] if stash else actions)
         ctx.want_bf16 = logits.dtype == torch.bfloat16
         ctx.coefs = (c_bl, c_ent)
         ctx.set_materialize_grads(False)
diff --git a/distributed_reinforcement_learning_amd/ops/xh_op.py b/distributed_reinforcement_learning_amd/ops/xh_op.py
--- /dev/null
+++ b/distributed_reinforcement_learning_amd/ops/xh_op.py
@@ -0,0 +1,33 @@
+
+from __future__ import annotations
+
+import torch
+
+PAD = 8
+
+
+def slab_width(conv_features: int, emb_features: int, hidden: int) -> int:
+    return conv_features + emb_features + hidden + PAD
+
+
+class _AssembleXh(torch.autograd.Function):
+
+    @staticmethod
+    def forward(ctx, conv_y: torch.Tensor, emb: torch.Tensor,
+                slab: torch.Tensor):
+        ctx.conv_shape = conv_y.shape
+        ctx.n_conv = conv_y[0].numel()
+        ctx.n_emb = emb.shape[1]
+        return slab.view_as(slab)
+
+    @staticmethod
+    def backward(ctx, dxh: torch.Tensor):
+        n_conv, n_emb = ctx.n_conv, ctx.n_emb
+        d_conv = dxh[:, :n_conv].view(ctx.conv_shape)
+        d_emb = dxh[:, n_conv:n_conv + n_emb]
+        return d_conv, d_emb, None
+
+
+def assemble_xh(conv_y: torch.Tensor, emb: torch.Tensor,
+                slab: torch.Tensor) -> torch.Tensor:
+    return _AssembleXh.apply(conv_y, emb, slab)
diff --git a/distributed_reinforcement_learning_amd/runtime/graphed.py b/distributed_reinforcement_learning_amd/runtime/graphed.py
--- a/distributed_reinforcement_learning_amd/runtime/graphed.py
+++ b/distributed_reinforcement_learning_amd/runtime/graphed.py
@@ -1,7 +1,6 @@
 
 from __future__ import annotations
 
-import os
 from typing import Dict, Optional, Tuple
 
 import numpy as np
@@ -67,10 +66,7 @@
 
     def _fwd(self):
         agent = self.agent
-        i = dict(self.inputs)
-        if os.environ.get("DRLA_NO_INPUT_CLONE") != "1":
-            for k in ("previous_action", "action", "initial_c"):
-                i[k] = i[k].clone()
+        i = self.inputs
         s = agent.prepare_frames(i["state"])
         pi_loss, baseline_loss, entropy, total = agent.compute_losses(
             s, i["reward"], i["action"], i["done"], i["behavior_policy"],
```

After: 1.044 million frames/s (median of 6 runs). +3.0%, better.
